# nackdai/aten

Measured on AMD Instinct MI355X. Metric: Mrays/sec (W*H*spp/1e6/s, reference definition), Sponza 1080p 1spp 5-bounce, higher is better.
Workload: dtype f32; 1 GPU; sponza_lod 1920x1080 1spp 5-bounce GGX+IBL, reference-built sponza_lod.sbvh (stand-in for missing sponza.obj); width=1920, height=1080, spp=1, max_depth=5, rr_depth=3, frames_in_flight=4, triangles=12852, bvh_nodes=38000, anyhit_twins=1, planar_area_lights=0

## Files before the change

aten_amd/_lib.py:

```python
import ctypes as C
import os

from . import build

_lib = None

K_NAMES = ["gen_path", "trace_closest", "shade", "trace_shadow", "accumulate_sample", "gather",
           "svgf_prepare", "svgf_temporal", "svgf_variance", "svgf_atrous", "trace_fused"]

SYMBOLS = [
    "atn_create", "atn_destroy", "atn_last_error", "atn_upload_scene", "atn_update_camera", "atn_update_tlas",
    "atn_init_sampler", "atn_set_random", "atn_set_screen_shard", "atn_render", "atn_reset", "atn_set_path_batches",
    "atn_set_frames_in_flight", "atn_bank_streams", "atn_side_stream", "atn_mgpu_set_frames_in_flight", "atn_set_sampling_options", "atn_sample_texture",
    "atn_svgf_render", "atn_svgf_set_motion_depth", "atn_svgf_reset", "atn_svgf_set_atrous_iterations",
    "atn_svgf_download", "atn_svgf_output_device", "atn_svgf_set_dilate_temporal_weight", "atn_svgf_denoise", "atn_svgf_upload",
    "atn_restir_set_options", "atn_restir_render", "atn_restir_set_motion_depth", "atn_restir_reset", "atn_restir_capture",
    "atn_restir_download", "atn_npr_render", "atn_npr_reset", "atn_npr_capture", "atn_npr_download",
    "atn_volume_render", "atn_volume_reset", "atn_volume_capture", "atn_volume_download", "atn_volume_phase_table",
    "atn_ao_set_params", "atn_ao_render", "atn_ao_reset", "atn_ao_capture", "atn_ao_download",
    "atn_film_device", "atn_tile_device", "atn_tile_slots", "atn_anyhit_twins", "atn_planar_area_lights", "atn_stream", "atn_synchronize",
    "atn_assemble_tiles", "atn_assemble_tiles_on", "atn_download_film", "atn_upload_film", "atn_get_stats", "atn_get_kernel_times",
    "atn_reset_kernel_times", "atn_generate_paths", "atn_trace_closest", "atn_cmj_samples", "atn_cmj_batch", "atn_ray_offset", "atn_get_random", "atn_random_count",
    "atn_material_table", "atn_material_eval", "atn_compact", "atn_compact2", "atn_sizeof_scene_desc", "atn_sizeof_destination",
    "atn_abi_version", "atn_build_id",
    "atn_download_path_cost", "atn_update_geometry", "atn_scene_device_arrays", "atn_lbvh_rebuild_list", "atn_lbvh_build",
    "atn_mgpu_update_geometry", "atn_mgpu_lbvh_rebuild_list",
    "atn_skin_create", "atn_skin_update", "atn_skin_compute", "atn_lbvh_rebuild_list_skinned", "atn_skin_download",
    "atn_skin_download_list", "atn_skin_destroy",
    "atn_set_geometry_motion", "atn_geometry_motion_stats", "atn_geometry_motion_matrices",
    "atn_mgpu_create", "atn_mgpu_destroy", "atn_mgpu_last_error", "atn_mgpu_shard_count", "atn_mgpu_shard_device",
    "atn_mgpu_upload_scene", "atn_mgpu_update_tlas", "atn_mgpu_update_camera", "atn_mgpu_init_sampler",
    "atn_mgpu_set_random", "atn_mgpu_render", "atn_mgpu_reset", "atn_mgpu_synchronize", "atn_mgpu_film_device",
    "atn_mgpu_download_film",
    "atn_set_regeneration", "atn_get_regeneration", "atn_render_burst", "atn_regen_stage_counts",
    "atn_mgpu_set_regeneration", "atn_mgpu_render_burst", "atn_set_upload_options", "atn_libm_probe", "atn_set_shade_math",
]


class Destination(C.Structure):
    _fields_ = [("width", C.c_int32), ("height", C.c_int32), ("maxDepth", C.c_int32),
                ("russianRouletteDepth", C.c_int32), ("sample", C.c_int32), ("frame", C.c_uint32),
                ("progressive", C.c_int32), ("break_on_terminate", C.c_int32),
                ("count_stats", C.c_int32), ("profile", C.c_int32)]


def lib():
    global _lib
    if _lib is None:
        path = os.environ.get("ATEN_AMD_LIB", build.HIP_LIB)
        if not os.path.exists(path):
            raise RuntimeError(
                "aten_amd: %s is missing. Build it with `python -m aten_amd.build hip` "
                "(or __graft_entry__.build()); there is no CPU fallback." % path)
        l = C.CDLL(path)
        vp = C.c_void_p
        l.atn_create.argtypes = [C.POINTER(vp), C.c_int]
        l.atn_destroy.argtypes = [vp]; l.atn_destroy.restype = None
        l.atn_last_error.argtypes = [vp]; l.atn_last_error.restype = C.c_char_p
        l.atn_upload_scene.argtypes = [vp, vp]
        l.atn_update_camera.argtypes = [vp, vp]
        l.atn_update_tlas.argtypes = [vp, vp, C.c_uint32, vp, C.c_uint32, vp, C.c_uint32]
        l.atn_download_path_cost.argtypes = [vp, vp]
        l.atn_update_geometry.argtypes = [vp, vp, vp, C.c_uint32, C.c_uint32, vp, C.c_uint32, C.c_uint32]
        l.atn_scene_device_arrays.argtypes = [vp, vp, vp, vp]
        l.atn_lbvh_rebuild_list.argtypes = [vp, C.c_uint32, C.c_uint32, C.c_uint32, vp, vp]
        l.atn_lbvh_build.argtypes = [vp, vp, C.c_uint32, C.c_int32, vp, vp, vp, C.c_uint32, C.c_int32, vp, vp, vp]
        l.atn_skin_create.argtypes = [vp, vp, C.c_uint32, C.c_uint32, C.c_uint32, C.c_uint32, C.c_uint32, C.POINTER(C.c_uint32)]
        l.atn_skin_update.argtypes = [vp, C.c_uint32, vp, C.c_uint32]
        l.atn_skin_compute.argtypes = [vp, C.c_uint32, C.c_int32, vp, vp]
        l.atn_lbvh_rebuild_list_skinned.argtypes = [vp, C.c_uint32, C.c_uint32]
        l.atn_skin_download.argtypes = [vp, C.c_uint32, C.c_int32, vp]
        l.atn_skin_download_list.argtypes = [vp, C.c_uint32, vp, C.c_uint32, C.POINTER(C.c_uint32)]
        l.atn_skin_destroy.argtypes = [vp, C.c_uint32]
        l.atn_set_geometry_motion.argtypes = [vp, C.c_int32]
        l.atn_geometry_motion_stats.argtypes = [vp, vp]
        l.atn_geometry_motion_matrices.argtypes = [vp, vp, vp]
        l.atn_mgpu_update_geometry.argtypes = [vp, vp, vp, C.c_uint32, C.c_uint32, vp, C.c_uint32, C.c_uint32]
        l.atn_mgpu_lbvh_rebuild_list.argtypes = [vp, C.c_uint32, C.c_uint32, C.c_uint32, vp, vp]
        l.atn_init_sampler.argtypes = [vp, C.c_int32, C.c_int32, C.c_int32]
        l.atn_set_random.argtypes = [vp, vp, C.c_uint32]
        l.atn_get_random.argtypes = [vp, vp, C.c_uint32]
        l.atn_random_count.argtypes = [vp]; l.atn_random_count.restype = C.c_uint32
        l.atn_set_screen_shard.argtypes = [vp, C.c_int32, C.c_int32]
        l.atn_render.argtypes = [vp, C.POINTER(Destination), vp]
        l.atn_reset.argtypes = [vp]
        l.atn_set_upload_options.argtypes = [vp, C.c_int32, C.c_int32, C.c_int32, C.c_int32]
        l.atn_set_regeneration.argtypes = [vp, C.c_int32]
        l.atn_set_shade_math.argtypes = [vp, C.c_int32]
        l.atn_get_regeneration.argtypes = [vp]; l.atn_get_regeneration.restype = C.c_int32
        l.atn_render_burst.argtypes = [vp, C.POINTER(Destination), C.c_int32, vp]
        l.atn_regen_stage_counts.argtypes = [vp, vp, vp, C.c_uint32, C.POINTER(C.c_uint32)]
        l.atn_set_path_batches.argtypes = [vp, C.c_int32]
        l.atn_set_frames_in_flight.argtypes = [vp, C.c_int32]
        l.atn_bank_streams.argtypes = [vp, C.POINTER(C.c_int32), C.POINTER(C.c_int32)]
        l.atn_set_sampling_options.argtypes = [vp, C.c_int32, C.c_int32]
        l.atn_sample_texture.argtypes = [vp, C.c_int32, C.c_uint32, vp, vp]
        l.atn_mgpu_set_frames_in_flight.argtypes = [vp, C.c_int32]
        l.atn_svgf_render.argtypes = [vp, vp, C.c_int32, vp, vp]
        l.atn_svgf_set_motion_depth.argtypes = [vp, vp, C.c_uint32]
        l.atn_svgf_reset.argtypes = [vp]
        l.atn_svgf_set_atrous_iterations.argtypes = [vp, C.c_int32]
        l.atn_svgf_download.argtypes = [vp, C.c_int32, vp]
        l.atn_restir_set_options.argtypes = [vp, C.c_int32, C.c_int32]
        l.atn_restir_render.argtypes = [vp, vp, C.c_int32, vp]
        l.atn_restir_set_motion_depth.argtypes = [vp, vp, C.c_uint32]
        l.atn_restir_reset.argtypes = [vp]
        l.atn_restir_capture.argtypes = [vp, C.c_int32]
        l.atn_restir_download.argtypes = [vp, C.c_int32, vp]
        l.atn_npr_render.argtypes = [vp, vp, vp]
        l.atn_npr_reset.argtypes = [vp]
        l.atn_npr_capture.argtypes = [vp, C.c_int32]
        l.atn_npr_download.argtypes = [vp, C.c_int32, vp]
        l.atn_volume_render.argtypes = [vp, vp, vp]
        l.atn_volume_reset.argtypes = [vp]
        l.atn_volume_capture.argtypes = [vp, C.c_int32]
        l.atn_volume_download.argtypes = [vp, C.c_int32, vp]
        l.atn_volume_phase_table.argtypes = [vp, C.c_float, C.c_uint32, vp, vp, vp, vp, vp, vp]
        l.atn_ao_set_params.argtypes = [vp, C.c_int32, C.c_float, C.c_int32]
        l.atn_ao_render.argtypes = [vp, vp, vp]
        l.atn_ao_reset.argtypes = [vp]
        l.atn_ao_capture.argtypes = [vp, C.c_int32]
        l.atn_ao_download.argtypes = [vp, C.c_int32, vp]
        l.atn_svgf_set_dilate_temporal_weight.argtypes = [vp, C.c_int32]
        l.atn_svgf_denoise.argtypes = [vp, vp, C.c_int32, vp, vp]
        l.atn_svgf_upload.argtypes = [vp, C.c_int32, C.c_int32, C.c_int32, vp]
        l.atn_svgf_output_device.argtypes = [vp]
        l.atn_svgf_output_device.restype = vp
        l.atn_film_device.argtypes = [vp]; l.atn_film_device.restype = vp
        l.atn_tile_device.argtypes = [vp]; l.atn_tile_device.restype = vp
        l.atn_tile_slots.argtypes = [vp]; l.atn_tile_slots.restype = C.c_uint32
        l.atn_anyhit_twins.argtypes = [vp]; l.atn_anyhit_twins.restype = C.c_uint32
        l.atn_planar_area_lights.argtypes = [vp]; l.atn_planar_area_lights.restype = C.c_uint32
        l.atn_stream.argtypes = [vp]; l.atn_stream.restype = vp
        l.atn_side_stream.argtypes = [vp]; l.atn_side_stream.restype = vp
        l.atn_synchronize.argtypes = [vp]
        l.atn_assemble_tiles.argtypes = [vp, vp, C.c_int32, vp]
        l.atn_assemble_tiles_on.argtypes = [vp, vp, C.c_int32, vp, vp]
        l.atn_download_film.argtypes = [vp, vp]
        l.atn_upload_film.argtypes = [vp, C.c_int32, C.c_int32, vp]
        l.atn_get_stats.argtypes = [vp, vp]
        l.atn_get_kernel_times.argtypes = [vp, vp, vp]
        l.atn_reset_kernel_times.argtypes = [vp]
        l.atn_generate_paths.argtypes = [vp, C.c_int32, C.c_int32, C.c_int32, C.c_uint32, vp]
        l.atn_trace_closest.argtypes = [vp, vp, C.c_uint32, C.c_float, C.c_float, vp, vp]
        l.atn_cmj_samples.argtypes = [vp, C.c_uint32, C.c_uint32, C.c_uint32, C.c_int32, vp]
        l.atn_cmj_batch.argtypes = [vp, C.c_uint32, vp, vp, vp, C.c_int32, vp]
        l.atn_ray_offset.argtypes = [vp, C.c_uint32, vp, vp, vp]
        l.atn_libm_probe.argtypes = [vp, C.c_int32, C.c_uint32, vp, vp, vp]
        l.atn_material_table.argtypes = [vp, C.c_int32, C.c_uint32, vp, vp, vp, vp, vp, vp, vp, vp]
        l.atn_material_eval.argtypes = [vp, C.c_int32, C.c_uint32, vp, vp, vp, vp, vp]
        l.atn_compact.argtypes = [vp, vp, C.c_uint32, vp, C.POINTER(C.c_uint32)]
        l.atn_compact2.argtypes = [vp, vp, vp, C.c_uint32, C.c_uint32, vp, C.POINTER(C.c_uint32), vp, C.POINTER(C.c_uint32)]
        l.atn_mgpu_create.argtypes = [C.POINTER(vp), vp, C.c_int32]
        l.atn_mgpu_destroy.argtypes = [vp]; l.atn_mgpu_destroy.restype = None
        l.atn_mgpu_last_error.argtypes = [vp]; l.atn_mgpu_last_error.restype = C.c_char_p
        l.atn_mgpu_shard_count.argtypes = [vp]; l.atn_mgpu_shard_count.restype = C.c_int32
        l.atn_mgpu_shard_device.argtypes = [vp, C.c_int32]; l.atn_mgpu_shard_device.restype = C.c_int32
        l.atn_mgpu_upload_scene.argtypes = [vp, vp]
        l.atn_mgpu_update_tlas.argtypes = [vp, vp, C.c_uint32, vp, C.c_uint32, vp, C.c_uint32]
        l.atn_mgpu_update_camera.argtypes = [vp, vp]
        l.atn_mgpu_init_sampler.argtypes = [vp, C.c_int32, C.c_int32, C.c_int32]
        l.atn_mgpu_set_random.argtypes = [vp, vp, C.c_uint32]
        l.atn_mgpu_render.argtypes = [vp, C.POINTER(Destination), vp]
        l.atn_mgpu_reset.argtypes = [vp]
        l.atn_mgpu_set_regeneration.argtypes = [vp, C.c_int32]
        l.atn_mgpu_render_burst.argtypes = [vp, C.POINTER(Destination), C.c_int32, vp]
        l.atn_mgpu_synchronize.argtypes = [vp]
        l.atn_mgpu_film_device.argtypes = [vp]; l.atn_mgpu_film_device.restype = vp
        l.atn_mgpu_download_film.argtypes = [vp, vp]
# ... 6 lines not shown
```

aten_amd/csrc/aten_amd.hip:

```cpp
#include <hip/hip_runtime.h>

#include <algorithm>
#include <cstdio>
#include <cstdlib>
#include <chrono>
#include <cstring>
#include <memory>
#include <random>
#include <string>
#include <vector>

#include "../../include/aten_amd.h"
#include "device/kernels.hpp"
#include "device/launch.hpp"
#include "device/svgf.hpp"
#include "device/restir.hpp"
#include "device/npr.hpp"
#include "device/ao.hpp"
#include "device/volume.hpp"
#include "device/lbvh.hpp"
#include "device/skinning.hpp"
#include "device/motion.hpp"
#include "host/scene_upload.hpp"
#include "host/ibl_precompute.hpp"

namespace atn {

#define ATN_HIP(expr)                                                                      \
    do {                                                                                   \
        hipError_t e_ = (expr);                                                            \
        if (e_ != hipSuccess) { return fail(ATN_ERR_HIP, std::string(#expr) + ": " + hipGetErrorString(e_)); } \
    } while (0)

template <class T>
struct DevBuf {
    T* p = nullptr;
    size_t n = 0;
    ~DevBuf() { release(); }
    void release() { if (p) { (void)hipFree(p); p = nullptr; n = 0; } }
    hipError_t resize(size_t count)
    {
        if (count <= n && p) return hipSuccess;
        release();
        if (count == 0) return hipSuccess;
        hipError_t e = hipMalloc((void**)&p, count * sizeof(T) + 256);
        if (e == hipSuccess) n = count;
        return e;
    }
    void swap(DevBuf& o) { std::swap(p, o.p); std::swap(n, o.n); }
    hipError_t upload(const std::vector<T>& v, hipStream_t s)
    {
        hipError_t e = resize(v.size() ? v.size() : 1);
        if (e != hipSuccess || v.empty()) return e;
        return hipMemcpyAsync(p, v.data(), v.size() * sizeof(T), hipMemcpyHostToDevice, s);
    }
};

__global__ void k_spin(unsigned long long ticks)
{
    const unsigned long long t0 = wall_clock64();
    while (wall_clock64() - t0 < ticks) { }
}
constexpr unsigned long long kSpinTicks = 30000;
inline bool streams_run_side_by_side(hipStream_t a, hipStream_t b, bool& ok)
{
    const double spin_us = (double)kSpinTicks / 100.0;
    for (int rep = 0; rep < 3; rep++) {
        if (hipStreamSynchronize(a) != hipSuccess || hipStreamSynchronize(b) != hipSuccess) { ok = false; return false; }
        const auto t0 = std::chrono::steady_clock::now();
        hipLaunchKernelGGL(k_spin, dim3(1), dim3(1), 0, a, kSpinTicks);
        hipLaunchKernelGGL(k_spin, dim3(1), dim3(1), 0, b, kSpinTicks);
        if (hipStreamSynchronize(a) != hipSuccess || hipStreamSynchronize(b) != hipSuccess) { ok = false; return false; }
        const double us = std::chrono::duration<double, std::micro>(std::chrono::steady_clock::now() - t0).count();
        ok = true;
        if (us < 1.5 * spin_us) return true;
    }
    ok = true;
    return false;
}

class PathTracing {
public:
    std::string last_error;
    int device = 0;
    hipStream_t stream = nullptr;
    static constexpr int kMaxBatches = 8;
    static constexpr int kMaxShards = 64;
    hipStream_t bstream[kMaxBatches] = {};
    hipEvent_t ev_fork = nullptr, ev_join[kMaxBatches] = {};
    int n_batches = 3;
    bool batches_forced = false;
    bool fuse_traces = true;
    bool env_probe_streams = true;
    bool env_lds_nodes = true;
    int env_anyhit_twin = 1;
    int env_anyhit_twin_dirs = 8;
    bool opt_node_layout = true, opt_planar_lights = true;
    bool env_atrous4 = true;
    int env_shade_waves = 0;
    int env_flavour = -1;

    DevBuf<float4> nodes, vtx_pos, vtx_nml, matrices, texels, carpaint, shade_tris;
    DevBuf<atn_triangle_param> tris;
    DevBuf<atn_object_param> objects;
    DevBuf<DevMaterial> materials;
    DevBuf<atn_light_param> lights;
    DevBuf<float4> light_plane;
    DevBuf<DevTexture> textures;
    DevBuf<atn_toon_param> toon;
    DevBuf<atn_light_param> npr_lights;
    DevBuf<float> screen_shadow;
    DevBuf<uint32_t> texels8;
    DevScene scene{};
    bool has_scene = false, has_camera = false;
    std::vector<int32_t> list_root_link;
    uint32_t n_planar_lights = 0;
    struct PlanarCert {
        int32_t inst_obj = -1, mesh_obj = -1, mtx_id = -1;
        atn_object_param inst{}, mesh{};
        atn_mat4 l2w{}, w2l{};
        uint32_t tri_first = 0, tri_count = 0, vtx_lo = 0, vtx_hi = 0;
    };
    std::vector<PlanarCert> planar_certs;
    void collect_planar_certs(const atn_scene_desc* s, const std::vector<atn_light_param>& lights)
    {
        planar_certs.clear();
        for (size_t i = 0; i < lights.size() && i < s->n_lights; i++) {
            if (!lights[i]._pad) continue;
            PlanarCert c;
            c.inst_obj = s->lights[i].arealight_objid;
            c.inst = s->objects[c.inst_obj];
            const atn_object_param* o = &s->objects[c.inst_obj];
            if (o->type == ATN_OBJ_INSTANCE) {
                c.mtx_id = o->mtx_id;
                if (c.mtx_id >= 0) { c.l2w = s->matrices[c.mtx_id]; c.w2l = s->matrices[c.mtx_id + 1]; }
                c.mesh_obj = o->object_id;
                c.mesh = s->objects[c.mesh_obj];
                o = &s->objects[c.mesh_obj];
            }
            c.tri_first = (uint32_t)o->triangle_id; c.tri_count = (uint32_t)o->triangle_num;
            c.vtx_lo = 0xFFFFFFFFu; c.vtx_hi = 0;
            for (uint32_t t = c.tri_first; t < c.tri_first + c.tri_count; t++)
                for (int k = 0; k < 3; k++) {
                    const uint32_t v = (uint32_t)s->triangles[t].idx[k];
                    c.vtx_lo = std::min(c.vtx_lo, v); c.vtx_hi = std::max(c.vtx_hi, v);
                }
            planar_certs.push_back(c);
        }
    }
    bool planar_certs_survive_objects(const atn_object_param* objs, uint32_t n_objs, const atn_mat4* mtxs, uint32_t n_mtxs) const
    {
        for (const PlanarCert& c : planar_certs) {
            if ((uint32_t)c.inst_obj >= n_objs || std::memcmp(&objs[c.inst_obj], &c.inst, sizeof(atn_object_param)) != 0) return false;
            if (c.mesh_obj >= 0 && ((uint32_t)c.mesh_obj >= n_objs || std::memcmp(&objs[c.mesh_obj], &c.mesh, sizeof(atn_object_param)) != 0)) return false;
            if (c.mtx_id >= 0 && n_mtxs
                && ((uint32_t)c.mtx_id + 1 >= n_mtxs || std::memcmp(&mtxs[c.mtx_id], &c.l2w, sizeof(atn_mat4)) != 0
                    || std::memcmp(&mtxs[c.mtx_id + 1], &c.w2l, sizeof(atn_mat4)) != 0)) return false;
        }
        return true;
    }
    bool planar_certs_survive_geometry(uint32_t vtx_offset, uint32_t n_vtx, uint32_t tri_offset, uint32_t n_tr) const
    {
        for (const PlanarCert& c : planar_certs) {
            if (n_vtx && vtx_offset <= c.vtx_hi && (uint64_t)vtx_offset + n_vtx > c.vtx_lo) return false;
            if (n_tr && tri_offset < c.tri_first + c.tri_count && (uint64_t)tri_offset + n_tr > c.tri_first) return false;
        }
        return true;
    }
    std::vector<int32_t> list_twin_delta;
    std::vector<HostSceneImage::TlasRef> tlas_refs;
    uint32_t top_base = 0, n_host_matrices = 0;
    std::vector<atn_mat4> host_matrices;
    std::vector<uint32_t> list_base, list_bytes, list_tri_leaves, list_inner;
    uint32_t n_scene_tris = 0, n_scene_vtx = 0, n_scene_mtrls = 0;

    struct LbvhScratch {
        DevBuf<uint32_t> codes[2], indices[2], counts, totals, arrived, offs;
        DevBuf<uint8_t> flips;
        DevBuf<int32_t> left, right, parent, first, last;
        DevBuf<atn_bvh_node> ref_nodes;
// ... 504 lines not shown
        if (const char* e = std::getenv("ATEN_AMD_PROBE_STREAMS")) env_probe_streams = std::atoi(e) != 0;
        if (const char* e = std::getenv("ATEN_AMD_TRACE")) { env_flavour = e[0] == 'r' ? 1 : 0; }
        if (const char* e = std::getenv("ATEN_AMD_BATCHES")) {
            n_batches = std::atoi(e);
            batches_forced = true;
            if (n_batches < 1) n_batches = 1;
            if (n_batches > kMaxBatches) n_batches = kMaxBatches;
        }
        return ATN_OK;
    }

    ~PathTracing()
    {
        for (auto& e : ev_pool) (void)hipEventDestroy(e);
        for (int k = 0; k < kMaxBatches; k++) {
            if (ev_join[k]) (void)hipEventDestroy(ev_join[k]);
            if (bstream[k]) (void)hipStreamDestroy(bstream[k]);
        }
        if (ev_fork) (void)hipEventDestroy(ev_fork);
        if (rs_ev) (void)hipEventDestroy(rs_ev);
        if (gm_ev) (void)hipEventDestroy(gm_ev);
        if (ao_ev) (void)hipEventDestroy(ao_ev);
        if (ev_gather) (void)hipEventDestroy(ev_gather);
        for (auto& e : sv_ev_prepare) if (e) (void)hipEventDestroy(e);
        if (ev_film) (void)hipEventDestroy(ev_film);
        if (sv_stream) (void)hipStreamDestroy(sv_stream);
        for (int i = 0; i < n_spare_ready; i++) {
            Bank& b = spare[i];
            for (int k = 0; k < kMaxBatches; k++) {
                if (b.ev_join[k]) (void)hipEventDestroy(b.ev_join[k]);
                if (b.bstream[k]) (void)hipStreamDestroy(b.bstream[k]);
            }
            if (b.ev_fork) (void)hipEventDestroy(b.ev_fork);
            if (b.ev_gather) (void)hipEventDestroy(b.ev_gather);
            for (auto& e : b.ev_read) if (e) (void)hipEventDestroy(e);
            if (b.stream) (void)hipStreamDestroy(b.stream);
        }
        if (stream) (void)hipStreamDestroy(stream);
        if (side_stream) (void)hipStreamDestroy(side_stream);
        if (scene_stream) (void)hipStreamDestroy(scene_stream);
        for (auto& e : ev_read) if (e) (void)hipEventDestroy(e);
        if (ev_scene) (void)hipEventDestroy(ev_scene);
        if (ev_stage) (void)hipEventDestroy(ev_stage);
        if (stage_p) (void)hipHostFree(stage_p);
    }

    int UpdateSceneData(const atn_scene_desc* s)
    {
        ATN_HIP(hipSetDevice(device));
        { int q = quiesce(); if (q) return q; }
        drop_alt_set(); cur_set = 0; scene_in_place = false; frame_since_update = true;
        skins.clear();
        HostSceneImage img;
        std::string err;
        const int layout_top = opt_node_layout ? kLayoutTopLevels : 0;
        const bool planar_lights = opt_planar_lights;
        if (!build_host_image(img, s, err, env_anyhit_twin, env_anyhit_twin_dirs, layout_top, planar_lights)) return fail(ATN_ERR_UNSUPPORTED, err);
        n_planar_lights = 0;
        for (const atn_light_param& l : img.lights) n_planar_lights += l._pad != 0 ? 1u : 0u;
        collect_planar_certs(s, img.lights);
        ATN_HIP(nodes.upload(img.nodes, stream));
        ATN_HIP(tris.upload(img.tris, stream));
        ATN_HIP(vtx_pos.upload(img.vtx_pos, stream));
        ATN_HIP(vtx_nml.upload(img.vtx_nml, stream));
        ATN_HIP(objects.upload(img.objects, stream));
        ATN_HIP(matrices.upload(img.matrices, stream));
        ATN_HIP(materials.upload(img.materials, stream));
        ATN_HIP(carpaint.upload(img.carpaint, stream));
        ATN_HIP(toon.upload(img.toon, stream));
        ATN_HIP(npr_lights.upload(img.npr_lights, stream));
        ATN_HIP(screen_shadow.upload(img.screen_shadow, stream));
        ATN_HIP(lights.upload(img.lights, stream));
        ATN_HIP(light_plane.upload(img.light_plane, stream));
        ATN_HIP(texels.upload(img.texels, stream));
        ATN_HIP(texels8.upload(img.texels8, stream));
        ATN_HIP(textures.upload(img.textures, stream));
        ATN_HIP(shade_tris.resize((size_t)kShadeTriQuads * (img.tris.size() ? img.tris.size() : 1)));
        if (!img.tris.empty())
            hipLaunchKernelGGL(k_pack_shade_tris, dim3(((uint32_t)img.tris.size() + 255) / 256), dim3(256), 0, stream, (const atn_triangle_param*)tris.p,
                               (const float4*)vtx_pos.p, (const float4*)vtx_nml.p, 0u, (uint32_t)img.tris.size(), shade_tris.p);
        ATN_HIP(hipGetLastError());
        ATN_HIP(hipStreamSynchronize(stream));
        scene = img.params;
        scene.nodes = nodes.p; scene.tris = tris.p; scene.shade_tris = shade_tris.p; scene.vtx_pos = vtx_pos.p; scene.vtx_nml = vtx_nml.p;
        scene.objects = objects.p; scene.matrices = matrices.p; scene.materials = materials.p; scene.carpaint = carpaint.p;
        scene.toon = toon.p; scene.npr_lights = npr_lights.p; scene.screen_shadow = img.screen_shadow.empty() ? nullptr : screen_shadow.p;
        scene.lights = lights.p; scene.light_plane = light_plane.p; scene.texels = texels.p; scene.texels8 = texels8.p; scene.textures = textures.p;
        scene.mtx_quads = (uint32_t)img.matrices.size();
        has_scene = true;
        if (gm_on) { gm_sv_ids[0] = gm_sv_ids[1] = gm_rs_has_ids = false; const int grc = gm_reset_history(); if (grc) return grc; }
        { const int nrc = npr_decode(s, img); if (nrc) return nrc; }
        { const int vrc = vol_decode(s, img); if (vrc) return vrc; }
        env_host.clear(); env_w = env_h = 0; ibl_tables_ready = false;
        {
            const int32_t ei = s->config.bg.envmap_tex_idx;
            if (ei >= 0 && (uint32_t)ei < s->n_textures && s->config.bg.enable_env_map) {
                const atn_texture_desc& t = s->textures[ei];
                env_host.assign(t.texels, t.texels + (size_t)t.width * t.height);
                env_w = t.width; env_h = t.height; env_multiplyer = s->config.bg.multiplyer;
            }
        }
        {
            int orc = apply_sampling_options();
            if (orc) return orc;
        }
        list_root_link = img.list_root_link; list_twin_delta = img.list_twin_delta; tlas_refs = img.tlas_refs;
        list_base = img.list_root; list_bytes = img.list_bytes; list_tri_leaves = img.list_tri_leaves; list_inner = img.list_inner;
        n_scene_tris = s->n_triangles; n_scene_vtx = s->n_vertices; n_scene_mtrls = s->n_materials;
        top_base = img.list_root[0];
        n_bottom_nodes = img.n_nodes - s->bvh_lists[0].count;
        n_host_matrices = s->n_matrices;
        host_matrices.assign(s->matrices, s->matrices + s->n_matrices);
        tree_is_deep = img.n_nodes >= kRefillMinNodes;
        return ATN_OK;
    }

    int apply_sampling_options()
    {
        scene.tex_bilinear = opt_tex_bilinear;
        scene.ibl_importance = 0;
        scene.ibl_cdf_v = nullptr; scene.ibl_cdf_u = nullptr; scene.ibl_w = 0; scene.ibl_h = 0;
        if (!opt_ibl_importance || env_host.empty()) return ATN_OK;
        if (!ibl_tables_ready) {
            IblTables t;
            const int32_t w = env_w, h = env_h;
            const atn_vec4* tex = env_host.data();
            const float mul = env_multiplyer;
            ibl_precompute(t, w, h, [&](int32_t x, int32_t y, float& r, float& g, float& b) {
                const float u = (float)(x + 0.5) / w, v = (float)(y + 0.5) / h;
                int32_t iu = (int32_t)(u * (float)(w - 1)), iv = (int32_t)(v * (float)(h - 1));
                iu = iu < 0 ? 0 : (iu > w - 1 ? w - 1 : iu); iv = iv < 0 ? 0 : (iv > h - 1 ? h - 1 : iv);
                const atn_vec4& c = tex[(size_t)iv * w + iu];
                r = c.x * mul; g = c.y * mul; b = c.z * mul;
            });
            ATN_HIP(ibl_cdf_v.upload(t.cdf_v, stream));
            ATN_HIP(ibl_cdf_u.upload(t.cdf_u, stream));
            ATN_HIP(hipStreamSynchronize(stream));
            ibl_tables_ready = true;
        }
        scene.ibl_cdf_v = ibl_cdf_v.p; scene.ibl_cdf_u = ibl_cdf_u.p; scene.ibl_w = env_w; scene.ibl_h = env_h;
        scene.ibl_importance = 1;
        return ATN_OK;
    }
    int set_sampling_options(int32_t ibl_importance, int32_t tex_bilinear)
    {
        ATN_HIP(hipSetDevice(device));
        { int q = quiesce(); if (q) return q; }
        opt_ibl_importance = ibl_importance ? 1 : 0;
        opt_tex_bilinear = tex_bilinear ? 1 : 0;
        return has_scene ? apply_sampling_options() : ATN_OK;
    }

    int updateBVH(const atn_object_param* objs, uint32_t n_objs, const atn_mat4* mtxs, uint32_t n_mtxs,
                  const atn_bvh_node* top, uint32_t n_top)
    {
        if (!has_scene) return fail(ATN_ERR_NO_SCENE, "atn_upload_scene has not been called");
        if (!objs || n_objs == 0 || !top || n_top == 0) return fail(ATN_ERR_INVALID_ARG, "empty object or top-layer array");
        ATN_HIP(hipSetDevice(device));
        if ((uint64_t)top_base + (uint64_t)n_top * kInnerBytes >= (1ull << 31)) return fail(ATN_ERR_UNSUPPORTED, "too many BVH nodes for 31-bit byte-offset links");
        if (n_mtxs && !mtxs) return fail(ATN_ERR_INVALID_ARG, "null matrix array");
        {
            std::string rerr;
            if (!validate_ranges(objs, n_objs, n_mtxs ? n_mtxs : n_host_matrices, nullptr, rerr)) return fail(ATN_ERR_UNSUPPORTED, rerr);
            for (uint32_t i = 0; i < n_objs; i++)
                if (objs[i].light_id >= scene.n_lights) return fail(ATN_ERR_UNSUPPORTED, "object light id out of range");
        }
        ListLayout lay;
        std::string err;
        if (!analyse_list(lay, top, n_top, true, err)) return fail(ATN_ERR_UNSUPPORTED, err);
        for (uint32_t j = 0; j < lay.order.size(); j++) {
            if (lay.kind[j] == KIND_TRI) return fail(ATN_ERR_UNSUPPORTED, "triangle leaves in this list need a full scene upload");
            lay.offset[j] = top_base + j * kInnerBytes;
        }
        ListEmitCtx c;
        c.objects = objs; c.n_objects = n_objs; c.n_matrices = n_mtxs ? n_mtxs : n_host_matrices;
        c.matrices = n_mtxs ? mtxs : (host_matrices.size() == n_host_matrices ? host_matrices.data() : nullptr);
        c.list_root_link = list_root_link.data(); c.n_lists = (uint32_t)list_root_link.size();
        c.list_twin_delta = list_twin_delta.size() == list_root_link.size() ? list_twin_delta.data() : nullptr;
        std::vector<HostSceneImage::TlasRef> new_refs;
        c.tlas_refs = &new_refs;
        const size_t top_bytes = lay.order.size() * (size_t)kInnerBytes;
        std::vector<float4> rec(top_bytes / 16 + 1, make_float4(0, 0, 0, 0));
        int32_t root = kLinkEnd;
        uint64_t counts[3] = { 0, 0, 0 };
        if (!emit_list(reinterpret_cast<char*>(rec.data()), lay, top, c, root, counts, err, top_base)) return fail(ATN_ERR_UNSUPPORTED, err);
        std::vector<float4> mv;
        if (n_mtxs) {
            mv.resize((size_t)n_mtxs * 4);
            for (uint32_t i = 0; i < n_mtxs; i++)
                for (int r = 0; r < 4; r++)
                    mv[4 * (size_t)i + r] = make_float4(mtxs[i].m[r][0], mtxs[i].m[r][1], mtxs[i].m[r][2], mtxs[i].m[r][3]);
        }
        const size_t need = ((size_t)top_base + top_bytes + 15) / 16;
        const size_t obj_bytes = (size_t)n_objs * sizeof(atn_object_param), mtx_bytes = mv.size() * sizeof(float4);
        const bool grow = need > nodes.n || n_objs > objects.n || mv.size() > matrices.n;
        if (grow) {
            { int q = quiesce(); if (q) return q; }
            drop_alt_set();
            if (need > nodes.n) {
                float4* bigger = nullptr;
                ATN_HIP(hipMalloc((void**)&bigger, need * sizeof(float4)));
                hipError_t e = hipMemcpyAsync(bigger, nodes.p, (size_t)top_base, hipMemcpyDeviceToDevice, stream);
                if (e == hipSuccess) e = hipStreamSynchronize(stream);
                if (e != hipSuccess) { (void)hipFree(bigger); return fail(ATN_ERR_HIP, hipGetErrorString(e)); }
                nodes.release();
                nodes.p = bigger; nodes.n = need;
            }
            if (n_objs > objects.n) ATN_HIP(objects.resize(n_objs));
            if (mv.size() > matrices.n) ATN_HIP(matrices.resize(mv.size()));
        }
        { int r = begin_scene_update(top_bytes + obj_bytes + mtx_bytes + 512); if (r) return r; }
        { int r = stage_copy(reinterpret_cast<char*>(nodes.p) + top_base, rec.data(), top_bytes); if (r) return r; log_range(SB_NODES, top_base, top_bytes); }
        { int r = stage_copy(objects.p, objs, obj_bytes); if (r) return r; log_range(SB_OBJECTS, 0, obj_bytes); }
        if (n_mtxs) { int r = stage_copy(matrices.p, mv.data(), mtx_bytes); if (r) return r; log_range(SB_MATRICES, 0, mtx_bytes); n_host_matrices = n_mtxs; host_matrices.assign(mtxs, mtxs + n_mtxs); }
        { int r = end_scene_update(); if (r) return r; }
        list_root_link[0] = root;
        if (scene.planar_lights && !planar_certs_survive_objects(objs, n_objs, mtxs, n_mtxs)) scene.planar_lights = 0;
        tlas_refs.swap(new_refs);
        scene.root_link = root;
        fill_root_direct(scene, rec.data(), top_base, n_mtxs ? mtxs : (host_matrices.size() == n_host_matrices ? host_matrices.data() : nullptr), n_mtxs ? n_mtxs : n_host_matrices);
        scene.node_bytes = (uint32_t)(top_base + top_bytes);
        scene.ident_row = c.ident_row;
        if (n_mtxs) scene.mtx_quads = (uint32_t)mv.size();
        point_scene_at_current_set();
        tree_is_deep = n_bottom_nodes + n_top >= kRefillMinNodes;
        return ATN_OK;
    }


    int updateGeometry(const atn_vec4* pos, const atn_vec4* nml, uint32_t n_vtx, uint32_t vtx_offset,
                       const atn_triangle_param* tr, uint32_t n_tr, uint32_t tri_offset)
    {
        if (!has_scene) return fail(ATN_ERR_NO_SCENE, "atn_upload_scene has not been called");
        if ((n_vtx && !pos && !nml) || (n_tr && !tr)) return fail(ATN_ERR_INVALID_ARG, "null geometry array");
        if ((uint64_t)vtx_offset + n_vtx > n_scene_vtx) return fail(ATN_ERR_INVALID_ARG, "vertex range outside the uploaded scene");
        if ((uint64_t)tri_offset + n_tr > n_scene_tris) return fail(ATN_ERR_INVALID_ARG, "triangle range outside the uploaded scene");
        for (uint32_t i = 0; i < n_tr; i++) {
            if (tr[i].mtrlid >= 0 && (uint32_t)tr[i].mtrlid >= n_scene_mtrls) return fail(ATN_ERR_UNSUPPORTED, "triangle material id out of range");
            for (int v = 0; v < 3; v++)
                if (tr[i].idx[v] < 0 || (uint32_t)tr[i].idx[v] >= n_scene_vtx) return fail(ATN_ERR_UNSUPPORTED, "triangle vertex index out of range");
        }
        skins_note_triangles(tr, n_tr, tri_offset);
        ATN_HIP(hipSetDevice(device));
        if (scene.planar_lights && !planar_certs_survive_geometry(vtx_offset, n_vtx, tri_offset, n_tr)) scene.planar_lights = 0;
        const size_t vb = (size_t)n_vtx * sizeof(float4), tb = (size_t)n_tr * sizeof(atn_triangle_param);
        { int r = begin_scene_update((pos ? vb : 0) + (nml ? vb : 0) + tb + 256); if (r) return r; }
        if (n_vtx && pos) { int r = stage_copy(vtx_pos.p + vtx_offset, pos, vb); if (r) return r; log_range(SB_VTX_POS, (size_t)vtx_offset * sizeof(float4), vb); }
        if (n_vtx && nml) { int r = stage_copy(vtx_nml.p + vtx_offset, nml, vb); if (r) return r; log_range(SB_VTX_NML, (size_t)vtx_offset * sizeof(float4), vb); }
        if (n_tr) { int r = stage_copy(tris.p + tri_offset, tr, tb); if (r) return r; log_range(SB_TRIS, (size_t)tri_offset * sizeof(atn_triangle_param), tb); }
        { int r = repack_shade_tris(0, n_scene_tris); if (r) return r; }
        return end_scene_update();
    }

    int repack_shade_tris(uint32_t first, uint32_t count)
    {
        if (!count) return ATN_OK;
        hipLaunchKernelGGL(k_pack_shade_tris, dim3((count + 255) / 256), dim3(256), 0, upd, (const atn_triangle_param*)tris.p,
                           (const float4*)vtx_pos.p, (const float4*)vtx_nml.p, first, count, shade_tris.p);
        ATN_HIP(hipGetLastError());
        log_range(SB_SHADE, (size_t)first * kShadeTriQuads * sizeof(float4), (size_t)count * kShadeTriQuads * sizeof(float4));
        return ATN_OK;
    }

    int lbvh_reserve(uint32_t n)
    {
        const uint32_t rounds = radix_rounds(n), tile = kSortThreads * rounds, nb = (n + tile - 1) / tile, nn = 2 * n - 1;
        for (int k = 0; k < 2; k++) {
            if (lb.codes[k].n < n) ATN_HIP(lb.codes[k].resize(n));
            if (lb.indices[k].n < n) ATN_HIP(lb.indices[k].resize(n));
        }
        if (lb.counts.n < 256u * nb) ATN_HIP(lb.counts.resize(256u * nb));
        if (lb.totals.n < 256u) ATN_HIP(lb.totals.resize(256u));
        if (lb.arrived.n < n) ATN_HIP(lb.arrived.resize(n));
        if (lb.offs.n < nn) ATN_HIP(lb.offs.resize(nn));
        if (lb.left.n < nn) ATN_HIP(lb.left.resize(nn));
        if (lb.right.n < nn) ATN_HIP(lb.right.resize(nn));
        if (lb.parent.n < nn) ATN_HIP(lb.parent.resize(nn));
        if (lb.first.n < n) ATN_HIP(lb.first.resize(n));
        if (lb.last.n < n) ATN_HIP(lb.last.resize(n));
        if (lb.ref_nodes.n < nn) ATN_HIP(lb.ref_nodes.resize(nn));
        if (lb.pre.n < n) ATN_HIP(lb.pre.resize(n));
        if (lb.suf.n < n) ATN_HIP(lb.suf.resize(n));
        { const uint32_t ns = (n + kBoundsBlock * kBoundsSuper - 1) / (kBoundsBlock * kBoundsSuper); if (lb.sup.n < ns) ATN_HIP(lb.sup.resize(ns)); }
        return ATN_OK;
    }

    int lbvh_enqueue(const atn_triangle_param* tr, uint32_t n, int32_t tri_id_offset, const float* bmin, const float* bmax,
                     const float4* vtx, int32_t vtx_offset, uint32_t image_base, hipStream_t st, const float* box_dev = nullptr)
    {
        { int r = lbvh_reserve(n); if (r) return r; }
        const uint32_t rounds = radix_rounds(n), tile = kSortThreads * rounds, nb = (n + tile - 1) / tile, nn = 2 * n - 1;
        const dim3 b256(256);
        if (box_dev) skin_launch_morton(st, tr, vtx, vtx_offset, n, box_dev, lb.codes[0].p, lb.indices[0].p);
        else {
            f3 mn, mx;
            mn.x = bmin[0]; mn.y = bmin[1]; mn.z = bmin[2]; mx.x = bmax[0]; mx.y = bmax[1]; mx.z = bmax[2];
            hipLaunchKernelGGL(k_lbvh_morton, dim3((n + 255) / 256), b256, 0, st, tr, vtx, vtx_offset, n, mn, mx, lb.codes[0].p, lb.indices[0].p);
        }
        for (uint32_t pass = 0; pass < 4; pass++) {
            const int in = pass & 1, out = in ^ 1;
            hipLaunchKernelGGL(k_radix_count, dim3(nb), dim3(kSortThreads), 0, st, (const uint32_t*)lb.codes[in].p, n, pass * 8u, lb.counts.p, nb, rounds);
            hipLaunchKernelGGL(k_radix_scan, dim3(256), dim3(64), 0, st, lb.counts.p, nb, lb.totals.p);
            hipLaunchKernelGGL(k_radix_scatter, dim3(nb), dim3(kSortThreads), 0, st, (const uint32_t*)lb.codes[in].p, (const uint32_t*)lb.indices[in].p,
// ... 306 lines not shown
        const uint32_t n_tiles = (uint32_t)tx * ty;
        const uint32_t tiles_per_rank = (n_tiles + world - 1) / world;
        const uint32_t slots = tiles_per_rank * 64;
        if (slots > kShadowSlotMask) return fail(ATN_ERR_UNSUPPORTED, "more than 2^26 path slots per GPU (shard the screen)");
        if (slots != n_slots) {
            ATN_HIP(ray_o.resize(slots)); ATN_HIP(ray_d.resize(slots)); ATN_HIP(thr.resize(slots));
            ATN_HIP(contrib.resize(slots)); ATN_HIP(isect.resize(slots));
            ATN_HIP(sh_o.resize(slots)); ATN_HIP(sh_d.resize(slots)); ATN_HIP(sh_c.resize(slots));
            ATN_HIP(accum.resize(slots)); ATN_HIP(done.resize(slots));
            ATN_HIP(queue0.resize(slots)); ATN_HIP(queue1.resize(slots)); ATN_HIP(shadow_q.resize(slots));
            ATN_HIP(tile_out.resize(slots));
            n_slots = slots;
        }
        if (w != film_w || h != film_h) {
            if (frames_in_flight > 1) { int qrc = quiesce(); if (qrc) return qrc; }
            ATN_HIP(film.resize((size_t)w * h));
            ATN_HIP(hipMemsetAsync(film.p, 0, (size_t)w * h * sizeof(float4), stream));
            film_w = w; film_h = h;
        }
        if (max_depth + 2 > counters_depth) {
            ATN_HIP(counters.resize((size_t)kMaxBatches * 4 * (max_depth + 2)));
            counters_depth = max_depth + 2;
        }
        if (!stats.p) {
            ATN_HIP(stats.resize(8));
            ATN_HIP(hipMemsetAsync(stats.p, 0, 64, stream));
        }
        return ATN_OK;
    }

    PathBuffers buffers(bool count, int batch = 0, uint32_t slot_begin = 0)
    {
        PathBuffers pb{};
        pb.ray_o = ray_o.p; pb.ray_d = ray_d.p; pb.thr = thr.p; pb.contrib = contrib.p; pb.seeds = seeds.p;
        pb.isect = isect.p; pb.sh_o = sh_o.p; pb.sh_d = sh_d.p; pb.sh_c = sh_c.p;
        pb.accum = accum.p; pb.done = done.p; pb.queue[0] = queue0.p + slot_begin; pb.queue[1] = queue1.p + slot_begin;
        pb.shadow_q = shadow_q.p + slot_begin;
        uint32_t* cb = counters.p + (size_t)batch * 4 * counters_depth;
        pb.q_count = cb; pb.sh_count = cb + counters_depth;
        pb.fetch_closest = cb + 2 * counters_depth; pb.fetch_shadow = cb + 3 * counters_depth;
        pb.stats = count ? stats.p : nullptr;
        pb.cost = count ? cost.p : nullptr;
        return pb;
    }

    FrameParams frame_params(const atn_destination& d)
    {
        FrameParams fp{};
        fp.width = d.width; fp.height = d.height; fp.n_slots = (int32_t)n_slots;
        fp.tiles_x = (d.width + 7) / 8; fp.tiles_y = (d.height + 7) / 8; fp.tiles_x_rcp = udiv_rcp((uint32_t)fp.tiles_x);
        fp.rank = rank; fp.world = world;
        fp.max_depth = d.maxDepth;
        fp.rr_depth = d.russianRouletteDepth;
        if (fp.rr_depth > fp.max_depth) fp.rr_depth = fp.max_depth - 1;
        fp.slot_begin = 0; fp.slot_end = (int32_t)n_slots;
        fp.chunk_items = kChunkItems;
        fp.sample = 0; fp.frame = d.frame; fp.n_seeds = n_seeds;
        fp.break_on_terminate = d.break_on_terminate; fp.progressive = d.progressive;
        return fp;
    }

    static uint32_t grid_for(uint32_t n, uint32_t cap_blocks = 256u * 16u)
    {
        uint32_t b = (n + 255u) / 256u;
        if (b == 0) b = 1;
        return b < cap_blocks ? b : cap_blocks;
    }

    bool tree_is_deep = false;
    static constexpr size_t kRefillMinNodes = 2048;
    static constexpr uint32_t kRefillMinPaths = 400u * 1000u;
    bool refill_walk(bool frame) const
    {
        if (env_flavour >= 0) return env_flavour == 1;
        return tree_is_deep && (!frame || n_slots >= kRefillMinPaths);
    }

    uint32_t lds_scene_bytes() const
    {
        const uint64_t b = (uint64_t)scene.node_bytes + (uint64_t)scene.mtx_quads * 16u;
        return (env_lds_nodes && b <= kLdsNodesMaxBytes) ? (uint32_t)b : 0u;
    }

    uint32_t trace_grid(uint32_t n_jobs, bool refill) const
    {
        if (refill) {
            const uint32_t waves_per_block = (uint32_t)kTraceBlock / 64u;
            uint32_t blocks = ((n_jobs + atn::kFetchChunk - 1u) / atn::kFetchChunk + waves_per_block - 1u) / waves_per_block;
            if (blocks < 1u) blocks = 1u;
            const uint32_t cap = (frames_in_flight > 1 ? 256u * 18u : 256u * 32u) / waves_per_block;
            return blocks < cap ? blocks : cap;
        }
        return grid_for(n_jobs);
    }

    PassPlan plan_pass(PassKind kind, uint32_t n) const
    {
        PassPlan p{};
        p.kind = kind;
        p.refill = refill_walk(true);
        p.lds_bytes = lds_scene_bytes();
        p.block = p.lds_bytes > 8192u ? 256u : 64u;
        p.trace_grid = trace_grid(n, p.refill);
        p.fused_grid = trace_grid(2u * n, p.refill);
        p.shade_items = n >= 400u * 1000u ? kChunkItems : 2;
        p.shade_grid = grid_for((n + (uint32_t)p.shade_items - 1u) / (uint32_t)p.shade_items);
        const bool big = n >= 1500u * 1000u;
        p.shade_waves = env_shade_waves ? env_shade_waves
                      : (kind == PassKind::Serial && frames_in_flight > 1 && (scene.material_set != kMsCore || big) ? 5 : 4);
        return p;
    }

    template <bool SHADOW>
    void launch_trace(const PassPlan& p, const PathBuffers& pb, bool count, int32_t b, hipStream_t st)
    {
        const dim3 g(p.trace_grid), t(p.refill ? (uint32_t)kTraceBlock : 256u);
        with_flags([&](auto c, auto refill) {
            if constexpr (SHADOW) hipLaunchKernelGGL((k_trace_shadow<decltype(c)::value, decltype(refill)::value>), g, t, 0, st, pb, scene, b);
            else hipLaunchKernelGGL((k_trace_closest<decltype(c)::value, decltype(refill)::value>), g, t, 0, st, pb, scene, b);
        }, count, p.refill);
    }

    template <bool SVGF>
    void launch_shade(const PassPlan& p, hipStream_t st, const PathBuffers& pb, const FrameParams& fp, int32_t b, const SvgfShade& sv)
    {
        if (!SVGF && shade_math_relaxed) {
            relaxed_launch_shade(scene.material_set, p.shade_waves, p.shade_grid, st, pb, scene, fp, camera, b);
            return;
        }
        with_shade_flavour(scene.material_set, p.shade_waves, [&](auto k) {
            using K = decltype(k);
            if constexpr (K::waves == 0) hipLaunchKernelGGL((k_shade<SVGF, K::ms>), dim3(p.shade_grid), dim3(256), 0, st, pb, scene, fp, camera, b, sv);
            else hipLaunchKernelGGL((k_shade_wn<SVGF, K::ms, K::waves>), dim3(p.shade_grid), dim3(256), 0, st, pb, scene, fp, camera, b, sv);
        });
    }

    void prof_begin(bool on, int kind, hipStream_t st = nullptr)
    {
        if (!st) st = stream;
        prof_stream = st;
        if (!on) return;
        if (spans.size() >= kMaxSpans) {
            (void)hipStreamSynchronize(stream);
            for (int k = 0; k < kMaxBatches; k++) (void)hipStreamSynchronize(bstream[k]);
            prof_collect();
        }
        if (ev_used + 2 > ev_pool.size()) {
            for (int i = 0; i < 64; i++) { hipEvent_t e; (void)hipEventCreate(&e); ev_pool.push_back(e); }
        }
        spans.push_back(Span{ kind, ev_used, ev_used + 1 });
        (void)hipEventRecord(ev_pool[ev_used], st);
    }
    void prof_end(bool on)
    {
        if (!on) return;
        (void)hipEventRecord(ev_pool[ev_used + 1], prof_stream);
        ev_used += 2;
    }
    void prof_collect()
    {
        for (const Span& s : spans) {
            float ms = 0;
            if (hipEventElapsedTime(&ms, ev_pool[s.e0], ev_pool[s.e1]) == hipSuccess) { k_ms[s.kind] += ms; k_launches[s.kind]++; }
        }
        spans.clear();
        ev_used = 0;
    }

    template <bool SVGF>
    int run_paths(const atn_destination* d, FrameParams fp, bool count, bool prof, const SvgfShade& sv, const SvgfFrame& sf)
    {
        int nb;
        if (batches_forced) {
            nb = n_batches;
            const uint32_t min_batch = 200u * 1000u;
            while (nb > 1 && n_slots / (uint32_t)nb < min_batch) nb--;
        }
        else {
            nb = refill_walk(true) ? 1 : (lds_scene_bytes() && frames_in_flight > 1) ? 1 : (n_slots >= (frames_in_flight > 1 ? 1500u : 800u) * 1000u ? 2 : 1);
            if (nb > n_batches) nb = n_batches;
        }
        if (nb > batch_streams_checked && nb > 1 && env_probe_streams) { int rc = separate_batch_streams(nb); if (rc) return rc; }
        uint32_t per = (n_slots + (uint32_t)nb - 1u) / (uint32_t)nb;
        per = (per + kChunk - 1u) / kChunk * kChunk;
        ATN_HIP(hipMemsetAsync(counters.p, 0, (size_t)nb * 4 * counters_depth * 4, stream));
        ATN_HIP(hipEventRecord(ev_fork, stream));
        for (int k = 0; k < nb; k++) {
            const uint32_t begin = (uint32_t)k * per;
            const uint32_t end = begin + per < n_slots ? begin + per : n_slots;
            if (begin >= end) continue;
            hipStream_t st = nb > 1 ? bstream[k] : stream;
            if (nb > 1) ATN_HIP(hipStreamWaitEvent(st, ev_fork, 0));
            PathBuffers pb = buffers(count, k, begin);
            fp.slot_begin = (int32_t)begin; fp.slot_end = (int32_t)end;
            const uint32_t n = end - begin;
            const PassPlan plan = plan_pass(SVGF ? PassKind::Svgf : PassKind::Serial, n);
            fp.chunk_items = plan.shade_items;
            const uint32_t g_slots = grid_for(n), g_all = (n + 255u) / 256u;
            for (int32_t s = 0; s < d->sample; s++) {
                fp.sample = s;
                if (s > 0) ATN_HIP(hipMemsetAsync(pb.q_count, 0, (size_t)4 * counters_depth * 4, st));
                prof_begin(prof, ATN_K_GEN, st);
                hipLaunchKernelGGL(k_gen_path, dim3(g_slots), dim3(256), 0, st, pb, fp, camera, (const uint32_t*)seeds.p);
// ... 1267 lines not shown
            { int q = quiesce(); if (q) return q; }
            ATN_HIP(hipMemsetAsync(film.p, 0, film.n * sizeof(float4), stream));
            return record_film_writer();
        }
        return ATN_OK;
    }
};

}

#include "host/mgpu.hpp"

struct atn_ctx { atn::PathTracing r; };
struct atn_mgpu { atn::MultiGpu m; };

using atn::PathTracing;

#define CTX_OR_FAIL(ctx) do { if (!(ctx)) return ATN_ERR_INVALID_ARG; } while (0)
#define CTX_QUIET_OR_FAIL(ctx) do { if (!(ctx)) return ATN_ERR_INVALID_ARG; \
    if ((ctx)->r.frames_in_flight > 1) { int q_ = (ctx)->r.quiesce(); if (q_) return q_; } } while (0)

template <class F>
static int guarded(atn_ctx* ctx, F&& f) noexcept
{
    try { return f(); }
    catch (const std::bad_alloc&) {
        try { return ctx->r.fail(ATN_ERR_OUT_OF_MEMORY, "out of host memory"); } catch (...) { return ATN_ERR_OUT_OF_MEMORY; }
    }
    catch (const std::exception& e) {
        try { return ctx->r.fail(ATN_ERR_INVALID_ARG, std::string("unexpected exception: ") + e.what()); } catch (...) { return ATN_ERR_INVALID_ARG; }
    }
    catch (...) { return ATN_ERR_INVALID_ARG; }
}
#define C_HIP(r, expr) do { hipError_t e_ = (expr); if (e_ != hipSuccess) return (r).fail(ATN_ERR_HIP, std::string(#expr) + ": " + hipGetErrorString(e_)); } while (0)

#define MG_OR_FAIL(mg) do { if (!(mg)) return ATN_ERR_INVALID_ARG; } while (0)
template <class F>
static int mg_guarded(atn_mgpu* mg, F&& f) noexcept
{
    try { return f(); }
    catch (const std::bad_alloc&) { try { return mg->m.fail(ATN_ERR_OUT_OF_MEMORY, "out of host memory"); } catch (...) { return ATN_ERR_OUT_OF_MEMORY; } }
    catch (...) { return ATN_ERR_INVALID_ARG; }
}

extern "C" {

int atn_create(atn_ctx** out, int device_ordinal)
{
    if (!out) return ATN_ERR_INVALID_ARG;
    *out = nullptr;
    atn_ctx* c = new (std::nothrow) atn_ctx();
    if (!c) return ATN_ERR_OUT_OF_MEMORY;
    int rc = c->r.init(device_ordinal);
    if (rc != ATN_OK) {
        std::fprintf(stderr, "atn_create: %s\n", c->r.last_error.c_str());
        delete c;
        return rc;
    }
    *out = c;
    return ATN_OK;
}

void atn_destroy(atn_ctx* ctx) { delete ctx; }

const char* atn_last_error(atn_ctx* ctx) { return ctx ? ctx->r.last_error.c_str() : "null context"; }

int atn_upload_scene(atn_ctx* ctx, const atn_scene_desc* scene)
{
    CTX_QUIET_OR_FAIL(ctx);
    if (!scene) return ctx->r.fail(ATN_ERR_INVALID_ARG, "null scene");
    return guarded(ctx, [&] { return ctx->r.UpdateSceneData(scene); });
}

int atn_set_upload_options(atn_ctx* ctx, int32_t anyhit_twin, int32_t anyhit_twin_dirs, int32_t node_layout, int32_t planar_lights)
{
    CTX_QUIET_OR_FAIL(ctx);
    if (anyhit_twin > 2 || (anyhit_twin_dirs >= 0 && anyhit_twin_dirs != 1 && anyhit_twin_dirs != 8)) return ctx->r.fail(ATN_ERR_INVALID_ARG, "upload option out of range");
    if (anyhit_twin >= 0) ctx->r.env_anyhit_twin = anyhit_twin;
    if (anyhit_twin_dirs >= 0) ctx->r.env_anyhit_twin_dirs = anyhit_twin_dirs;
    if (node_layout >= 0) ctx->r.opt_node_layout = node_layout != 0;
    if (planar_lights >= 0) ctx->r.opt_planar_lights = planar_lights != 0;
    return ATN_OK;
}
int atn_update_camera(atn_ctx* ctx, const atn_camera_param* camera) { CTX_OR_FAIL(ctx); return guarded(ctx, [&] { return ctx->r.updateCamera(camera); }); }

int atn_update_tlas(atn_ctx* ctx, const atn_object_param* objects, uint32_t n_objects, const atn_mat4* matrices, uint32_t n_matrices,
                    const atn_bvh_node* top_nodes, uint32_t n_top_nodes)
{
    CTX_OR_FAIL(ctx);
    return guarded(ctx, [&] { return ctx->r.updateBVH(objects, n_objects, matrices, n_matrices, top_nodes, n_top_nodes); });
}
int atn_update_geometry(atn_ctx* ctx, const atn_vec4* vtx_pos, const atn_vec4* vtx_nml, uint32_t n_vertices, uint32_t vtx_offset,
                        const atn_triangle_param* triangles, uint32_t n_triangles, uint32_t tri_offset)
{
    CTX_OR_FAIL(ctx);
    return guarded(ctx, [&] { return ctx->r.updateGeometry(vtx_pos, vtx_nml, n_vertices, vtx_offset, triangles, n_triangles, tri_offset); });
}
int atn_lbvh_rebuild_list(atn_ctx* ctx, uint32_t list_index, uint32_t tri_offset, uint32_t n_triangles, const float* bbox_min, const float* bbox_max)
{
    CTX_OR_FAIL(ctx);
    return guarded(ctx, [&] { return ctx->r.lbvh_rebuild_list(list_index, tri_offset, n_triangles, bbox_min, bbox_max, false); });
}
int atn_lbvh_build(atn_ctx* ctx, const atn_triangle_param* triangles, uint32_t n_triangles, int32_t tri_id_offset,
                   const float* bbox_min, const float* bbox_max, const atn_vec4* vtx_pos, uint32_t n_vertices, int32_t vtx_offset,
                   atn_bvh_node* out_nodes, uint32_t* out_sorted_codes, uint32_t* out_sorted_indices)
{
    CTX_QUIET_OR_FAIL(ctx);
    return guarded(ctx, [&] { return ctx->r.lbvh_build(triangles, n_triangles, tri_id_offset, bbox_min, bbox_max, vtx_pos, n_vertices, vtx_offset,
                                                       out_nodes, out_sorted_codes, out_sorted_indices); });
}
int atn_skin_create(atn_ctx* ctx, const atn_skinning_vertex* vertices, uint32_t n_vertices, uint32_t vtx_offset, uint32_t tri_offset, uint32_t n_triangles,
                    uint32_t n_matrices, atn_skin* out_skin)
{
    CTX_OR_FAIL(ctx);
    return guarded(ctx, [&] { return ctx->r.skin_create(vertices, n_vertices, vtx_offset, tri_offset, n_triangles, n_matrices, out_skin); });
}
int atn_skin_update(atn_ctx* ctx, atn_skin skin, const atn_mat4* matrices, uint32_t n)
{
    CTX_OR_FAIL(ctx);
    return guarded(ctx, [&] { return ctx->r.skin_update(skin, matrices, n); });
}
int atn_skin_compute(atn_ctx* ctx, atn_skin skin, int32_t is_restart, float* bbox_min, float* bbox_max)
{
    CTX_OR_FAIL(ctx);
    return guarded(ctx, [&] { return ctx->r.skin_compute(skin, is_restart != 0, bbox_min, bbox_max); });
}
int atn_lbvh_rebuild_list_skinned(atn_ctx* ctx, uint32_t list_index, atn_skin skin)
{
    CTX_OR_FAIL(ctx);
    return guarded(ctx, [&] { return ctx->r.lbvh_rebuild_list_skinned(list_index, skin); });
}
int atn_skin_download(atn_ctx* ctx, atn_skin skin, int32_t which, void* out_host)
{
    CTX_OR_FAIL(ctx);
    return guarded(ctx, [&] { return ctx->r.skin_download(skin, which, out_host); });
}
int atn_skin_download_list(atn_ctx* ctx, uint32_t list_index, void* out_host, uint32_t capacity_bytes, uint32_t* n_bytes)
{
    CTX_OR_FAIL(ctx);
    return guarded(ctx, [&] { return ctx->r.download_list(list_index, out_host, capacity_bytes, n_bytes); });
}
int atn_skin_destroy(atn_ctx* ctx, atn_skin skin)
{
    CTX_OR_FAIL(ctx);
    return guarded(ctx, [&] { return ctx->r.skin_destroy(skin); });
}
int atn_scene_device_arrays(atn_ctx* ctx, void** vtx_pos, void** vtx_nml, void** triangles)
{
    CTX_QUIET_OR_FAIL(ctx);
    if (!ctx->r.has_scene) return ctx->r.fail(ATN_ERR_NO_SCENE, "atn_upload_scene has not been called");
    { int q = ctx->r.quiesce(); if (q) return q; }
    ctx->r.drop_alt_set(); ctx->r.scene_in_place = true;
    if (ctx->r.gm_on) { const int g = ctx->r.set_geometry_motion(0); if (g) return g; }
    ctx->r.scene.planar_lights = 0;
    if (vtx_pos) *vtx_pos = ctx->r.vtx_pos.p;
    if (vtx_nml) *vtx_nml = ctx->r.vtx_nml.p;
    if (triangles) *triangles = ctx->r.tris.p;
    return ATN_OK;
}
int atn_set_geometry_motion(atn_ctx* ctx, int32_t on)
{
    CTX_QUIET_OR_FAIL(ctx);
    return guarded(ctx, [&] { return ctx->r.set_geometry_motion(on); });
}
int atn_geometry_motion_stats(atn_ctx* ctx, uint64_t* out3)
{
// ... 406 lines not shown
}
int atn_mgpu_render_burst(atn_mgpu* mg, const atn_destination* dst, int32_t n_frames, atn_vec4* out_host)
{
    MG_OR_FAIL(mg);
    return mg_guarded(mg, [&] { return mg->m.render_burst(dst, n_frames, out_host); });
}
int atn_mgpu_set_regeneration(atn_mgpu* mg, int32_t mode)
{
    MG_OR_FAIL(mg);
    if (mode < 0 || mode > 1) return mg->m.fail(ATN_ERR_INVALID_ARG, "regeneration mode out of range");
    return mg_guarded(mg, [&] {
        int rc = mg->m.synchronize();
        if (rc) return rc;
        for (int i = 0; i < mg->m.n; i++) mg->m.shard[i]->regen_mode = mode;
        return (int)ATN_OK;
    });
}
int atn_mgpu_reset(atn_mgpu* mg)
{
    MG_OR_FAIL(mg);
    return mg_guarded(mg, [&] { return mg->m.on_all([&](int i) { return mg->m.shard[i]->reset(); }); });
}
int atn_mgpu_synchronize(atn_mgpu* mg) { MG_OR_FAIL(mg); return mg_guarded(mg, [&] { return mg->m.synchronize(); }); }
int atn_mgpu_set_frames_in_flight(atn_mgpu* mg, int32_t n)
{
    MG_OR_FAIL(mg);
    return mg_guarded(mg, [&] { return mg->m.on_all([&](int i) { return mg->m.shard[i]->set_frames_in_flight(n); }); });
}
void* atn_mgpu_film_device(atn_mgpu* mg) { return mg ? (void*)mg->m.full.p : nullptr; }
int atn_mgpu_download_film(atn_mgpu* mg, atn_vec4* out_host)
{
    MG_OR_FAIL(mg);
    atn::MultiGpu& m = mg->m;
    if (!out_host || !m.full.p || m.width <= 0) return m.fail(ATN_ERR_INVALID_ARG, "atn_mgpu_download_film: nothing rendered yet");
    if (hipSetDevice(m.shard[0]->device) != hipSuccess
        || hipMemcpyAsync(out_host, m.full.p, (size_t)m.width * m.height * sizeof(float4), hipMemcpyDeviceToHost, m.comm) != hipSuccess
        || hipStreamSynchronize(m.comm) != hipSuccess) return m.fail(ATN_ERR_HIP, "film download failed");
    return ATN_OK;
}

int atn_generate_paths(atn_ctx* ctx, int32_t width, int32_t height, int32_t sample, uint32_t frame, atn_ray* out_host)
{
    CTX_QUIET_OR_FAIL(ctx);
    PathTracing& r = ctx->r;
    if (!r.has_camera || r.n_seeds == 0 || !out_host) return r.fail(ATN_ERR_INVALID_ARG, "atn_generate_paths: camera / sampler / output missing");
    C_HIP(r, hipSetDevice(r.device));
    const int32_t sr = r.rank, sw = r.world;
    r.rank = 0; r.world = 1;
    int rc = r.ensure_frame(width, height, 1);
    if (rc) { r.rank = sr; r.world = sw; return rc; }
    atn_destination d{}; d.width = width; d.height = height; d.maxDepth = 1; d.russianRouletteDepth = 1; d.sample = 1; d.frame = frame;
    atn::FrameParams fp = r.frame_params(d);
    fp.sample = sample;
    atn::PathBuffers pb = r.buffers(false);
    atn::DevBuf<atn_ray> out;
    C_HIP(r, out.resize((size_t)width * height));
    C_HIP(r, hipMemsetAsync(r.counters.p, 0, (size_t)4 * r.counters_depth * 4, r.stream));
    if (sample > 0) C_HIP(r, hipMemsetAsync(r.done.p, 0, (size_t)r.n_slots * 4, r.stream));
    hipLaunchKernelGGL(atn::k_gen_path, dim3(PathTracing::grid_for(r.n_slots)), dim3(256), 0, r.stream, pb, fp, r.camera, (const uint32_t*)r.seeds.p);
    hipLaunchKernelGGL(atn::k_export_rays, dim3((r.n_slots + 255) / 256), dim3(256), 0, r.stream, pb, fp, out.p);
    C_HIP(r, hipMemcpyAsync(out_host, out.p, (size_t)width * height * sizeof(atn_ray), hipMemcpyDeviceToHost, r.stream));
    C_HIP(r, hipStreamSynchronize(r.stream));
    r.rank = sr; r.world = sw;
    return ATN_OK;
}

int atn_trace_closest(atn_ctx* ctx, const atn_ray* rays_host, uint32_t n, float t_min, float t_max,
                      atn_intersection* out_host, uint64_t* stats_out)
{
    CTX_QUIET_OR_FAIL(ctx);
    PathTracing& r = ctx->r;
    if (!r.has_scene) return r.fail(ATN_ERR_NO_SCENE, "atn_upload_scene has not been called");
    if (!rays_host || !out_host) return r.fail(ATN_ERR_INVALID_ARG, "null rays / output");
    if (n == 0) { if (stats_out) { stats_out[0] = stats_out[1] = 0; } return ATN_OK; }
    C_HIP(r, hipSetDevice(r.device));
    atn::DevBuf<atn_ray> rays; atn::DevBuf<atn_intersection> out; atn::DevBuf<unsigned long long> st;
    C_HIP(r, rays.resize(n)); C_HIP(r, out.resize(n)); C_HIP(r, st.resize(8));
    C_HIP(r, hipMemcpyAsync(rays.p, rays_host, (size_t)n * sizeof(atn_ray), hipMemcpyHostToDevice, r.stream));
    C_HIP(r, hipMemsetAsync(st.p, 0, 64, r.stream));
    {
        const bool refill = r.refill_walk(false);
        const dim3 g(r.trace_grid(n, refill)), t(refill ? (uint32_t)atn::kTraceBlock : 256u);
        const atn_ray* rp = rays.p;
        atn::with_flags([&](auto c, auto rf) {
            hipLaunchKernelGGL((atn::k_trace_batch<decltype(c)::value, decltype(rf)::value>), g, t, 0, r.stream, r.scene, rp, n, t_min, t_max, out.p, st.p);
        }, stats_out != nullptr, refill);
    }
    C_HIP(r, hipGetLastError());
    C_HIP(r, hipMemcpyAsync(out_host, out.p, (size_t)n * sizeof(atn_intersection), hipMemcpyDeviceToHost, r.stream));
    unsigned long long hs[8] = {};
    C_HIP(r, hipMemcpyAsync(hs, st.p, 64, hipMemcpyDeviceToHost, r.stream));
    C_HIP(r, hipStreamSynchronize(r.stream));
    if (stats_out) { stats_out[0] = hs[3]; stats_out[1] = hs[4]; }
    return ATN_OK;
}

int atn_cmj_samples(atn_ctx* ctx, uint32_t index, uint32_t dimension, uint32_t scramble, int32_t n, float* out_host)
{
    CTX_QUIET_OR_FAIL(ctx);
    PathTracing& r = ctx->r;
    if (n <= 0 || !out_host) return r.fail(ATN_ERR_INVALID_ARG, "bad sample count");
    C_HIP(r, hipSetDevice(r.device));
    atn::DevBuf<float> out;
    C_HIP(r, out.resize(n));
    hipLaunchKernelGGL(atn::k_cmj_samples, dim3(1), dim3(64), 0, r.stream, index, dimension, scramble, n, out.p);
    C_HIP(r, hipMemcpyAsync(out_host, out.p, (size_t)n * 4, hipMemcpyDeviceToHost, r.stream));
    C_HIP(r, hipStreamSynchronize(r.stream));
    return ATN_OK;
}

int atn_cmj_batch(atn_ctx* ctx, uint32_t n, const uint32_t* index, const uint32_t* dimension, const uint32_t* scramble,
                  int32_t draws, float* out_host)
{
    CTX_QUIET_OR_FAIL(ctx);
    PathTracing& r = ctx->r;
    if (n == 0 || draws <= 0 || !index || !dimension || !scramble || !out_host) return r.fail(ATN_ERR_INVALID_ARG, "bad cmj batch");
    C_HIP(r, hipSetDevice(r.device));
    atn::DevBuf<uint32_t> di, dd, ds; atn::DevBuf<float> out;
    C_HIP(r, di.resize(n)); C_HIP(r, dd.resize(n)); C_HIP(r, ds.resize(n)); C_HIP(r, out.resize((size_t)n * draws));
    C_HIP(r, hipMemcpyAsync(di.p, index, 4 * (size_t)n, hipMemcpyHostToDevice, r.stream));
    C_HIP(r, hipMemcpyAsync(dd.p, dimension, 4 * (size_t)n, hipMemcpyHostToDevice, r.stream));
    C_HIP(r, hipMemcpyAsync(ds.p, scramble, 4 * (size_t)n, hipMemcpyHostToDevice, r.stream));
    hipLaunchKernelGGL(atn::k_cmj_batch, dim3((n + 255) / 256), dim3(256), 0, r.stream, n, (const uint32_t*)di.p,
                       (const uint32_t*)dd.p, (const uint32_t*)ds.p, (int)draws, out.p);
    C_HIP(r, hipGetLastError());
    C_HIP(r, hipMemcpyAsync(out_host, out.p, 4 * (size_t)n * draws, hipMemcpyDeviceToHost, r.stream));
    C_HIP(r, hipStreamSynchronize(r.stream));
    return ATN_OK;
}

int atn_ray_offset(atn_ctx* ctx, uint32_t n, const float* origins, const float* normals, float* out_host)
{
    CTX_QUIET_OR_FAIL(ctx);
    PathTracing& r = ctx->r;
    if (n == 0 || !origins || !normals || !out_host) return r.fail(ATN_ERR_INVALID_ARG, "bad ray offset batch");
    C_HIP(r, hipSetDevice(r.device));
    atn::DevBuf<float> o, nm, out;
    C_HIP(r, o.resize(3 * (size_t)n)); C_HIP(r, nm.resize(3 * (size_t)n)); C_HIP(r, out.resize(3 * (size_t)n));
    C_HIP(r, hipMemcpyAsync(o.p, origins, 12 * (size_t)n, hipMemcpyHostToDevice, r.stream));
    C_HIP(r, hipMemcpyAsync(nm.p, normals, 12 * (size_t)n, hipMemcpyHostToDevice, r.stream));
    hipLaunchKernelGGL(atn::k_ray_offset, dim3((n + 255) / 256), dim3(256), 0, r.stream, n, (const float*)o.p, (const float*)nm.p, out.p);
    C_HIP(r, hipGetLastError());
    C_HIP(r, hipMemcpyAsync(out_host, out.p, 12 * (size_t)n, hipMemcpyDeviceToHost, r.stream));
    C_HIP(r, hipStreamSynchronize(r.stream));
    return ATN_OK;
}

int atn_libm_probe(atn_ctx* ctx, int32_t kind, uint32_t n, const float* a, const float* b, float* out_host)
{
    CTX_QUIET_OR_FAIL(ctx);
    PathTracing& r = ctx->r;
    if (n == 0 || !a || !b || !out_host || kind < 0 || kind > 10) return r.fail(ATN_ERR_INVALID_ARG, "bad libm probe");
    C_HIP(r, hipSetDevice(r.device));
    atn::DevBuf<float> da, db, out;
    C_HIP(r, da.resize(n)); C_HIP(r, db.resize(n)); C_HIP(r, out.resize(n));
    C_HIP(r, hipMemcpyAsync(da.p, a, 4 * (size_t)n, hipMemcpyHostToDevice, r.stream));
    C_HIP(r, hipMemcpyAsync(db.p, b, 4 * (size_t)n, hipMemcpyHostToDevice, r.stream));
    hipLaunchKernelGGL(atn::k_libm_probe, dim3((n + 255) / 256), dim3(256), 0, r.stream, kind, n, (const float*)da.p, (const float*)db.p, out.p);
    C_HIP(r, hipGetLastError());
    C_HIP(r, hipMemcpyAsync(out_host, out.p, 4 * (size_t)n, hipMemcpyDeviceToHost, r.stream));
    C_HIP(r, hipStreamSynchronize(r.stream));
    return ATN_OK;
}

int atn_material_table(atn_ctx* ctx, int32_t mtrl_id, uint32_t n, const float* nrm, const float* wi,
                       const uint32_t* index, const uint32_t* dimension, const uint32_t* scramble, const float* uv,
                       float* out_sample, float* out_eval)
{
    CTX_QUIET_OR_FAIL(ctx);
// ... 103 lines not shown
```

aten_amd/csrc/device/kernels.hpp:

```cpp
#pragma once
#include "shading.hpp"
#include "toon.hpp"

#if defined(ATN_REGEN_TU) || defined(ATN_TEMPLATES_ONLY)
#define ATN_MAIN_TU 0
#else
#define ATN_MAIN_TU 1
#endif
#ifdef ATN_REGEN_TU
#define ATN_REGEN_KERNELS 1
#else
#define ATN_REGEN_KERNELS 0
#endif

namespace atn {

constexpr uint32_t F_TERMINATED = 1u, F_SINGULAR = 2u, F_HIT = 4u;
constexpr uint32_t kShadowSlotMask = (1u << 26) - 1u;
constexpr uint32_t kShadowStencilFlag = 0x40000000u;
constexpr uint32_t F_LAST_SPECULAR = 8u;

constexpr uint32_t F_PENDING = 16u;
constexpr uint32_t kRegenFlagMask = 31u;
constexpr uint32_t kRegenBounceShift = 5u, kRegenBounceMask = 255u;
// ... 243 lines not shown
            const RegenState st = regen_primary_state(pb, fp, cam, slot, 0u, 0u);
            pb.ray_o[slot] = st.o; pb.ray_d[slot] = st.d; pb.thr[slot] = st.t;
            pb.contrib[slot] = make_float4(0.0F, 0.0F, 0.0F, 0.0F);
            flags |= 1u << k;
        }
        auto entry_of = [&](int k) { return chunk + (uint32_t)k * 256u + threadIdx.x; };
        const uint32_t c = chunk / chunk_size;
        block_append2<decltype(entry_of), true>(sh, pb.q_regions + chunk, &pb.region_counts[2u * c], flags,
                                                pb.sh_regions + chunk, &pb.region_counts[2u * c + 1u], 0u, entry_of);
        if (threadIdx.x == 0u) { const uint32_t v = pb.region_counts[2u * c]; if (v) atomicAdd(&pb.group_counts[2u * (c / kRegenGroup)], v); }
    }
}

__global__ void __launch_bounds__(256) k_regen_compact(PathBuffers pb, int32_t stage, uint32_t chunk_size, uint32_t* group_counts_next, uint32_t n_groups)
{
    __shared__ uint32_t red[2][4];
    const uint32_t n_prev = pb.q_count[stage - 1];
    const uint32_t n_chunks = (n_prev + chunk_size - 1u) / chunk_size;
    const uint32_t c = blockIdx.x;
    if (c == 0u) { for (uint32_t g = threadIdx.x; g < 2u * n_groups; g += 256u) group_counts_next[g] = 0u; }
    if (c >= n_chunks) return;
    const uint32_t g0 = c / kRegenGroup;
    uint32_t sq = 0, ss = 0;
    for (uint32_t g = threadIdx.x; g < g0; g += 256u) { sq += pb.group_counts[2u * g]; ss += pb.group_counts[2u * g + 1u]; }
    for (uint32_t r = g0 * kRegenGroup + threadIdx.x; r < c; r += 256u) { sq += pb.region_counts[2u * r]; ss += pb.region_counts[2u * r + 1u]; }
    for (int off = 32; off > 0; off >>= 1) { sq += __shfl_down(sq, off); ss += __shfl_down(ss, off); }
    if ((threadIdx.x & 63u) == 0u) { red[0][threadIdx.x >> 6] = sq; red[1][threadIdx.x >> 6] = ss; }
    __syncthreads();
    const uint32_t base_q = red[0][0] + red[0][1] + red[0][2] + red[0][3];
    const uint32_t base_s = red[1][0] + red[1][1] + red[1][2] + red[1][3];
    const uint32_t nq = pb.region_counts[2u * c], ns = pb.region_counts[2u * c + 1u];
    uint32_t* __restrict__ qd = pb.queue[stage & 1];
    for (uint32_t e = threadIdx.x; e < nq; e += 256u) qd[base_q + e] = pb.q_regions[(size_t)c * chunk_size + e];
    for (uint32_t e = threadIdx.x; e < ns; e += 256u) pb.shadow_q[base_s + e] = pb.sh_regions[(size_t)c * chunk_size + e];
    if (c == n_chunks - 1u && threadIdx.x == 0u) { pb.q_count[stage] = base_q + nq; pb.sh_count[stage - 1] = base_s + ns; }
}

__global__ void __launch_bounds__(256) k_regen_flush(PathBuffers pb, FrameParams fp, RegenOut ro)
{
    const uint32_t slot = blockIdx.x * blockDim.x + threadIdx.x;
    if (slot >= (fp.n_valid < fp.n_items ? fp.n_valid : fp.n_items)) return;
    const uint32_t w = __float_as_uint(pb.ray_d[slot].w);
    if (w & F_PENDING) {
        const float4 pd = pb.pend[slot];
        regen_epilogue(pb, fp, ro, slot, mk3(pd), (uint32_t)fp.spp - 1u, __float_as_uint(pd.w), true);
    }
}

__global__ void __launch_bounds__(256) k_regen_end(PathBuffers pb, FrameParams fp, RegenOut ro)
{
    const uint32_t slot = blockIdx.x * blockDim.x + threadIdx.x;
    if (slot >= (uint32_t)fp.n_slots) return;
    int32_t x, y;
    if (!slot_to_pixel(fp, slot, x, y)) {
        if (ro.tile_out) ro.tile_out[slot] = make_float4(0.0F, 0.0F, 0.0F, 0.0F);
        return;
    }
    const uint32_t pixel = (uint32_t)(y * fp.width + x);
    float4 out = make_float4(0.0F, 0.0F, 0.0F, 0.0F);
    if (fp.progressive) out = ro.film[pixel];
    for (int32_t k = 0; k < fp.burst_frames; k++) {
        const float4 v = ro.frames[(size_t)k * (uint32_t)fp.n_slots + slot];
        if (fp.progressive) {
            const float4 cur = out;
            const float n = (float)((int32_t)cur.w);
            const float d = n + 1;
            out = make_float4((n * cur.x + v.x) / d, (n * cur.y + v.y) / d, (n * cur.z + v.z) / d, n + 1);
        }
        else {
            out = v;
        }
    }
    ro.film[pixel] = out;
    if (ro.tile_out) ro.tile_out[slot] = out;
}
#endif

#ifdef ATN_TRACE_WPE
#define ATN_TRACE_ATTR __attribute__((amdgpu_waves_per_eu(ATN_TRACE_WPE, ATN_TRACE_WPE)))
#else
#define ATN_TRACE_ATTR
#endif

template <bool COUNT, bool REFILL, class Job, bool LDSN = false>
ATN_DEV void trace_dispatch(const DevScene& sc, uint32_t count, uint32_t* fetch_counter, const Job& job, TravCounters* tc)
{
    if constexpr (REFILL) {
        __shared__ TraceShared sh;
        if (LDSN) lds_scene_copy(sc);
        trace_refill<COUNT, Job, LDSN>(sc, sh, count, fetch_counter, job, tc);
    }
    else {
        trace_simple<COUNT, Job, LDSN>(sc, count, job, tc);
    }
}

struct ClosestJob {
    PathBuffers pb;
    const uint32_t* __restrict__ q;
    float t_min;
    ATN_DEV void fetch(uint32_t j, float4& a, float4& b, float& stop_t) const { fetch_slot(q[j], a, b, stop_t); }
    ATN_DEV void fetch_slot(uint32_t slot, float4& a, float4& b, float& stop_t) const
    {
        const float4 ro = pb.ray_o[slot], rd = pb.ray_d[slot];
        stop_t = -kInf;
        a = make_float4(ro.x, ro.y, ro.z, kInf);
        b = make_float4(rd.x, rd.y, rd.z, __uint_as_float(slot));
    }
    ATN_DEV bool finish(uint32_t slot, const Hit& h, bool, float4&, float4&, float&) const
    {
        pb.isect[slot] = make_float4(__int_as_float(h.objid), h.a, h.b, __int_as_float(h.tri));
        return false;
    }
    ATN_DEV void cost(uint32_t slot, uint32_t nodes, uint32_t tris) const
    {
        if (pb.cost) { atomicAdd(&pb.cost[2u * slot], nodes); atomicAdd(&pb.cost[2u * slot + 1u], tris); }
    }
};

template <bool COUNT, bool REFILL>
__global__ void __launch_bounds__(kTraceBlock > 256 ? kTraceBlock : 256) k_trace_closest(PathBuffers pb, DevScene sc, int32_t bounce)
{
    const uint32_t count = pb.q_count[bounce];
    const ClosestJob job{ pb, pb.queue[bounce & 1], kEps };
    TravCounters tc{};
    trace_dispatch<COUNT, REFILL>(sc, count, &pb.fetch_closest[bounce], job, &tc);
    if (COUNT) {
        if (blockIdx.x == 0 && threadIdx.x == 0) atomicAdd(&pb.stats[0], (unsigned long long)count);
        wave_add_stat(&pb.stats[3], tc.nodes);
        wave_add_stat(&pb.stats[4], tc.tris);
    }
}

struct SvgfShade {
    float4* nd;
    float4* am;
    float4* primary;
    float w2c3[4];
};

#ifdef ATN_SHADE_WPE
#define ATN_SHADE_ATTR __attribute__((amdgpu_waves_per_eu(ATN_SHADE_WPE, ATN_SHADE_WPE)))
#else
#define ATN_SHADE_ATTR
#endif
#ifndef ATN_SHADE_PARTITION
#define ATN_SHADE_PARTITION 1
#endif
struct ShadePartShared { uint32_t perm[kChunk]; uint32_t wcount[kChunkItems][4][2]; };
template <bool ON> struct ShadeOrderShared { uint16_t inv[ON ? kChunk : 1]; uint8_t oflag[ON ? kChunk : 1]; };

template <bool SVGF, int MS, bool REGEN = false>
ATN_DEV void shade_body(const PathBuffers& pb, const DevScene& sc, const FrameParams& fp, const atn_camera_param& cam, int32_t bounce_arg, const SvgfShade& sv,
                        const RegenOut& ro = RegenOut{})
{
    __shared__ BlockAppendShared sh;
#if ATN_SHADE_PARTITION
    __shared__ ShadePartShared part;
    __shared__ ShadeOrderShared<REGEN> order[1];
#endif
    const uint32_t count = pb.q_count[bounce_arg];
    const uint32_t* __restrict__ q = pb.queue[bounce_arg & 1];
    uint32_t* __restrict__ qn = pb.queue[(bounce_arg + 1) & 1];
#if !ATN_SHADE_PARTITION
    uint32_t nhits = 0;
#endif

    const int items = fp.chunk_items;
    const uint32_t chunk_size = 256u * (uint32_t)items;
    for (uint32_t chunk = blockIdx.x * chunk_size; chunk < count; chunk += gridDim.x * chunk_size) {
      uint32_t push_bits = 0;
#if ATN_SHADE_PARTITION
      const uint32_t n_valid = count - chunk < chunk_size ? count - chunk : chunk_size;
      {
          const uint32_t tid = here_v(threadIdx.x);
          const uint32_t lane = tid & 63u, wave = tid >> 6;
          uint32_t hitmask = 0;
          __syncthreads();
#pragma unroll 1
          for (int k = 0; k < items; k++) {
              const uint32_t j = chunk + (uint32_t)k * 256u + threadIdx.x;
              const bool valid = j < count;
              const bool hit = valid && __float_as_int(pb.isect[q[j]].x) >= 0;
              if (hit) hitmask |= 1u << k;
              const unsigned long long bh = __ballot(hit), bm = __ballot(valid && !hit);
              if (lane == 0) { part.wcount[k][wave][0] = (uint32_t)__popcll(bh); part.wcount[k][wave][1] = (uint32_t)__popcll(bm); }
          }
          if (pb.stats) wave_add_stat(&pb.stats[2], (uint32_t)__popc(hitmask));
          __syncthreads();
          uint32_t total_hits = 0;
          for (int k = 0; k < items; k++) for (uint32_t w = 0; w < 4; w++) total_hits += part.wcount[k][w][0];
          uint32_t before_h = 0, before_m = 0;
#pragma unroll 1
          for (int k = 0; k < items; k++) {
              const uint32_t j = chunk + (uint32_t)k * 256u + threadIdx.x;
              const bool valid = j < count;
              const bool hit = (hitmask >> k) & 1u;
              const unsigned long long bh = __ballot(hit), bm = __ballot(valid && !hit);
              uint32_t bh_w = before_h, bm_w = before_m;
              for (uint32_t w = 0; w < 4; w++) {
                  if (w < wave) { bh_w += part.wcount[k][w][0]; bm_w += part.wcount[k][w][1]; }
                  before_h += part.wcount[k][w][0]; before_m += part.wcount[k][w][1];
              }
              if (valid) {
                  const uint32_t pos = hit ? bh_w + bits_below_lane(bh) : total_hits + bm_w + bits_below_lane(bm);
                  part.perm[pos] = q[j];
                  if constexpr (REGEN) order[0].inv[pos] = (uint16_t)(j - chunk);
              }
          }
// ... 450 lines not shown
                const uint32_t mattr = mid >= 0 ? sc.materials[mid].attrib : 0u;
                bool ignore = need_stencil && (mattr & kAttrStencilStencil);
                f3 hit_p = mk3(0.0F), hit_n = mk3(0.0F, 1.0F, 0.0F);
                if (ignore || (mattr & kAttrMaybeAlpha)) {
                    HitRec rec;
                    evaluate_hit(rec, sc, h.objid, h.tri, h.a, h.b);
                    hit_p = rec.p; hit_n = rec.normal;
                    if (mattr & kAttrMaybeAlpha) {
                        const DevMaterial& hm = sc.materials[mid];
                        const float4 albedo = sample_texture(sc, hm.albedoMap, rec.u, rec.v, make_float4(1.0F, 1.0F, 1.0F, 1.0F));
                        if (albedo.w * hm.baseColor.w < 1.0F) ignore = true;
                    }
                }
                if (ignore) {
                    if (lookups + 1u >= max_lookups) return false;
                    const float distToLight = pb.sh_o[slot].w;
                    const f3 odir = normalize(mk3(pb.sh_d[slot]));
                    const bool is_same_facing = dot(hit_n, odir) > 0.0F;
                    const f3 on = is_same_facing ? hit_n : -hit_n;
                    const f3 o = ray_offset(hit_p, on);
                    const f3 d = normalize(odir);
                    ra = make_float4(o.x, o.y, o.z, distToLight - kEps);
                    rb = make_float4(d.x, d.y, d.z, __uint_as_float(slot | ((lookups + 1u) << 27) | (h.objid == lightobj ? (1u << 26) : 0u)));
                    rstop = -kInf;
                    return true;
                }
            }
        }
        if (visible) {
            float4* dst = pb.contrib;
            if constexpr (REGEN) { if (lbits & kShadowFinalFlag) dst = pb.pend; }
            const float4 c = dst[slot];
            dst[slot] = make_float4(c.x + lc.x, c.y + lc.y, c.z + lc.z, REGEN ? c.w : 0.0F);
        }
        return false;
    }
};

template <bool COUNT, bool REFILL>
__global__ void __launch_bounds__(kTraceBlock > 256 ? kTraceBlock : 256) k_trace_shadow(PathBuffers pb, DevScene sc, int32_t bounce)
{
    const uint32_t count = pb.sh_count[bounce];
    const ShadowJob<true> job{ pb, sc, kEps };
    TravCounters tc{};
    trace_dispatch<COUNT, REFILL>(sc, count, &pb.fetch_shadow[bounce], job, &tc);
    if (COUNT) {
        if (blockIdx.x == 0 && threadIdx.x == 0) atomicAdd(&pb.stats[1], (unsigned long long)count);
        wave_add_stat(&pb.stats[5], tc.nodes);
        wave_add_stat(&pb.stats[6], tc.tris);
    }
}

template <bool ALPHA, bool REGEN = false>
struct FusedJob {
    ShadowJob<ALPHA, REGEN> s;
    ClosestJob c;
    uint32_t n_shadow;
    float t_min;
    ATN_DEV void fetch(uint32_t j, float4& a, float4& b, float& stop_t) const
    {
        if (j < n_shadow) {
            s.fetch(j, a, b, stop_t);
            b.w = __uint_as_float(__float_as_uint(b.w) | 0x80000000u);
        }
        else {
            c.fetch(j - n_shadow, a, b, stop_t);
        }
    }
    ATN_DEV bool finish(uint32_t payload, const Hit& h, bool is_hit, float4& ra, float4& rb, float& rstop) const
    {
        if (payload & 0x80000000u) {
            const bool again = s.finish(payload & 0x7fffffffu, h, is_hit, ra, rb, rstop);
            if (again) rb.w = __uint_as_float(__float_as_uint(rb.w) | 0x80000000u);
            return again;
        }
        return c.finish(payload, h, is_hit, ra, rb, rstop);
    }
    ATN_DEV void cost(uint32_t payload, uint32_t nodes, uint32_t tris) const
    {
        if (payload & 0x80000000u) s.cost(payload & 0x7fffffffu, nodes, tris); else c.cost(payload, nodes, tris);
    }
};

template <bool REFILL, bool ALPHA, bool LDSN = false, bool REGEN = false>
__global__ void ATN_TRACE_ATTR __launch_bounds__(kTraceBlock > 256 ? kTraceBlock : 256) k_trace_fused(PathBuffers pb, DevScene sc, int32_t bs, int32_t bc, int32_t launch)
{
    const uint32_t n_shadow = bs >= 0 ? pb.sh_count[bs] : 0u;
    const uint32_t n_closest = bc >= 0 ? pb.q_count[bc] : 0u;
    const FusedJob<ALPHA, REGEN> job{ ShadowJob<ALPHA, REGEN>{ pb, sc, kEps }, ClosestJob{ pb, pb.queue[(bc >= 0 ? bc : 0) & 1], kEps }, n_shadow, kEps };
    TravCounters tc{};
    trace_dispatch<false, REFILL, FusedJob<ALPHA, REGEN>, LDSN>(sc, n_shadow + n_closest, &pb.fetch_closest[launch], job, &tc);
}

template <int MS>
__global__ void __launch_bounds__(256) k_regen_shade(PathBuffers pb, DevScene sc, FrameParams fp, atn_camera_param cam, int32_t stage, RegenOut ro)
{
    shade_body<false, MS, true>(pb, sc, fp, cam, stage, SvgfShade{}, ro);
}
template <int MS, int WAVES>
__global__ void __attribute__((amdgpu_waves_per_eu(WAVES, WAVES))) __launch_bounds__(256) k_regen_shade_wn(PathBuffers pb, DevScene sc, FrameParams fp, atn_camera_param cam, int32_t stage, RegenOut ro)
{
    shade_body<false, MS, true>(pb, sc, fp, cam, stage, SvgfShade{}, ro);
}

#if ATN_MAIN_TU
__global__ void __launch_bounds__(256) k_accumulate_sample(PathBuffers pb, FrameParams fp)
{
    const uint32_t slot = (uint32_t)fp.slot_begin + blockIdx.x * blockDim.x + threadIdx.x;
    if (slot >= (uint32_t)fp.slot_end) return;
    int32_t x, y;
    if (!slot_to_pixel(fp, slot, x, y)) return;
    if (fp.sample > 0 && pb.done[slot]) return;
    const float4 c = pb.contrib[slot];
    const bool invalid = isnan(c.x) || isinf(c.x) || isnan(c.y) || isinf(c.y) || isnan(c.z) || isinf(c.z)
        || c.x < 0 || c.y < 0 || c.z < 0;
    if (invalid) return;
    float4 a = pb.accum[slot];
    a.x += c.x; a.y += c.y; a.z += c.z; a.w += 1.0F;
    pb.accum[slot] = a;
    const uint32_t flags = __float_as_uint(pb.ray_d[slot].w);
    if (fp.break_on_terminate && (flags & F_TERMINATED)) pb.done[slot] = 1;
}
#endif

template <bool ONE_SAMPLE>
__global__ void __launch_bounds__(256) k_gather(PathBuffers pb, FrameParams fp, float4* film, float4* tile_out)
{
    const uint32_t slot = blockIdx.x * blockDim.x + threadIdx.x;
    if (slot >= (uint32_t)fp.n_slots) return;
    int32_t x, y;
    float4 out = make_float4(0, 0, 0, 0);
    if (slot_to_pixel(fp, slot, x, y)) {
        float4 a;
        if (ONE_SAMPLE) {
            const float4 c = pb.contrib[slot];
            const bool invalid = isnan(c.x) || isinf(c.x) || isnan(c.y) || isinf(c.y) || isnan(c.z) || isinf(c.z)
                || c.x < 0 || c.y < 0 || c.z < 0;
            a = invalid ? make_float4(0.0F, 0.0F, 0.0F, 0.0F) : make_float4(0.0F + c.x, 0.0F + c.y, 0.0F + c.z, 1.0F);
        }
        else {
            a = pb.accum[slot];
        }
        const float cnt = a.w;
        const float4 v = make_float4(a.x / cnt, a.y / cnt, a.z / cnt, 1.0F);
        const uint32_t idx = (uint32_t)(y * fp.width + x);
        if (fp.progressive) {
            const float4 cur = film[idx];
            const float n = (float)((int32_t)cur.w);
            const float d = n + 1;
            out = make_float4((n * cur.x + v.x) / d, (n * cur.y + v.y) / d, (n * cur.z + v.z) / d, n + 1);
        }
        else {
            out = v;
        }
        film[idx] = out;
    }
    if (tile_out) tile_out[slot] = out;
}

#if ATN_MAIN_TU
__global__ void __launch_bounds__(256) k_assemble_tiles(const float4* __restrict__ gathered, float4* film,
                                                        int32_t width, int32_t height, int32_t tiles_x, int32_t tiles_y,
                                                        int32_t world, int32_t slots_per_rank)
{
    const uint32_t g = blockIdx.x * blockDim.x + threadIdx.x;
    if (g >= (uint32_t)(world * slots_per_rank)) return;
    FrameParams fp{};
    fp.width = width; fp.height = height; fp.tiles_x = tiles_x; fp.tiles_y = tiles_y; fp.tiles_x_rcp = udiv_rcp((uint32_t)tiles_x);
    fp.world = world; fp.rank = (int32_t)(g / (uint32_t)slots_per_rank);
    const uint32_t slot = g % (uint32_t)slots_per_rank;
    int32_t x, y;
    if (slot_to_pixel(fp, slot, x, y)) film[y * width + x] = gathered[g];
}

struct BatchJob {
    DevScene sc;
    const atn_ray* __restrict__ rays;
    atn_intersection* out;
    float t_min, t_max;
    ATN_DEV void fetch(uint32_t j, float4& a, float4& b, float& stop_t) const
    {
        const atn_ray r = rays[j];
        stop_t = -kInf;
        a = make_float4(r.org[0], r.org[1], r.org[2], t_max);
        b = make_float4(r.dir[0], r.dir[1], r.dir[2], __uint_as_float(j));
    }
    ATN_DEV bool finish(uint32_t j, const Hit& h, bool, float4&, float4&, float&) const
    {
        atn_intersection o;
        o.t = h.t; o.objid = h.objid; o.tri_id = h.tri; o.a = h.a; o.b = h.b; o.isVoxel = 0;
        o.mtrlid = -1; o.meshid = -1;
        if (h.objid >= 0) {
            const atn_triangle_param tp = sc.tris[h.tri];
            o.mtrlid = tp.mtrlid;
            o.meshid = tp.mesh_id < 0 ? h.meshid : tp.mesh_id;
        }
        out[j] = o;
        return false;
    }
    ATN_DEV void cost(uint32_t, uint32_t, uint32_t) const {}
};

template <bool COUNT, bool REFILL>
__global__ void __launch_bounds__(kTraceBlock > 256 ? kTraceBlock : 256) k_trace_batch(DevScene sc, const atn_ray* __restrict__ rays, uint32_t n,
                                                     float t_min, float t_max, atn_intersection* out,
                                                     unsigned long long* stats)
{
    const BatchJob job{ sc, rays, out, t_min, t_max };
    TravCounters tc{};
    trace_dispatch<COUNT, REFILL>(sc, n, reinterpret_cast<uint32_t*>(&stats[7]), job, &tc);
    if (COUNT) { wave_add_stat(&stats[3], tc.nodes); wave_add_stat(&stats[4], tc.tris); }
}

__global__ void __launch_bounds__(256) k_export_rays(PathBuffers pb, FrameParams fp, atn_ray* out)
{
    const uint32_t slot = blockIdx.x * blockDim.x + threadIdx.x;
    if (slot >= (uint32_t)fp.n_slots) return;
    int32_t x, y;
    if (!slot_to_pixel(fp, slot, x, y)) return;
    const float4 o = pb.ray_o[slot], d = pb.ray_d[slot];
    atn_ray r; r.org[0] = o.x; r.org[1] = o.y; r.org[2] = o.z; r.dir[0] = d.x; r.dir[1] = d.y; r.dir[2] = d.z;
    out[y * fp.width + x] = r;
}

__global__ void __launch_bounds__(64) k_cmj_samples(uint32_t index, uint32_t dim, uint32_t scramble, int n, float* out)
{
    if (blockIdx.x == 0 && threadIdx.x == 0) {
        Cmj s; s.idx = index; s.dim = dim; s.scramble = scramble;
        for (int i = 0; i < n; i++) out[i] = cmj_next(s);
    }
}

__global__ void __launch_bounds__(256) k_libm_probe(int32_t kind, uint32_t n, const float* __restrict__ a, const float* __restrict__ b, float* __restrict__ out)
{
    const uint32_t i = blockIdx.x * blockDim.x + threadIdx.x;
    if (i >= n) return;
    const float x = a[i], y = b[i];
    float r = 0.0F;
    switch (kind) {
    case 0: r = sinf(x); break;
    case 1: r = cosf(x); break;
    case 2: r = atanf(x); break;
    case 3: r = acosf(x); break;
    case 4: r = atan2f(x, y); break;
    case 5: r = logf(x); break;
    case 6: r = expf(x); break;
    case 7: r = powf(x, y); break;
    case 8: r = sqrtf(x); break;
    case 9: r = x / y; break;
    case 10: r = 1.0F / sqrtf(x); break;
    default: break;
    }
    out[i] = r;
}

__global__ void __launch_bounds__(256) k_ray_offset(uint32_t n, const float* __restrict__ o, const float* __restrict__ nrm, float* __restrict__ out)
{
    const uint32_t k = blockIdx.x * blockDim.x + threadIdx.x;
    if (k >= n) return;
    const f3 r = ray_offset(mk3(o[3 * k], o[3 * k + 1], o[3 * k + 2]), mk3(nrm[3 * k], nrm[3 * k + 1], nrm[3 * k + 2]));
    out[3 * k] = r.x; out[3 * k + 1] = r.y; out[3 * k + 2] = r.z;
}

__global__ void __launch_bounds__(256) k_cmj_batch(uint32_t n, const uint32_t* __restrict__ index, const uint32_t* __restrict__ dim,
                                                   const uint32_t* __restrict__ scramble, int draws, float* __restrict__ out)
{
    const uint32_t k = blockIdx.x * blockDim.x + threadIdx.x;
    if (k >= n) return;
    Cmj s; s.idx = index[k]; s.dim = dim[k]; s.scramble = scramble[k];
    for (int d = 0; d < draws; d++) out[(size_t)k * draws + d] = cmj_next(s);
}

__global__ void __launch_bounds__(256) k_sample_texture(DevScene sc, int32_t texid, uint32_t n, const float* __restrict__ uv, float* out)
{
    const uint32_t i = blockIdx.x * blockDim.x + threadIdx.x;
    if (i >= n) return;
    const float4 c = sample_texture(sc, texid, uv[2 * i], uv[2 * i + 1], make_float4(0, 0, 0, 0));
    out[4 * i] = c.x; out[4 * i + 1] = c.y; out[4 * i + 2] = c.z; out[4 * i + 3] = c.w;
}

__global__ void __launch_bounds__(64) k_material_table(DevScene sc, int32_t mtrl_id, uint32_t n, const float* nrm, const float* wi,
                                                       const uint32_t* index, const uint32_t* dimension, const uint32_t* scramble, const float* uv,
                                                       float* out_sample, float* out_eval)
{
    const uint32_t i = blockIdx.x * blockDim.x + threadIdx.x;
    if (i >= n) return;
    const DevMaterial m = sc.materials[mtrl_id];
    Cmj s; s.idx = index[i]; s.dim = dimension ? dimension[i] : 0u; s.scramble = scramble[i];
    f3 N = mk3(nrm[3 * i], nrm[3 * i + 1], nrm[3 * i + 2]);
    const f3 WI = mk3(wi[3 * i], wi[3 * i + 1], wi[3 * i + 2]);
    const float pre_r = m.type == ATN_MTRL_CARPAINT ? apply_normal<kMsCarPaint>(sc, m, mtrl_id, N, uv[2 * i], uv[2 * i + 1], WI, s) : 0.0F;
    MtrlSample ms;
    sample_material(ms, sc, m, N, WI, s, uv[2 * i], uv[2 * i + 1], mtrl_id, pre_r);
// ... 78 lines not shown
```

aten_amd/csrc/device/launch.hpp:

```cpp
#pragma once
#include <type_traits>
#include "kernels.hpp"

namespace atn {

template <class F>
void with_flags(F&& f) { f(); }
template <class F, class... B>
void with_flags(F&& f, bool flag, B... rest)
{
    if (flag) with_flags([&](auto... x) { f(std::true_type{}, x...); }, rest...);
    else with_flags([&](auto... x) { f(std::false_type{}, x...); }, rest...);
}

template <int MS, int WAVES>
struct ShadeFlavour { static constexpr int ms = MS, waves = WAVES; };
template <class F>
void with_shade_flavour(int material_set, int waves, F&& f)
{
    switch (material_set) {
    case kMsCore: if (waves == 5) f(ShadeFlavour<kMsCore, 5>{}); else f(ShadeFlavour<kMsCore, 4>{}); break;
    case kMsDisney: if (waves == 5) f(ShadeFlavour<kMsDisney, 5>{}); else f(ShadeFlavour<kMsDisney, 4>{}); break;
    case kMsAnalytic: if (waves == 5) f(ShadeFlavour<kMsAnalytic, 5>{}); else f(ShadeFlavour<kMsAnalytic, 4>{}); break;
    case kMsCarPaint: f(ShadeFlavour<kMsCarPaint, 0>{}); break;
    default: f(ShadeFlavour<kMsToon, 0>{}); break;
    }
}

enum class PassKind { Serial, Svgf, Regen };

struct PassPlan {
    PassKind kind;
    bool refill;
    uint32_t lds_bytes;
    uint32_t block;
    uint32_t trace_grid;
    uint32_t fused_grid;
    int shade_items;
    uint32_t shade_grid;
    int shade_waves;
};

struct TraceLaunch {
    bool closest;
    bool refill, lds;
    uint32_t grid, block, lds_bytes;
    int prof_kind;
};

inline TraceLaunch trace_launch(const PassPlan& p, int32_t stage)
{
    const bool refill = p.refill && stage != 0;
    const bool closest = p.kind != PassKind::Regen && stage == 0 && p.lds_bytes == 0u;
    return TraceLaunch{ closest, refill, p.lds_bytes != 0u, refill ? p.fused_grid : p.fused_grid * (256u / p.block),
                        refill ? (uint32_t)kTraceBlock : p.block, p.lds_bytes, p.refill && stage == 0 ? ATN_K_TRACE_CLOSEST : ATN_K_TRACE_FUSED };
}

template <bool REGEN>
void launch_trace_fused(const TraceLaunch& l, hipStream_t st, const PathBuffers& pb, const DevScene& sc, int32_t bs, int32_t bc, int32_t launch)
{
    const dim3 g(l.grid), t(l.block);
    if constexpr (!REGEN) if (l.closest) { hipLaunchKernelGGL((k_trace_closest<false, false>), g, t, l.lds_bytes, st, pb, sc, bc); return; }
    with_flags([&](auto refill, auto alpha, auto lds) {
        hipLaunchKernelGGL((k_trace_fused<decltype(refill)::value, decltype(alpha)::value, decltype(lds)::value, REGEN>), g, t, l.lds_bytes, st, pb, sc, bs, bc, launch);
    }, l.refill, sc.any_alpha != 0, l.lds);
}

void regen_launch_begin(uint32_t grid, hipStream_t st, const PathBuffers& pb, const FrameParams& fp, const atn_camera_param& cam);
void regen_launch_trace(const TraceLaunch& l, hipStream_t st, const PathBuffers& pb, const DevScene& sc, int32_t bs, int32_t bc, int32_t launch);
void regen_launch_shade(int material_set, int waves, uint32_t grid, hipStream_t st, const PathBuffers& pb, const DevScene& sc, const FrameParams& fp,
                        const atn_camera_param& cam, int32_t stage, const RegenOut& ro);
void regen_launch_compact(uint32_t grid, hipStream_t st, const PathBuffers& pb, int32_t stage, uint32_t chunk_size, uint32_t* group_counts_next, uint32_t n_groups);
void regen_launch_flush(uint32_t grid, hipStream_t st, const PathBuffers& pb, const FrameParams& fp, const RegenOut& ro);
void regen_launch_end(uint32_t grid, hipStream_t st, const PathBuffers& pb, const FrameParams& fp, const RegenOut& ro);

void relaxed_launch_shade(int material_set, int waves, uint32_t grid, hipStream_t st, const PathBuffers& pb, const DevScene& sc, const FrameParams& fp,
                          const atn_camera_param& cam, int32_t bounce);

struct RestirArgs;
void restir_launch_shade(int material_set, uint32_t grid, hipStream_t st, const PathBuffers& pb, const DevScene& sc, const FrameParams& fp,
                         const atn_camera_param& cam, const RestirArgs& ra);
void restir_launch_vis_prep(uint32_t grid, hipStream_t st, const PathBuffers& pb, const DevScene& sc, const FrameParams& fp, const RestirArgs& ra);
void restir_launch_temporal(int material_set, bool temporal, hipStream_t st, const PathBuffers& pb, const DevScene& sc, const FrameParams& fp,
                            const RestirArgs& ra);
void restir_launch_spatial(int material_set, hipStream_t st, const PathBuffers& pb, const DevScene& sc, const FrameParams& fp, const RestirArgs& ra);
void restir_launch_color(int material_set, hipStream_t st, const PathBuffers& pb, const DevScene& sc, const FrameParams& fp, const RestirArgs& ra);
void restir_launch_motion(hipStream_t st, const FrameParams& fp, const RestirArgs& ra);

struct NprArgs;
struct NprLaunch {
    uint32_t grid;
    bool refill;
    uint32_t trace_grid, trace_block, lds_bytes;
};
void npr_launch_gen(uint32_t grid, hipStream_t st, const PathBuffers& pb, const FrameParams& fp, const NprArgs& na);
void npr_launch_bounce(const NprLaunch& l, hipStream_t st, const PathBuffers& pb, const DevScene& sc, const FrameParams& fp,
                       const atn_camera_param& cam, const NprArgs& na, int32_t bounce);
void npr_launch_capture0(uint32_t grid, hipStream_t st, const PathBuffers& pb, const FrameParams& fp, const NprArgs& na);

struct AoArgs;
struct AoLaunch {
    uint32_t grid;
    uint32_t slot_grid;
    bool refill;
    uint32_t trace_grid, trace_block, lds_bytes;
};
void ao_launch_primary(const TraceLaunch& l, hipStream_t st, const PathBuffers& pb, const DevScene& sc, const AoArgs& aa);
void ao_launch_rays(const AoLaunch& l, hipStream_t st, const PathBuffers& pb, const DevScene& sc, const FrameParams& fp, const AoArgs& aa);
void ao_launch_resolve(const AoLaunch& l, hipStream_t st, const FrameParams& fp, const AoArgs& aa, float4* film, float4* tile_out);

struct VolArgs;
struct VolLaunch {
    uint32_t grid;
    uint32_t slot_grid;
    bool refill;
    uint32_t trace_grid, trace_block, lds_bytes;
};
inline VolLaunch vol_launch(const PassPlan& p, uint32_t n_slots, uint32_t shade_grid, uint32_t plain_trace_grid)
{
    VolLaunch l{};
    l.grid = shade_grid; l.slot_grid = (n_slots + 255u) / 256u;
    l.refill = p.refill; l.lds_bytes = p.lds_bytes;
    l.trace_block = p.refill ? (uint32_t)kTraceBlock : p.block;
    l.trace_grid = p.refill ? p.trace_grid : plain_trace_grid * (256u / p.block);
    return l;
}
void vol_launch_begin(const VolLaunch& l, hipStream_t st, const FrameParams& fp, const VolArgs& va);
void vol_launch_closest(const VolLaunch& l, hipStream_t st, const PathBuffers& pb, const DevScene& sc, const VolArgs& va, int32_t it);
void vol_launch_shade(int material_set, const VolLaunch& l, hipStream_t st, const PathBuffers& pb, const DevScene& sc, const FrameParams& fp,
                      const atn_camera_param& cam, const VolArgs& va, int32_t it);
void vol_launch_transmit(const VolLaunch& l, hipStream_t st, const PathBuffers& pb, const DevScene& sc, const VolArgs& va, int32_t it);
void vol_launch_reduce(const VolLaunch& l, hipStream_t st, const FrameParams& fp, const VolArgs& va);
void vol_launch_phase_table(hipStream_t st, float g, uint32_t n, const float* w, const float* r1, const float* r2, const float* wo, float* out_dir, float* out_eval);

struct SkinVtxArgs;
struct SkinTriArgs;
struct SkinLaunch {
    uint32_t vtx_grid, tri_grid;
    bool palette_lds;
};
inline SkinLaunch skin_launch(uint32_t n_vtx, uint32_t n_tri, uint32_t n_matrices, uint32_t palette_lds_max)
{
    SkinLaunch l{};
    l.vtx_grid = (n_vtx + 255u) / 256u;
    l.tri_grid = n_tri ? (n_tri + 255u) / 256u : 1u;
    l.palette_lds = n_matrices <= palette_lds_max;
    return l;
}
// ... 17 lines not shown
```

aten_amd/csrc/device/traverse.hpp:

```cpp
#pragma once
#include "scene_dev.hpp"

namespace atn {

struct Hit {
    float t;
    int32_t objid;
    int32_t tri;
    float a, b;
    int32_t meshid;
};

struct TravCounters { uint32_t nodes, tris, ray_nodes, ray_tris; };

struct RaySlab { f3 org, dir, invdir, oxinvdir; bool finite; };

ATN_DEV bool is_finite3(const f3& v)
{
    return (fabsf(v.x) <= kInf) && (fabsf(v.y) <= kInf) && (fabsf(v.z) <= kInf);
}

ATN_DEV void slab_setup(RaySlab& s, const f3& org, const f3& dir)
{
    s.org = org; s.dir = dir;
    s.invdir = 1.0F / (dir + 1e-6F);
    s.oxinvdir = (-org) * s.invdir;
    s.finite = is_finite3(s.invdir) && is_finite3(s.oxinvdir);
}

ATN_DEV bool slab_hit_exact(const RaySlab& s, const f3& bmin, const f3& bmax, float t_min, float t_max)
{
    const f3 f = bmax * s.invdir + s.oxinvdir;
    const f3 n = bmin * s.invdir + s.oxinvdir;
    const f3 tmx = mk3(smax(f.x, n.x), smax(f.y, n.y), smax(f.z, n.z));
    const f3 tmn = mk3(smin(f.x, n.x), smin(f.y, n.y), smin(f.z, n.z));
    const float t1 = smin(min3(tmx), t_max);
    const float t0 = smax(max3(tmn), t_min);
    return t0 <= t1;
}

ATN_DEV float hw_max(float a, float b) { float r; asm("v_max_f32 %0, %1, %2" : "=v"(r) : "v"(a), "v"(b)); return r; }
ATN_DEV float hw_min(float a, float b) { float r; asm("v_min_f32 %0, %1, %2" : "=v"(r) : "v"(a), "v"(b)); return r; }
ATN_DEV float hw_max3(float a, float b, float c) { float r; asm("v_max3_f32 %0, %1, %2, %3" : "=v"(r) : "v"(a), "v"(b), "v"(c)); return r; }
ATN_DEV float hw_min3(float a, float b, float c) { float r; asm("v_min3_f32 %0, %1, %2, %3" : "=v"(r) : "v"(a), "v"(b), "v"(c)); return r; }

ATN_DEV bool slab_hit_fast(const RaySlab& s, const f3& bmin, const f3& bmax, float t_min, float t_max)
{
    const f3 f = bmax * s.invdir + s.oxinvdir;
    const f3 n = bmin * s.invdir + s.oxinvdir;
    const float t1 = hw_min3(hw_min(hw_max(f.x, n.x), hw_max(f.y, n.y)), hw_max(f.z, n.z), t_max);
    const float t0 = hw_max3(hw_max(hw_min(f.x, n.x), hw_min(f.y, n.y)), hw_min(f.z, n.z), t_min);
    return t0 <= t1;
}

#ifndef ATN_TRACE_BLOCK
#define ATN_TRACE_BLOCK 256
#endif
constexpr int kTraceBlock = ATN_TRACE_BLOCK;

ATN_DEV float4 ld16(const char* base, uint32_t byte_off)
{
    return *reinterpret_cast<const float4*>(base + byte_off);
}

typedef int atn_v4i __attribute__((ext_vector_type(4)));
ATN_DEV __amdgpu_buffer_rsrc_t node_rsrc(const DevScene& sc)
{
    return __builtin_amdgcn_make_buffer_rsrc((void*)sc.nodes, 0, (int)sc.node_bytes, 0x00020000);
}
ATN_DEV float4 ld16_buf(__amdgpu_buffer_rsrc_t r, uint32_t byte_off)
{
    const atn_v4i v = __builtin_amdgcn_raw_buffer_load_b128(r, (int)byte_off, 0, 0);
    return make_float4(__int_as_float(v.x), __int_as_float(v.y), __int_as_float(v.z), __int_as_float(v.w));
}

extern __shared__ float4 atn_dyn_lds[];
template <bool LDSN>
ATN_DEV float4 ldn(const char* base, uint32_t byte_off)
{
    if constexpr (LDSN) return atn_dyn_lds[byte_off >> 4];
    else return ld16(base, byte_off);
}

ATN_DEV void lds_scene_copy(const DevScene& sc)
{
    const uint32_t n16 = sc.node_bytes >> 4;
    for (uint32_t i = threadIdx.x; i < n16; i += blockDim.x) atn_dyn_lds[i] = sc.nodes[i];
    for (uint32_t i = threadIdx.x; i < sc.mtx_quads; i += blockDim.x) atn_dyn_lds[n16 + i] = sc.matrices[i];
    __syncthreads();
}
template <bool LDSN>
ATN_DEV float4 ldm(const DevScene& sc, int32_t row)
{
    if constexpr (LDSN) return atn_dyn_lds[(sc.node_bytes >> 4) + (uint32_t)row];
    else return sc.matrices[row];
}

ATN_DEV bool leaf_test(const RaySlab& ray, const float4& q0, const float4& q1, const float4& q2, float t_min,
                       Hit& hit, float& t_max, int32_t objid, int32_t meshid, bool& accept, float& t_out)
{
    const f3 e1 = mk3(q1), e2 = mk3(q2);
    const f3 r = ray.org - mk3(q0);
    const f3 u = cross(ray.dir, e2);
    const f3 v = cross(r, e1);
    const float inv = 1.0F / dot(u, e1);
    const float t = dot(v, e2) * inv;
    const float beta = dot(u, r) * inv;
    const float gamma = dot(v, ray.dir) * inv;
    const bool isect = ((beta >= 0.0F && beta <= 1.0F) && (gamma >= 0.0F && gamma <= 1.0F)
        && (beta + gamma <= 1.0F) && t >= 0.0F);
    const bool is_hit = isect && (t < kInf);
    accept = (t_min < (is_hit ? t : kInf)) && is_hit && (t < hit.t);
    if (accept) {
        hit.t = t; hit.a = beta; hit.b = gamma;
        hit.objid = objid; hit.tri = __float_as_int(q0.w); hit.meshid = meshid;
        t_max = t;
    }
    t_out = t;
    return is_hit;
}


struct Walk {
    RaySlab wray, ray;
    RaySlab lray;
    bool pending;
    Hit hit;
    float t_max, stop_t;
    uint32_t payload;
    int32_t node, objid, meshid, top_hit, top_miss;
};

ATN_DEV int32_t anyhit_root(int32_t root, int32_t twin, const f3& d)
{
    const int32_t delta = twin & ~15;
    const uint32_t octant = (d.x > 0.0F ? 1u : 0u) | (d.y > 0.0F ? 2u : 0u) | (d.z > 0.0F ? 4u : 0u);
    return root + delta + (int32_t)((twin & 1) ? octant : 0u) * delta;
}

template <bool IDENT = false, bool COUNT = false>
ATN_DEV void walk_start(Walk& w, const DevScene& sc, const float4& a, const float4& b, float stop_t, TravCounters* cnt = nullptr)
{
    w.t_max = a.w;
    w.stop_t = stop_t;
    w.payload = __float_as_uint(b.w);
    w.hit.t = kInf; w.hit.objid = -1; w.hit.tri = -1; w.hit.a = 0.0F; w.hit.b = 0.0F; w.hit.meshid = -1;
    if (sc.root_direct) {
        if (COUNT) { cnt->nodes++; cnt->ray_nodes++; }
        w.wray.org = mk3(a); w.wray.dir = mk3(b); w.wray.invdir = mk3(0.0F); w.wray.oxinvdir = mk3(0.0F); w.wray.finite = true;
        if (sc.root_w2l >= 0) {
            m4 m;
            m.r0 = make_float4(sc.root_m[0], sc.root_m[1], sc.root_m[2], sc.root_m[3]);
            m.r1 = make_float4(sc.root_m[4], sc.root_m[5], sc.root_m[6], sc.root_m[7]);
            m.r2 = make_float4(sc.root_m[8], sc.root_m[9], sc.root_m[10], sc.root_m[11]);
            m.r3 = make_float4(0.0F, 0.0F, 0.0F, 1.0F);
            const f3 o = m4_apply(m, w.wray.org);
            const f3 d = normalize(m4_applyXYZ(m, w.wray.dir));
            slab_setup(w.ray, o, d);
        }
        else {
            slab_setup(w.ray, w.wray.org, w.wray.dir);
        }
        w.lray = w.ray;
        w.node = sc.root_blas;
        if (sc.root_twin != 0 && stop_t == kInf) w.node = anyhit_root(sc.root_blas, sc.root_twin, w.ray.dir);
        w.objid = sc.root_objid; w.meshid = sc.root_meshid; w.top_hit = kLinkEnd; w.top_miss = kLinkEnd;
        return;
    }
    slab_setup(w.wray, mk3(a), mk3(b));
    w.ray = w.wray;
    w.node = sc.root_link; w.objid = -1; w.meshid = -1; w.top_hit = kLinkEnd; w.top_miss = kLinkEnd;
    if constexpr (IDENT) {
        if (sc.ident_row >= 0) {
            m4 m;
            m.r0 = ldm<true>(sc, sc.ident_row + 0); m.r1 = ldm<true>(sc, sc.ident_row + 1);
            m.r2 = ldm<true>(sc, sc.ident_row + 2); m.r3 = ldm<true>(sc, sc.ident_row + 3);
            const f3 o = m4_apply(m, w.wray.org);
            const f3 d = normalize(m4_applyXYZ(m, w.wray.dir));
            slab_setup(w.lray, o, d);
        }
    }
}

#ifndef ATN_INNER_BURST
#define ATN_INNER_BURST 5
#endif
constexpr int kInnerBurst = ATN_INNER_BURST;
#ifndef ATN_SIMPLE_BURST_LDS
#define ATN_SIMPLE_BURST_LDS 2
#endif
constexpr int kSimpleBurstLds = ATN_SIMPLE_BURST_LDS;

template <bool LDSN>
ATN_DEV void ld32(const char* base, uint32_t byte_off, float4& a, float4& b)
{
    if constexpr (LDSN) { a = atn_dyn_lds[byte_off >> 4]; b = atn_dyn_lds[(byte_off >> 4) + 1u]; }
    else {
        const float4* p = reinterpret_cast<const float4*>(base + byte_off);
        a = p[0]; b = p[1];
    }
}

template <bool COUNT, int BURST, bool FAST, bool LDSN>
ATN_DEV void inner_burst(Walk& w, const char* __restrict__ nb, float t_min, TravCounters* cnt)
{
#pragma unroll
    for (int k = 0; k < BURST; k++) {
        if (w.node >= 0) {
            float4 q0, q1;
            ld32<LDSN>(nb, (uint32_t)w.node, q0, q1);
            if (COUNT) { cnt->nodes++; cnt->ray_nodes++; }
            const bool box = FAST ? slab_hit_fast(w.ray, mk3(q0), mk3(q1), t_min, w.t_max)
                                  : slab_hit_exact(w.ray, mk3(q0), mk3(q1), t_min, w.t_max);
            w.node = __float_as_int(box ? q0.w : q1.w);
        }
    }
}

#ifndef ATN_TLAS_PERIOD
#define ATN_TLAS_PERIOD 3
#endif
template <bool COUNT, int BURST, class Job, bool LDSN = false, bool DEFER = false>
ATN_DEV void walk_iteration(Walk& w, bool& all_finite, const DevScene& sc, const char* __restrict__ nb, float t_min,
                            const Job& job, TravCounters* cnt, uint32_t iter = 0)
{
    const bool live = w.node != kLinkEnd;
    if (all_finite) inner_burst<COUNT, BURST, true, LDSN>(w, nb, t_min, cnt);
    else inner_burst<COUNT, BURST, false, LDSN>(w, nb, t_min, cnt);
    bool ended = live && w.node == kLinkEnd;
    bool is_hit = false;

    const bool tlas_turn = LDSN || ATN_TLAS_PERIOD <= 1 || (iter % (uint32_t)ATN_TLAS_PERIOD) == 0u;
    const bool at_tlas = w.node != kLinkEnd && (w.node & kLinkTypeMask) == kLinkTlasBit && tlas_turn;
    if (w.node != kLinkEnd && w.node < 0 && ((w.node & kLinkLeafBit) || tlas_turn)) {
        const uint32_t off = (uint32_t)w.node & kLinkOffsetMask;
        float4 q0, q1;
        if constexpr (LDSN) { q0 = ldn<true>(nb, off); q1 = ldn<true>(nb, off + 16u); }
        else { const __amdgpu_buffer_rsrc_t rs = node_rsrc(sc); q0 = ld16_buf(rs, off); q1 = ld16_buf(rs, off + 16u); }
        if (COUNT) { cnt->nodes++; cnt->ray_nodes++; }
        if (w.node & kLinkLeafBit) {
            float4 q2;
            if constexpr (LDSN) q2 = ldn<true>(nb, off + 32u);
            else q2 = ld16_buf(node_rsrc(sc), off + 32u);
            if (COUNT) { cnt->tris++; cnt->ray_tris++; }
            bool accept; float t;
            is_hit = leaf_test(w.ray, q0, q1, q2, t_min, w.hit, w.t_max, w.objid, w.meshid, accept, t);
            w.node = __float_as_int(q1.w);
            if (accept && t <= w.stop_t) { w.node = kLinkEnd; w.top_hit = kLinkEnd; w.top_miss = kLinkEnd; }
            ended = w.node == kLinkEnd;
        }
        else {
            w.objid = __float_as_int(q0.x);
            const int32_t w2l = __float_as_int(q0.y);
            w.meshid = __float_as_int(q1.x);
            w.top_hit = __float_as_int(q1.y);
            w.top_miss = __float_as_int(q1.z);
            if (LDSN && (__float_as_int(q0.w) & kTlasIdentity)) {
                w.ray = w.lray;
            }
            else if (w2l >= 0) {
                m4 m;
                m.r0 = ldm<LDSN>(sc, w2l + 0); m.r1 = ldm<LDSN>(sc, w2l + 1);
                m.r2 = ldm<LDSN>(sc, w2l + 2); m.r3 = ldm<LDSN>(sc, w2l + 3);
                const f3 o = m4_apply(m, w.wray.org);
                const f3 d = normalize(m4_applyXYZ(m, w.wray.dir));
                slab_setup(w.ray, o, d);
            }
            else {
                w.ray = w.wray;
            }
            is_hit = true;
            w.node = __float_as_int(q0.z);
            if (w.stop_t == kInf && __float_as_int(q1.w) != 0) w.node = anyhit_root(w.node, __float_as_int(q1.w), w.ray.dir);
            ended = false;
        }
    }

    if (ended) {
        w.node = is_hit ? w.top_hit : w.top_miss;
        w.top_hit = kLinkEnd; w.top_miss = kLinkEnd;
        if (w.node != kLinkEnd) w.ray = w.wray;
        if (w.node == kLinkEnd) {
            if constexpr (DEFER) w.pending = true;
            else {
                float4 ra, rb;
                float rstop;
                if (COUNT) { job.cost(w.payload, cnt->ray_nodes, cnt->ray_tris); cnt->ray_nodes = 0; cnt->ray_tris = 0; }
                if (job.finish(w.payload, w.hit, w.hit.objid >= 0, ra, rb, rstop)) walk_start<LDSN, COUNT>(w, sc, ra, rb, rstop, cnt);
            }
        }
    }
    if (__any(ended || at_tlas) || !all_finite) all_finite = __all(w.node == kLinkEnd || w.ray.finite) != 0;
}

template <bool COUNT>
ATN_DEV void walk_run(Walk& w, const DevScene& sc, const char* __restrict__ nb, float t_min, TravCounters* cnt)
{
    while (w.node != kLinkEnd) {
        const uint32_t off = (uint32_t)w.node & kLinkOffsetMask;
        const float4 q0 = ld16(nb, off);
        const float4 q1 = ld16(nb, off + 16u);
        if (COUNT) { cnt->nodes++; cnt->ray_nodes++; }
        bool is_hit;
        if (w.node >= 0) {
            const bool box = w.ray.finite ? slab_hit_fast(w.ray, mk3(q0), mk3(q1), t_min, w.t_max)
                                          : slab_hit_exact(w.ray, mk3(q0), mk3(q1), t_min, w.t_max);
            w.node = __float_as_int(box ? q0.w : q1.w);
            is_hit = false;
        }
        else if (w.node & kLinkLeafBit) {
            const float4 q2 = ld16(nb, off + 32u);
            if (COUNT) { cnt->tris++; cnt->ray_tris++; }
            bool accept; float t;
            is_hit = leaf_test(w.ray, q0, q1, q2, t_min, w.hit, w.t_max, w.objid, w.meshid, accept, t);
            w.node = __float_as_int(q1.w);
            if (accept && t <= w.stop_t) { w.node = kLinkEnd; w.top_hit = kLinkEnd; w.top_miss = kLinkEnd; }
        }
        else {
            w.objid = __float_as_int(q0.x);
            const int32_t w2l = __float_as_int(q0.y);
            w.meshid = __float_as_int(q1.x);
            w.top_hit = __float_as_int(q1.y);
            w.top_miss = __float_as_int(q1.z);
            if (w2l >= 0) {
                m4 m;
                m.r0 = sc.matrices[w2l + 0]; m.r1 = sc.matrices[w2l + 1];
                m.r2 = sc.matrices[w2l + 2]; m.r3 = sc.matrices[w2l + 3];
                const f3 o = m4_apply(m, w.wray.org);
                const f3 d = normalize(m4_applyXYZ(m, w.wray.dir));
                slab_setup(w.ray, o, d);
            }
            else {
                w.ray = w.wray;
            }
            is_hit = true;
            w.node = __float_as_int(q0.z);
            if (w.stop_t == kInf && __float_as_int(q1.w) != 0) w.node = anyhit_root(w.node, __float_as_int(q1.w), w.ray.dir);
        }
        if (w.node == kLinkEnd) {
            w.node = is_hit ? w.top_hit : w.top_miss;
            w.top_hit = kLinkEnd; w.top_miss = kLinkEnd;
            w.ray = w.wray;
        }
    }
}

#ifndef ATN_DEFER_FINISH
#define ATN_DEFER_FINISH 1
#endif
template <bool COUNT, class Job, bool LDSN>
ATN_DEV bool walk_finish(Walk& w, const DevScene& sc, const Job& job, TravCounters* cnt)
{
    bool restarted = false;
    if (w.pending) {
        w.pending = false;
        float4 ra, rb;
        float rstop;
        if (COUNT) { job.cost(w.payload, cnt->ray_nodes, cnt->ray_tris); cnt->ray_nodes = 0; cnt->ray_tris = 0; }
        if (job.finish(w.payload, w.hit, w.hit.objid >= 0, ra, rb, rstop)) { walk_start<LDSN, COUNT>(w, sc, ra, rb, rstop, cnt); restarted = true; }
    }
    return __any(restarted) != 0;
}

template <bool COUNT, class Job, bool LDSN = false>
ATN_DEV void trace_simple(const DevScene& sc, uint32_t count, const Job& job, TravCounters* cnt)
{
    const char* __restrict__ nb = reinterpret_cast<const char*>(sc.nodes);
    if constexpr (LDSN) lds_scene_copy(sc);
    const float t_min = sc.bvh_hit_min > 0 ? sc.bvh_hit_min : job.t_min;
    const uint32_t stride = gridDim.x * blockDim.x;
    for (uint32_t j = blockIdx.x * blockDim.x + threadIdx.x; j < count; j += stride) {
        Walk w;
        float4 a, b;
        float stop_t;
        job.fetch(j, a, b, stop_t);
        if constexpr (LDSN && kSimpleBurstLds > 0) {
            walk_start<true, COUNT>(w, sc, a, b, stop_t, cnt);
            w.pending = false;
            bool all_finite = __all(w.ray.finite) != 0;
            for (;;) {
                while (__any(w.node != kLinkEnd))
                    walk_iteration<COUNT, kSimpleBurstLds, Job, LDSN, true>(w, all_finite, sc, nb, t_min, job, cnt);
                if (!walk_finish<COUNT, Job, LDSN>(w, sc, job, cnt)) break;
                all_finite = __all(w.node == kLinkEnd || w.ray.finite) != 0;
            }
            continue;
        }
      restart:
        walk_start<LDSN, COUNT>(w, sc, a, b, stop_t, cnt);
        while (w.node != kLinkEnd) {
            const uint32_t off = (uint32_t)w.node & kLinkOffsetMask;
            const float4 q0 = ldn<LDSN>(nb, off);
            const float4 q1 = ldn<LDSN>(nb, off + 16u);
            if (COUNT) { cnt->nodes++; cnt->ray_nodes++; }
            bool is_hit;
            if (w.node >= 0) {
                const bool box = w.ray.finite ? slab_hit_fast(w.ray, mk3(q0), mk3(q1), t_min, w.t_max)
                                              : slab_hit_exact(w.ray, mk3(q0), mk3(q1), t_min, w.t_max);
                w.node = __float_as_int(box ? q0.w : q1.w);
                is_hit = false;
            }
            else if (w.node & kLinkLeafBit) {
                const float4 q2 = ldn<LDSN>(nb, off + 32u);
                if (COUNT) { cnt->tris++; cnt->ray_tris++; }
                bool accept; float t;
                is_hit = leaf_test(w.ray, q0, q1, q2, t_min, w.hit, w.t_max, w.objid, w.meshid, accept, t);
                w.node = __float_as_int(q1.w);
                if (accept && t <= w.stop_t) { w.node = kLinkEnd; w.top_hit = kLinkEnd; w.top_miss = kLinkEnd; }
            }
            else {
                w.objid = __float_as_int(q0.x);
                const int32_t w2l = __float_as_int(q0.y);
                w.meshid = __float_as_int(q1.x);
                w.top_hit = __float_as_int(q1.y);
                w.top_miss = __float_as_int(q1.z);
                if (LDSN && (__float_as_int(q0.w) & kTlasIdentity)) {
                    w.ray = w.lray;
                }
                else if (w2l >= 0) {
                    m4 m;
                    m.r0 = ldm<LDSN>(sc, w2l + 0); m.r1 = ldm<LDSN>(sc, w2l + 1);
                    m.r2 = ldm<LDSN>(sc, w2l + 2); m.r3 = ldm<LDSN>(sc, w2l + 3);
                    const f3 o = m4_apply(m, w.wray.org);
                    const f3 d = normalize(m4_applyXYZ(m, w.wray.dir));
                    slab_setup(w.ray, o, d);
                }
                else {
                    w.ray = w.wray;
                }
                is_hit = true;
                w.node = __float_as_int(q0.z);
            if (w.stop_t == kInf && __float_as_int(q1.w) != 0) w.node = anyhit_root(w.node, __float_as_int(q1.w), w.ray.dir);
            }
            if (w.node == kLinkEnd) {
                w.node = is_hit ? w.top_hit : w.top_miss;
                w.top_hit = kLinkEnd; w.top_miss = kLinkEnd;
                w.ray = w.wray;
            }
        }
        if (COUNT) { job.cost(w.payload, cnt->ray_nodes, cnt->ray_tris); cnt->ray_nodes = 0; cnt->ray_tris = 0; }
        if (job.finish(w.payload, w.hit, w.hit.objid >= 0, a, b, stop_t)) goto restart;
    }
}

#ifndef ATN_REFILL_LANES
#define ATN_REFILL_LANES 16
#endif
constexpr uint32_t kRefillLanes = ATN_REFILL_LANES;
#ifndef ATN_FETCH_CHUNK
#define ATN_FETCH_CHUNK 128
#endif
constexpr uint32_t kFetchChunk = ATN_FETCH_CHUNK;
constexpr int kTraceWavesPerBlock = kTraceBlock / 64;
struct TraceShared {
    float4 stage[kTraceWavesPerBlock][kFetchChunk][2]; float stop[kTraceWavesPerBlock][kFetchChunk];
};

template <bool COUNT, class Job, bool LDSN = false>
ATN_DEV void trace_refill(const DevScene& sc, TraceShared& sh, uint32_t count, uint32_t* fetch_counter,
                          const Job& job, TravCounters* cnt)
{
    const char* __restrict__ nb = reinterpret_cast<const char*>(sc.nodes);
    const float t_min = sc.bvh_hit_min > 0 ? sc.bvh_hit_min : job.t_min;
    const uint32_t lane = __lane_id();
    float4 (*stage)[2] = sh.stage[threadIdx.x >> 6];
    float* stage_stop = sh.stop[threadIdx.x >> 6];

    uint32_t c_count = 0, c_next = 0;
    bool drained = false;
    const uint32_t wave_id = (blockIdx.x * blockDim.x + threadIdx.x) >> 6;
    const uint32_t n_waves = (gridDim.x * blockDim.x) >> 6;
    bool first_chunk = true;
    bool all_finite = true;
    uint32_t iter = 0;
    Walk w;
    slab_setup(w.wray, mk3(0.0F), mk3(0.0F, 0.0F, 1.0F));
    w.ray = w.wray;
    w.node = kLinkEnd;
    w.t_max = 0.0F; w.stop_t = -kInf; w.payload = 0;
    w.hit.t = kInf; w.hit.objid = -1; w.hit.tri = -1; w.hit.a = 0.0F; w.hit.b = 0.0F; w.hit.meshid = -1;
    w.objid = -1; w.meshid = -1; w.top_hit = kLinkEnd; w.top_miss = kLinkEnd;
    w.pending = false;

    for (;;) {
        unsigned long long m_idle = __ballot(w.node == kLinkEnd);
        uint32_t n_idle = (uint32_t)__popcll(m_idle);
        if (n_idle >= kRefillLanes) {
            if (walk_finish<COUNT, Job, LDSN>(w, sc, job, cnt)) {
                m_idle = __ballot(w.node == kLinkEnd);
                n_idle = (uint32_t)__popcll(m_idle);
                all_finite = __all(w.node == kLinkEnd || w.ray.finite) != 0;
            }
            if (c_next >= c_count && !drained) {
                uint32_t base = 0;
                if (first_chunk) {
                    base = wave_id * kFetchChunk;
                    first_chunk = false;
                }
                else {
                    if (lane == 0) base = (atomicAdd(fetch_counter, 1u) + n_waves) * kFetchChunk;
                }
                base = (uint32_t)__builtin_amdgcn_readfirstlane((int)base);
                if (base >= count) { drained = true; c_count = 0; c_next = 0; }
                else {
                    c_count = count - base < kFetchChunk ? count - base : kFetchChunk;
                    c_next = 0;
#pragma unroll
                    for (uint32_t e = 0; e < kFetchChunk; e += 64) {
                        if (e + lane < c_count) {
                            float4 a, b;
                            float st;
                            job.fetch(base + e + lane, a, b, st);
                            stage[e + lane][0] = a;
                            stage[e + lane][1] = b;
                            stage_stop[e + lane] = st;
                        }
                    }
                }
            }
            if (c_next < c_count) {
                const uint32_t avail = c_count - c_next;
                if (w.node == kLinkEnd) {
                    const uint32_t k = bits_below_lane(m_idle);
                    if (k < avail) walk_start<LDSN, COUNT>(w, sc, stage[c_next + k][0], stage[c_next + k][1], stage_stop[c_next + k], cnt);
                }
                c_next += n_idle < avail ? n_idle : avail;
                all_finite = __all(w.node == kLinkEnd || w.ray.finite) != 0;
            }
            else if (n_idle == 64u) {
                break;
            }
        }
        walk_iteration<COUNT, kInnerBurst, Job, LDSN, ATN_DEFER_FINISH != 0>(w, all_finite, sc, nb, t_min, job, cnt, iter++);
    }
}

}
```

aten_amd/renderer.py:

```python
import ctypes as C

import numpy as np

from . import layout as L
from ._lib import Destination, K_NAMES, lib


class AtenAmdError(RuntimeError):
    pass


class PathTracing:
    def __init__(self, device=0):
        self._l = lib()
        self._ctx = C.c_void_p()
        rc = self._l.atn_create(C.byref(self._ctx), device)
        if rc != 0:
            raise AtenAmdError("atn_create failed (%d): no usable HIP device; libaten_amd has no CPU fallback" % rc)
        if self._l.atn_sizeof_scene_desc() != C.sizeof(L.SceneDesc):
            raise AtenAmdError("atn_scene_desc ABI mismatch")
        if self._l.atn_sizeof_destination() != C.sizeof(Destination):
            raise AtenAmdError("atn_destination ABI mismatch")
        self.width = self.height = 0
        self._skin_sizes = {}
# ... 67 lines not shown
            self._check(self._l.atn_skin_compute(self._ctx, skin, int(bool(is_restart)), None, None))
            return None
        mn, mx = np.zeros(3, np.float32), np.zeros(3, np.float32)
        self._check(self._l.atn_skin_compute(self._ctx, skin, int(bool(is_restart)), mn.ctypes.data, mx.ctypes.data))
        return mn, mx

    def lbvh_rebuild_list_skinned(self, list_index, skin):
        self._check(self._l.atn_lbvh_rebuild_list_skinned(self._ctx, list_index, skin))

    def skin_buffer(self, skin, name):
        which = {"pos": 0, "nml": 1, "prev": 2, "bbox": 3, "area": 4}[name]
        nv, nt = self._skin_sizes.get(skin, (0, 0))
        out = np.zeros((max(nv, 1), 4), np.float32) if which < 3 else np.zeros(6 if which == 3 else max(nt, 1), np.float32)
        self._check(self._l.atn_skin_download(self._ctx, skin, which, out.ctypes.data))
        return out[:nv] if which < 3 else (out if which == 3 else out[:nt])

    def skin_scene_arrays(self, skin, n_vertices, n_triangles):
        out = dict(shade=np.zeros((n_triangles, 8, 4), np.float32), vtx_pos=np.zeros((n_vertices, 4), np.float32),
                   vtx_nml=np.zeros((n_vertices, 4), np.float32), triangles=np.zeros(n_triangles, L.TRIANGLE_PARAM))
        for which, k in ((5, "shade"), (6, "vtx_pos"), (7, "vtx_nml"), (8, "triangles")):
            self._check(self._l.atn_skin_download(self._ctx, skin, which, out[k].ctypes.data))
        return out

    def bvh_list_bytes(self, list_index):
        n = C.c_uint32(0)
        self._check(self._l.atn_skin_download_list(self._ctx, list_index, None, 0, C.byref(n)))
        out = np.zeros(n.value, np.uint8)
        self._check(self._l.atn_skin_download_list(self._ctx, list_index, out.ctypes.data, n.value, C.byref(n)))
        return out

    def skin_close(self, skin):
        self._check(self._l.atn_skin_destroy(self._ctx, skin))
        self._skin_sizes.pop(skin, None)

    def set_geometry_motion(self, on=True):
        self._check(self._l.atn_set_geometry_motion(self._ctx, int(bool(on))))

    def geometry_motion_stats(self):
        s = np.zeros(3, np.uint64)
        self._check(self._l.atn_geometry_motion_stats(self._ctx, s.ctypes.data))
        return dict(passes=int(s[0]), copies=int(s[1]), copied_float4=int(s[2]))

    def geometry_motion_matrices(self):
        a, b = np.zeros((4, 4), np.float32), np.zeros((4, 4), np.float32)
        self._check(self._l.atn_geometry_motion_matrices(self._ctx, a.ctypes.data, b.ctypes.data))
        return a, b

    def scene_device_arrays(self):
        p = [C.c_void_p() for _ in range(3)]
        self._check(self._l.atn_scene_device_arrays(self._ctx, C.byref(p[0]), C.byref(p[1]), C.byref(p[2])))
        return tuple(x.value for x in p)

    def updateCamera(self, cam):
        self._check(self._l.atn_update_camera(self._ctx, cam.ctypes.data))

    def initSampler(self, width, height, seed=0):
        self._check(self._l.atn_init_sampler(self._ctx, width, height, seed))

    def setRandom(self, seeds):
        seeds = np.ascontiguousarray(seeds, np.uint32)
        self._check(self._l.atn_set_random(self._ctx, seeds.ctypes.data, len(seeds)))

    def getRandom(self):
        out = np.zeros(self._l.atn_random_count(self._ctx), np.uint32)
        if len(out):
            self._check(self._l.atn_get_random(self._ctx, out.ctypes.data, len(out)))
        return out

    def setScreenShard(self, rank, world):
        self._check(self._l.atn_set_screen_shard(self._ctx, rank, world))

    def render(self, width, height, max_depth=5, rr_depth=3, spp=1, frame=0, progressive=True,
               break_on_terminate=True, download=True, count_stats=False, profile=False):
        d = Destination(width, height, max_depth, rr_depth, spp, frame, int(progressive),
                        int(break_on_terminate), int(count_stats), int(profile))
        out = np.empty((height, width, 4), np.float32) if download else None
        self._check(self._l.atn_render(self._ctx, C.byref(d), out.ctypes.data if download else None))
        self.width, self.height = width, height
        return out

    def set_upload_options(self, anyhit_twin=None, anyhit_twin_dirs=None, node_layout=None, planar_lights=None):
        v = lambda x: -1 if x is None else int(x)
        self._check(self._l.atn_set_upload_options(self._ctx, v(anyhit_twin), v(anyhit_twin_dirs), v(node_layout), v(planar_lights)))

    def set_shade_math(self, relaxed):
        self._check(self._l.atn_set_shade_math(self._ctx, int(relaxed)))

    def set_regeneration(self, on):
        self._check(self._l.atn_set_regeneration(self._ctx, int(on)))

    def render_burst(self, width, height, n_frames, max_depth=5, rr_depth=3, spp=1, frame=0, progressive=True,
                     break_on_terminate=True, download=True, profile=False):
        d = Destination(width, height, max_depth, rr_depth, spp, frame, int(progressive), int(break_on_terminate), 0, int(profile))
        out = np.empty((height, width, 4), np.float32) if download else None
        self._check(self._l.atn_render_burst(self._ctx, C.byref(d), n_frames, out.ctypes.data if download else None))
        self.width, self.height = width, height
        return out

    def regen_stage_counts(self):
        n = C.c_uint32(0)
        self._check(self._l.atn_regen_stage_counts(self._ctx, None, None, 0, C.byref(n)))
        q = np.zeros(n.value, np.uint32); sh = np.zeros(n.value, np.uint32)
        if n.value:
            self._check(self._l.atn_regen_stage_counts(self._ctx, q.ctypes.data, sh.ctypes.data, n.value, C.byref(n)))
        return q, sh

    def set_path_batches(self, n):
        self._check(self._l.atn_set_path_batches(self._ctx, n))

    def set_frames_in_flight(self, n):
        self._check(self._l.atn_set_frames_in_flight(self._ctx, n))

    def side_stream_ptr(self):
        p = self._l.atn_side_stream(self._ctx)
        if not p:
            raise AtenAmdError("atn_side_stream failed")
        return p

    def bank_streams(self):
        sw, cc = C.c_int32(0), C.c_int32(0)
        self._check(self._l.atn_bank_streams(self._ctx, C.byref(sw), C.byref(cc)))
        self.side_stream_concurrent = bool(cc.value & 2)
        return sw.value, bool(cc.value & 1)

    def set_sampling_options(self, ibl_importance=False, tex_bilinear=False):
        self._check(self._l.atn_set_sampling_options(self._ctx, int(ibl_importance), int(tex_bilinear)))

    def sample_texture(self, texid, uv):
        uv = np.ascontiguousarray(uv, np.float32).reshape(-1, 2)
        out = np.zeros((len(uv), 4), np.float32)
        self._check(self._l.atn_sample_texture(self._ctx, texid, len(uv), uv.ctypes.data, out.ctypes.data))
        return out

    def reset(self):
        self._check(self._l.atn_reset(self._ctx))

    def synchronize(self):
        self._check(self._l.atn_synchronize(self._ctx))

    def film_device_ptr(self):
        return self._l.atn_film_device(self._ctx)

    def tile_device_ptr(self):
        return self._l.atn_tile_device(self._ctx)

    def tile_slots(self):
        return int(self._l.atn_tile_slots(self._ctx))

    def stream_ptr(self):
        return self._l.atn_stream(self._ctx)

    def assemble_tiles(self, gathered_dev_ptr, world, out_dev_ptr=None, stream_ptr=None):
        self._check(self._l.atn_assemble_tiles_on(self._ctx, gathered_dev_ptr, world, out_dev_ptr, stream_ptr))

    def download_film(self):
        out = np.empty((self.height, self.width, 4), np.float32)
        self._check(self._l.atn_download_film(self._ctx, out.ctypes.data))
        return out

    def upload_film(self, film):
        film = np.ascontiguousarray(film, np.float32)
        h, w = film.shape[:2]
        self._check(self._l.atn_upload_film(self._ctx, w, h, film.ctypes.data))
        self.width, self.height = w, h

    def path_cost(self):
# ... 451 lines not shown
```

aten_amd/scene/scenedefs.py:

```python
import os

import numpy as np

from .. import layout as L
from .builder import SceneBuilder

ASSETS = os.path.join(os.path.dirname(os.path.dirname(os.path.dirname(os.path.abspath(__file__)))), "assets")


def cornell_box(asset_dir=None):
    asset_dir = asset_dir or os.path.join(ASSETS, "cornellbox")
    b = SceneBuilder()
    emit = b.add_material("light", L.MTRL_EMISSIVE, (1.0, 1.0, 1.0))

    def create_mtrl(name, mtype, clr, albedo, nml):
        if name == "shortBox":
            return b.add_material(name, L.MTRL_SPECULAR, (0.7, 0.6, 0.5), roughness=0.1, ior=0.01)
        if name == "floor":
            return b.add_material(name, L.MTRL_GGX, (0.7, 0.6, 0.5), roughness=0.1, ior=0.01)
        return b.add_material(name, mtype, clr)

    objs = b.load_obj(os.path.join(asset_dir, "orig.obj"), create_mtrl=create_mtrl,
                      separate_objs=True, normal_on_the_fly=True)
    light = b.create_instance(objs[0])
    b.add_area_light(light, b.materials[emit][1]["baseColor"][:3], 200.0)
    for o in objs[1:]:
        b.create_instance(o)
    b.set_background((0.0, 0.0, 0.0))
    cam = dict(pos=(0.0, 1.0, 3.0), at=(0.0, 1.0, 0.0), vfov=45.0)
    return b.build(), cam


def synthetic_envmap(w=2048, h=1024, seed=0):
    v = (np.arange(h, dtype=np.float32) + 0.5) / h
    u = (np.arange(w, dtype=np.float32) + 0.5) / w
    t = np.clip((v - 0.45) / 0.3, 0, 1)
    t = t * t * (3 - 2 * t)
    ground = np.array([0.35, 0.30, 0.25], np.float32)
    sky = np.array([0.45, 0.65, 1.0], np.float32)
    col = (ground[None, :] * (1 - t[:, None]) + sky[None, :] * t[:, None]) * np.float32(1.2)
    img = np.repeat(col[:, None, :], w, axis=1)
    d2 = (u[None, :] - 0.3) ** 2 + (v[:, None] - 0.8) ** 2
    sun = np.exp(-d2 / 0.0008).astype(np.float32)
    img = img + sun[:, :, None] * np.array([60, 55, 45], np.float32)[None, None, :]
    out = np.ones((h, w, 4), np.float32)
    out[:, :, :3] = img
    return out


def envmap_avg_illum(tex):
    h = tex.shape[0]
    lum = 0.212639 * tex[:, :, 0] + 0.71517 * tex[:, :, 1] + 0.0721926 * tex[:, :, 2]
    theta = np.pi * (np.arange(h) + 0.5) / h
    s = np.sin(theta)[:, None]
    return float((lum * s).sum() / (s.sum() * tex.shape[1]))


def sponza_lod(asset_dir=None, mtype=L.MTRL_GGX, ibl=True, use_sbvh=True, textures=True, bvh_options=None, optimize_sbvh=False,
               add_lights=None):
    asset_dir = asset_dir or os.path.join(ASSETS, "sponza")
    b = SceneBuilder()

    def create_mtrl(name, mt, clr, albedo, nml):
        alb = b.load_image(os.path.join(asset_dir, albedo)) if (albedo and textures) else -1
        nm = b.load_image(os.path.join(asset_dir, nml)) if (nml and textures) else -1
        if mtype == L.MTRL_GGX:
            return b.add_material(name, L.MTRL_GGX, clr, albedo_map=alb, normal_map=nm, roughness=0.3, ior=0.01)
        if mtype == L.MTRL_DISNEY:
            return b.add_material(name, L.MTRL_DISNEY, clr, albedo_map=alb, normal_map=nm,
                                  roughness=0.4, metallic=0.1, specular=0.5, clearcoat=0.2)
        return b.add_material(name, mt, clr, albedo_map=alb, normal_map=nm)

    cam = dict(pos=(0.0, 1.0, 3.0), at=(0.0, 1.0, 0.0), vfov=45.0)
    b.bvh_options = dict(order_point=cam["pos"]) if bvh_options is None else bvh_options
    objs = b.load_obj(os.path.join(asset_dir, "sponza_lod.obj"), create_mtrl=create_mtrl)
    if use_sbvh:
        b.import_sbvh(objs[0], os.path.join(asset_dir, "sponza_lod.sbvh"), optimize=optimize_sbvh)
    b.create_instance(objs[0])
    if add_lights is not None:
        p = np.asarray(b.pos, np.float32).reshape(-1, 4)[:, :3]
        add_lights(b, p.min(axis=0), p.max(axis=0), cam)
    if ibl:
        env = synthetic_envmap()
        tid = b.add_texture("synthetic_sky_2048x1024", env)
        b.add_ibl(tid, avg_illum=envmap_avg_illum(env))
    else:
        b.set_background((1.0, 1.0, 1.0))
    return b.build(), cam


def _light_grid(b, bmin, bmax, intensity, scale, step=5):
    sv = (np.asarray(bmax, np.float32) - np.asarray(bmin, np.float32)) / np.float32(step)
    colors = [(1.0, 0.0, 0.0), (0.0, 1.0, 0.0), (0.0, 0.0, 1.0)]
    num = 0
    y = np.float32(bmin[1])
    for _ in range(step):
        z = np.float32(0.0)
        for _ in range(step):
            x = np.float32(0.0)
            for _ in range(step):
                b.add_point_light((float(x), float(y), float(z)), colors[num % 3], intensity, scale=scale)
                x = np.float32(x + sv[0])
                num += 1
            z = np.float32(z + sv[2])
        y = np.float32(y + sv[1])


def many_light_sponza(asset_dir=None, textures=True):
    def add(b, bmin, bmax, cam):
        _light_grid(b, bmin, bmax, 500.0, 0.01)
        b.add_point_light(tuple(float(c) for c in cam["at"]), (1.0, 1.0, 1.0), 500.0, scale=0.01)
    fs, cam = sponza_lod(asset_dir, ibl=False, textures=textures, add_lights=add)
    return fs, cam


def many_light_cornell(n=8, asset_dir=None):
    asset_dir = asset_dir or os.path.join(ASSETS, "cornellbox")
    b = SceneBuilder()

    def create_mtrl(name, mtype, clr, albedo, nml):
        return b.add_material(name, L.MTRL_DIFFUSE, (1.0, 1.0, 1.0))

    objs = b.load_obj(os.path.join(asset_dir, "orig.obj"), create_mtrl=create_mtrl, separate_objs=True, normal_on_the_fly=True)
    for o in objs:
        if b.objects[o]["name"] != "light":
            b.create_instance(o)
    rng = np.random.default_rng(7)
    colors = [(1.0, 0.3, 0.3), (0.3, 1.0, 0.3), (0.3, 0.3, 1.0), (1.0, 1.0, 0.6)]
    for i in range(n):
        x, z = rng.uniform(-0.8, 0.8), rng.uniform(-0.8, 0.8)
        b.add_point_light((float(x), 1.2 + 0.3 * float(rng.uniform()), float(z)), colors[i % 4], 4.0 * 8.0 / max(n, 1))
    b.set_background((0.0, 0.0, 0.0))
    cam = dict(pos=(0.0, 1.0, 3.0), at=(0.0, 1.0, 0.0), vfov=45.0)
    return b.build(), cam


def cornell_box_variant(lights="area", move_boxes=True, asset_dir=None, extra_materials=False):
    asset_dir = asset_dir or os.path.join(ASSETS, "cornellbox")
    b = SceneBuilder()
    emit = b.add_material("light", L.MTRL_EMISSIVE, (1.0, 1.0, 1.0))

    def create_mtrl(name, mtype, clr, albedo, nml):
        if name == "shortBox":
            return b.add_material(name, L.MTRL_DISNEY, (0.7, 0.6, 0.5), roughness=0.35, metallic=0.3,
                                  specular=0.6, clearcoat=0.4, clearcoatGloss=0.7, sheen=0.3)
        if name == "floor":
            return b.add_material(name, L.MTRL_GGX, (0.7, 0.6, 0.5), roughness=0.1, ior=0.01)
        if extra_materials is True and name == "tallBox":
            return b.add_material(name, L.MTRL_REFRACTION, (0.9, 0.9, 0.9), ior=1.5)
        if extra_materials and name == "leftWall":
            return b.add_material(name, L.MTRL_OREN_NAYAR, clr, roughness=0.6)
        if extra_materials == "rough" and name == "tallBox":
            return b.add_material(name, L.MTRL_MICROFACET_REFRACTION, (0.9, 0.9, 0.9), ior=1.5, roughness=0.2)
        if extra_materials == "rough" and name == "rightWall":
            return b.add_material(name, L.MTRL_VELVET, clr, roughness=0.4)
        if extra_materials == "carpaint" and name == "shortBox":
            return b.add_carpaint_material(name, (1.0, 1.0, 1.0))
        if extra_materials == "carpaint" and name == "backWall":
            return b.add_carpaint_material(name, (0.9, 0.9, 0.9), diffuse_color=(0.1, 0.3, 0.8), flakes_color=(0.9, 0.9, 1.0),
                                           flake_size=0.4, clearcoat_ior=1.6, flake_scale=60.0)
        if extra_materials == "retro" and name == "rightWall":
# ... 505 lines not shown
```

include/aten_amd.h:

```cpp
#ifndef ATEN_AMD_H_
#define ATEN_AMD_H_

#include "aten_layout.h"

#ifdef __cplusplus
extern "C" {
#endif

typedef struct atn_ctx atn_ctx;

typedef enum atn_status {
    ATN_OK = 0,
    ATN_ERR_INVALID_ARG = -1,
    ATN_ERR_NO_DEVICE = -2,
    ATN_ERR_HIP = -3,
    ATN_ERR_NO_SCENE = -4,
    ATN_ERR_UNSUPPORTED = -5,
    ATN_ERR_OUT_OF_MEMORY = -6
} atn_status;

typedef struct atn_destination {
    int32_t width;
    int32_t height;
    int32_t maxDepth;
    int32_t russianRouletteDepth;
    int32_t sample;
    uint32_t frame;
    int32_t progressive;
    int32_t break_on_terminate;
    int32_t count_stats;
    int32_t profile;
} atn_destination;

int atn_create(atn_ctx** out, int device_ordinal);
void atn_destroy(atn_ctx* ctx);
const char* atn_last_error(atn_ctx* ctx);

int atn_upload_scene(atn_ctx* ctx, const atn_scene_desc* scene);

int atn_update_tlas(atn_ctx* ctx, const atn_object_param* objects, uint32_t n_objects,
                    const atn_mat4* matrices, uint32_t n_matrices,
                    const atn_bvh_node* top_nodes, uint32_t n_top_nodes);

int atn_set_upload_options(atn_ctx* ctx, int32_t anyhit_twin, int32_t anyhit_twin_dirs, int32_t node_layout, int32_t planar_lights);

int atn_update_camera(atn_ctx* ctx, const atn_camera_param* camera);



int atn_update_geometry(atn_ctx* ctx, const atn_vec4* vtx_pos, const atn_vec4* vtx_nml, uint32_t n_vertices, uint32_t vtx_offset,
                        const atn_triangle_param* triangles, uint32_t n_triangles, uint32_t tri_offset);
int atn_scene_device_arrays(atn_ctx* ctx, void** vtx_pos, void** vtx_nml, void** triangles);
int atn_lbvh_rebuild_list(atn_ctx* ctx, uint32_t list_index, uint32_t tri_offset, uint32_t n_triangles,
                          const float bbox_min[3], const float bbox_max[3]);
int atn_lbvh_build(atn_ctx* ctx, const atn_triangle_param* triangles, uint32_t n_triangles, int32_t tri_id_offset,
                   const float bbox_min[3], const float bbox_max[3], const atn_vec4* vtx_pos, uint32_t n_vertices, int32_t vtx_offset,
                   atn_bvh_node* out_nodes, uint32_t* out_sorted_codes, uint32_t* out_sorted_indices);

typedef uint32_t atn_skin;
int atn_skin_create(atn_ctx* ctx, const atn_skinning_vertex* vertices, uint32_t n_vertices, uint32_t vtx_offset,
                    uint32_t tri_offset, uint32_t n_triangles, uint32_t n_matrices, atn_skin* out_skin);
int atn_skin_update(atn_ctx* ctx, atn_skin skin, const atn_mat4* matrices, uint32_t n);
int atn_skin_compute(atn_ctx* ctx, atn_skin skin, int32_t is_restart, float bbox_min[3], float bbox_max[3]);
int atn_lbvh_rebuild_list_skinned(atn_ctx* ctx, uint32_t list_index, atn_skin skin);
int atn_skin_download(atn_ctx* ctx, atn_skin skin, int32_t which, void* out_host);
int atn_skin_download_list(atn_ctx* ctx, uint32_t list_index, void* out_host, uint32_t capacity_bytes, uint32_t* n_bytes);
int atn_skin_destroy(atn_ctx* ctx, atn_skin skin);

int atn_init_sampler(atn_ctx* ctx, int32_t width, int32_t height, int32_t seed);
int atn_set_random(atn_ctx* ctx, const uint32_t* seeds, uint32_t n);
int atn_get_random(atn_ctx* ctx, uint32_t* out_host, uint32_t n);
uint32_t atn_random_count(atn_ctx* ctx);

int atn_set_screen_shard(atn_ctx* ctx, int32_t rank, int32_t world);

int atn_render(atn_ctx* ctx, const atn_destination* dst, atn_vec4* out_host);

int atn_set_regeneration(atn_ctx* ctx, int32_t mode);
int32_t atn_get_regeneration(atn_ctx* ctx);
int atn_render_burst(atn_ctx* ctx, const atn_destination* dst, int32_t n_frames, atn_vec4* out_host);
int atn_regen_stage_counts(atn_ctx* ctx, uint32_t* closest, uint32_t* shadow, uint32_t capacity, uint32_t* n_stages);

int atn_set_shade_math(atn_ctx* ctx, int32_t mode);

int atn_reset(atn_ctx* ctx);

void* atn_film_device(atn_ctx* ctx);
void* atn_tile_device(atn_ctx* ctx);
uint32_t atn_anyhit_twins(atn_ctx* ctx);
uint32_t atn_planar_area_lights(atn_ctx* ctx);
uint32_t atn_tile_slots(atn_ctx* ctx);
void* atn_stream(atn_ctx* ctx);
int atn_synchronize(atn_ctx* ctx);

int atn_assemble_tiles(atn_ctx* ctx, const void* gathered_dev, int32_t world, void* film_dev_out);
int atn_assemble_tiles_on(atn_ctx* ctx, const void* gathered_dev, int32_t world, void* film_dev_out, void* hip_stream);
int atn_download_film(atn_ctx* ctx, atn_vec4* out_host);
int atn_upload_film(atn_ctx* ctx, int32_t width, int32_t height, const atn_vec4* film_host);

int atn_get_stats(atn_ctx* ctx, uint64_t out[8]);
int atn_download_path_cost(atn_ctx* ctx, uint32_t* out_host);

enum { ATN_K_GEN = 0, ATN_K_TRACE_CLOSEST = 1, ATN_K_SHADE = 2, ATN_K_TRACE_SHADOW = 3,
       ATN_K_ACCUM = 4, ATN_K_GATHER = 5,
       ATN_K_SVGF_PREPARE = 6, ATN_K_SVGF_TEMPORAL = 7, ATN_K_SVGF_VARIANCE = 8, ATN_K_SVGF_ATROUS = 9,
       ATN_K_TRACE_FUSED = 10,
       ATN_K_COUNT = 11 };
int atn_get_kernel_times(atn_ctx* ctx, float ms[ATN_K_COUNT], uint32_t launches[ATN_K_COUNT]);
int atn_reset_kernel_times(atn_ctx* ctx);

int atn_set_path_batches(atn_ctx* ctx, int32_t n);

int atn_set_frames_in_flight(atn_ctx* ctx, int32_t n);
int atn_bank_streams(atn_ctx* ctx, int32_t* swaps, int32_t* concurrent);
void* atn_side_stream(atn_ctx* ctx);

int atn_set_sampling_options(atn_ctx* ctx, int32_t ibl_importance, int32_t tex_bilinear);
int atn_sample_texture(atn_ctx* ctx, int32_t texid, uint32_t n, const float* uv_host, float* out_host);

typedef struct atn_mgpu atn_mgpu;
int atn_mgpu_create(atn_mgpu** out, const int32_t* devices, int32_t n_devices);
void atn_mgpu_destroy(atn_mgpu* mg);
const char* atn_mgpu_last_error(atn_mgpu* mg);
int32_t atn_mgpu_shard_count(atn_mgpu* mg);
int32_t atn_mgpu_shard_device(atn_mgpu* mg, int32_t shard);
int atn_mgpu_upload_scene(atn_mgpu* mg, const atn_scene_desc* scene);
int atn_mgpu_update_tlas(atn_mgpu* mg, const atn_object_param* objects, uint32_t n_objects,
// ... 86 lines not shown
```

Measured before the change: 667.8 Mrays/s.

## Specialize BVH traversal for single-instance scenes with a direct BLAS walk

Adds a compile-time DIRECT traversal path used when the scene has a single root instance (root_direct). The ray is transformed into the BLAS local space once, at staging time, and the walk skips all TLAS node handling, objid/meshid tracking and top-level return bookkeeping. objid/meshid are reconstructed at finish from scene constants. The aim is fewer registers, branches and per-iteration checks in the hot traversal loop. The trace grid cap is also made a macro, still defaulting to 18. The change adds more kernel template instantiations and a toggle to disable the path.

```diff
diff --git a/aten_amd/_lib.py b/aten_amd/_lib.py
--- a/aten_amd/_lib.py
+++ b/aten_amd/_lib.py
@@ -34,6 +34,7 @@
     "atn_mgpu_download_film",
     "atn_set_regeneration", "atn_get_regeneration", "atn_render_burst", "atn_regen_stage_counts",
     "atn_mgpu_set_regeneration", "atn_mgpu_render_burst", "atn_set_upload_options", "atn_libm_probe", "atn_set_shade_math",
+    "atn_set_direct_walk", "atn_direct_walk",
 ]
 
 
@@ -85,6 +86,8 @@
         l.atn_render.argtypes = [vp, C.POINTER(Destination), vp]
         l.atn_reset.argtypes = [vp]
         l.atn_set_upload_options.argtypes = [vp, C.c_int32, C.c_int32, C.c_int32, C.c_int32]
+        l.atn_set_direct_walk.argtypes = [vp, C.c_int32]
+        l.atn_direct_walk.argtypes = [vp]; l.atn_direct_walk.restype = C.c_uint32
         l.atn_set_regeneration.argtypes = [vp, C.c_int32]
         l.atn_set_shade_math.argtypes = [vp, C.c_int32]
         l.atn_get_regeneration.argtypes = [vp]; l.atn_get_regeneration.restype = C.c_int32
diff --git a/aten_amd/csrc/aten_amd.hip b/aten_amd/csrc/aten_amd.hip
--- a/aten_amd/csrc/aten_amd.hip
+++ b/aten_amd/csrc/aten_amd.hip
@@ -96,6 +96,7 @@
     int env_anyhit_twin = 1;
     int env_anyhit_twin_dirs = 8;
     bool opt_node_layout = true, opt_planar_lights = true;
+    bool opt_direct_walk = true;
     bool env_atrous4 = true;
     int env_shade_waves = 0;
     int env_flavour = -1;
@@ -766,6 +767,7 @@
         ATN_HIP(hipGetLastError());
         ATN_HIP(hipStreamSynchronize(stream));
         scene = img.params;
+        if (!opt_direct_walk) scene.root_direct = 0;
         scene.nodes = nodes.p; scene.tris = tris.p; scene.shade_tris = shade_tris.p; scene.vtx_pos = vtx_pos.p; scene.vtx_nml = vtx_nml.p;
         scene.objects = objects.p; scene.matrices = matrices.p; scene.materials = materials.p; scene.carpaint = carpaint.p;
         scene.toon = toon.p; scene.npr_lights = npr_lights.p; scene.screen_shadow = img.screen_shadow.empty() ? nullptr : screen_shadow.p;
@@ -903,6 +905,7 @@
         tlas_refs.swap(new_refs);
         scene.root_link = root;
         fill_root_direct(scene, rec.data(), top_base, n_mtxs ? mtxs : (host_matrices.size() == n_host_matrices ? host_matrices.data() : nullptr), n_mtxs ? n_mtxs : n_host_matrices);
+        if (!opt_direct_walk) scene.root_direct = 0;
         scene.node_bytes = (uint32_t)(top_base + top_bytes);
         scene.ident_row = c.ident_row;
         if (n_mtxs) scene.mtx_quads = (uint32_t)mv.size();
@@ -1375,13 +1378,16 @@
         return (env_lds_nodes && b <= kLdsNodesMaxBytes) ? (uint32_t)b : 0u;
     }
 
+#ifndef ATN_TRACE_GRID_IN_FLIGHT
+#define ATN_TRACE_GRID_IN_FLIGHT 18
+#endif
     uint32_t trace_grid(uint32_t n_jobs, bool refill) const
     {
         if (refill) {
             const uint32_t waves_per_block = (uint32_t)kTraceBlock / 64u;
             uint32_t blocks = ((n_jobs + atn::kFetchChunk - 1u) / atn::kFetchChunk + waves_per_block - 1u) / waves_per_block;
             if (blocks < 1u) blocks = 1u;
-            const uint32_t cap = (frames_in_flight > 1 ? 256u * 18u : 256u * 32u) / waves_per_block;
+            const uint32_t cap = (frames_in_flight > 1 ? 256u * (uint32_t)ATN_TRACE_GRID_IN_FLIGHT : 256u * 32u) / waves_per_block;
             return blocks < cap ? blocks : cap;
         }
         return grid_for(n_jobs);
@@ -1408,10 +1414,10 @@
     void launch_trace(const PassPlan& p, const PathBuffers& pb, bool count, int32_t b, hipStream_t st)
     {
         const dim3 g(p.trace_grid), t(p.refill ? (uint32_t)kTraceBlock : 256u);
-        with_flags([&](auto c, auto refill) {
+        with_flags([&](auto c, auto refill, auto direct) {
             if constexpr (SHADOW) hipLaunchKernelGGL((k_trace_shadow<decltype(c)::value, decltype(refill)::value>), g, t, 0, st, pb, scene, b);
-            else hipLaunchKernelGGL((k_trace_closest<decltype(c)::value, decltype(refill)::value>), g, t, 0, st, pb, scene, b);
-        }, count, p.refill);
+            else hipLaunchKernelGGL((k_trace_closest<decltype(c)::value, decltype(refill)::value, decltype(direct)::value>), g, t, 0, st, pb, scene, b);
+        }, count, p.refill, !SHADOW && direct_walk(scene, false));
     }
 
     template <bool SVGF>
@@ -2845,6 +2851,13 @@
     if (planar_lights >= 0) ctx->r.opt_planar_lights = planar_lights != 0;
     return ATN_OK;
 }
+int atn_set_direct_walk(atn_ctx* ctx, int32_t on)
+{
+    CTX_QUIET_OR_FAIL(ctx);
+    ctx->r.opt_direct_walk = on != 0;
+    return ATN_OK;
+}
+uint32_t atn_direct_walk(atn_ctx* ctx) { return (ctx && ctx->r.has_scene && ctx->r.scene.root_direct != 0) ? 1u : 0u; }
 int atn_update_camera(atn_ctx* ctx, const atn_camera_param* camera) { CTX_OR_FAIL(ctx); return guarded(ctx, [&] { return ctx->r.updateCamera(camera); }); }
 
 int atn_update_tlas(atn_ctx* ctx, const atn_object_param* objects, uint32_t n_objects, const atn_mat4* matrices, uint32_t n_matrices,
@@ -3417,9 +3430,9 @@
         const bool refill = r.refill_walk(false);
         const dim3 g(r.trace_grid(n, refill)), t(refill ? (uint32_t)atn::kTraceBlock : 256u);
         const atn_ray* rp = rays.p;
-        atn::with_flags([&](auto c, auto rf) {
-            hipLaunchKernelGGL((atn::k_trace_batch<decltype(c)::value, decltype(rf)::value>), g, t, 0, r.stream, r.scene, rp, n, t_min, t_max, out.p, st.p);
-        }, stats_out != nullptr, refill);
+        atn::with_flags([&](auto c, auto rf, auto direct) {
+            hipLaunchKernelGGL((atn::k_trace_batch<decltype(c)::value, decltype(rf)::value, decltype(direct)::value>), g, t, 0, r.stream, r.scene, rp, n, t_min, t_max, out.p, st.p);
+        }, stats_out != nullptr, refill, atn::direct_walk(r.scene, false));
     }
     C_HIP(r, hipGetLastError());
     C_HIP(r, hipMemcpyAsync(out_host, out.p, (size_t)n * sizeof(atn_intersection), hipMemcpyDeviceToHost, r.stream));
diff --git a/aten_amd/csrc/device/kernels.hpp b/aten_amd/csrc/device/kernels.hpp
--- a/aten_amd/csrc/device/kernels.hpp
+++ b/aten_amd/csrc/device/kernels.hpp
@@ -349,16 +349,16 @@
 #define ATN_TRACE_ATTR
 #endif
 
-template <bool COUNT, bool REFILL, class Job, bool LDSN = false>
+template <bool COUNT, bool REFILL, class Job, bool LDSN = false, bool DIRECT = false>
 ATN_DEV void trace_dispatch(const DevScene& sc, uint32_t count, uint32_t* fetch_counter, const Job& job, TravCounters* tc)
 {
     if constexpr (REFILL) {
         __shared__ TraceShared sh;
         if (LDSN) lds_scene_copy(sc);
-        trace_refill<COUNT, Job, LDSN>(sc, sh, count, fetch_counter, job, tc);
+        trace_refill<COUNT, Job, LDSN, DIRECT>(sc, sh, count, fetch_counter, job, tc);
     }
     else {
-        trace_simple<COUNT, Job, LDSN>(sc, count, job, tc);
+        trace_simple<COUNT, Job, LDSN, DIRECT>(sc, count, job, tc);
     }
 }
 
@@ -385,13 +385,13 @@
     }
 };
 
-template <bool COUNT, bool REFILL>
+template <bool COUNT, bool REFILL, bool DIRECT = false>
 __global__ void __launch_bounds__(kTraceBlock > 256 ? kTraceBlock : 256) k_trace_closest(PathBuffers pb, DevScene sc, int32_t bounce)
 {
     const uint32_t count = pb.q_count[bounce];
     const ClosestJob job{ pb, pb.queue[bounce & 1], kEps };
     TravCounters tc{};
-    trace_dispatch<COUNT, REFILL>(sc, count, &pb.fetch_closest[bounce], job, &tc);
+    trace_dispatch<COUNT, REFILL, ClosestJob, false, DIRECT>(sc, count, &pb.fetch_closest[bounce], job, &tc);
     if (COUNT) {
         if (blockIdx.x == 0 && threadIdx.x == 0) atomicAdd(&pb.stats[0], (unsigned long long)count);
         wave_add_stat(&pb.stats[3], tc.nodes);
@@ -1008,14 +1008,14 @@
     }
 };
 
-template <bool REFILL, bool ALPHA, bool LDSN = false, bool REGEN = false>
+template <bool REFILL, bool ALPHA, bool LDSN = false, bool REGEN = false, bool DIRECT = false>
 __global__ void ATN_TRACE_ATTR __launch_bounds__(kTraceBlock > 256 ? kTraceBlock : 256) k_trace_fused(PathBuffers pb, DevScene sc, int32_t bs, int32_t bc, int32_t launch)
 {
     const uint32_t n_shadow = bs >= 0 ? pb.sh_count[bs] : 0u;
     const uint32_t n_closest = bc >= 0 ? pb.q_count[bc] : 0u;
     const FusedJob<ALPHA, REGEN> job{ ShadowJob<ALPHA, REGEN>{ pb, sc, kEps }, ClosestJob{ pb, pb.queue[(bc >= 0 ? bc : 0) & 1], kEps }, n_shadow, kEps };
     TravCounters tc{};
-    trace_dispatch<false, REFILL, FusedJob<ALPHA, REGEN>, LDSN>(sc, n_shadow + n_closest, &pb.fetch_closest[launch], job, &tc);
+    trace_dispatch<false, REFILL, FusedJob<ALPHA, REGEN>, LDSN, DIRECT>(sc, n_shadow + n_closest, &pb.fetch_closest[launch], job, &tc);
 }
 
 template <int MS>
@@ -1127,14 +1127,14 @@
     ATN_DEV void cost(uint32_t, uint32_t, uint32_t) const {}
 };
 
-template <bool COUNT, bool REFILL>
+template <bool COUNT, bool REFILL, bool DIRECT = false>
 __global__ void __launch_bounds__(kTraceBlock > 256 ? kTraceBlock : 256) k_trace_batch(DevScene sc, const atn_ray* __restrict__ rays, uint32_t n,
                                                      float t_min, float t_max, atn_intersection* out,
                                                      unsigned long long* stats)
 {
     const BatchJob job{ sc, rays, out, t_min, t_max };
     TravCounters tc{};
-    trace_dispatch<COUNT, REFILL>(sc, n, reinterpret_cast<uint32_t*>(&stats[7]), job, &tc);
+    trace_dispatch<COUNT, REFILL, BatchJob, false, DIRECT>(sc, n, reinterpret_cast<uint32_t*>(&stats[7]), job, &tc);
     if (COUNT) { wave_add_stat(&stats[3], tc.nodes); wave_add_stat(&stats[4], tc.tris); }
 }
 
diff --git a/aten_amd/csrc/device/launch.hpp b/aten_amd/csrc/device/launch.hpp
--- a/aten_amd/csrc/device/launch.hpp
+++ b/aten_amd/csrc/device/launch.hpp
@@ -56,14 +56,21 @@
                         refill ? (uint32_t)kTraceBlock : p.block, p.lds_bytes, p.refill && stage == 0 ? ATN_K_TRACE_CLOSEST : ATN_K_TRACE_FUSED };
 }
 
+inline bool direct_walk(const DevScene& sc, bool lds) { return sc.root_direct != 0 && !lds; }
+
 template <bool REGEN>
 void launch_trace_fused(const TraceLaunch& l, hipStream_t st, const PathBuffers& pb, const DevScene& sc, int32_t bs, int32_t bc, int32_t launch)
 {
     const dim3 g(l.grid), t(l.block);
-    if constexpr (!REGEN) if (l.closest) { hipLaunchKernelGGL((k_trace_closest<false, false>), g, t, l.lds_bytes, st, pb, sc, bc); return; }
-    with_flags([&](auto refill, auto alpha, auto lds) {
-        hipLaunchKernelGGL((k_trace_fused<decltype(refill)::value, decltype(alpha)::value, decltype(lds)::value, REGEN>), g, t, l.lds_bytes, st, pb, sc, bs, bc, launch);
-    }, l.refill, sc.any_alpha != 0, l.lds);
+    if constexpr (!REGEN) if (l.closest) {
+        if (direct_walk(sc, l.lds)) hipLaunchKernelGGL((k_trace_closest<false, false, true>), g, t, l.lds_bytes, st, pb, sc, bc);
+        else hipLaunchKernelGGL((k_trace_closest<false, false>), g, t, l.lds_bytes, st, pb, sc, bc);
+        return;
+    }
+    with_flags([&](auto refill, auto alpha, auto lds, auto direct) {
+        constexpr bool kDirect = decltype(direct)::value && !decltype(lds)::value && !REGEN;
+        hipLaunchKernelGGL((k_trace_fused<decltype(refill)::value, decltype(alpha)::value, decltype(lds)::value, REGEN, kDirect>), g, t, l.lds_bytes, st, pb, sc, bs, bc, launch);
+    }, l.refill, sc.any_alpha != 0, l.lds, !REGEN && direct_walk(sc, l.lds));
 }
 
 void regen_launch_begin(uint32_t grid, hipStream_t st, const PathBuffers& pb, const FrameParams& fp, const atn_camera_param& cam);
diff --git a/aten_amd/csrc/device/traverse.hpp b/aten_amd/csrc/device/traverse.hpp
--- a/aten_amd/csrc/device/traverse.hpp
+++ b/aten_amd/csrc/device/traverse.hpp
@@ -96,6 +96,7 @@
     else return sc.matrices[row];
 }
 
+template <bool DIRECT = false>
 ATN_DEV bool leaf_test(const RaySlab& ray, const float4& q0, const float4& q1, const float4& q2, float t_min,
                        Hit& hit, float& t_max, int32_t objid, int32_t meshid, bool& accept, float& t_out)
 {
@@ -113,7 +114,8 @@
     accept = (t_min < (is_hit ? t : kInf)) && is_hit && (t < hit.t);
     if (accept) {
         hit.t = t; hit.a = beta; hit.b = gamma;
-        hit.objid = objid; hit.tri = __float_as_int(q0.w); hit.meshid = meshid;
+        hit.tri = __float_as_int(q0.w);
+        if constexpr (!DIRECT) { hit.objid = objid; hit.meshid = meshid; }
         t_max = t;
     }
     t_out = t;
@@ -138,12 +140,42 @@
     return root + delta + (int32_t)((twin & 1) ? octant : 0u) * delta;
 }
 
-template <bool IDENT = false, bool COUNT = false>
+ATN_DEV void direct_local_ray(const DevScene& sc, const f3& org, const f3& dir, f3& o, f3& d)
+{
+    if (sc.root_w2l >= 0) {
+        m4 m;
+        m.r0 = make_float4(sc.root_m[0], sc.root_m[1], sc.root_m[2], sc.root_m[3]);
+        m.r1 = make_float4(sc.root_m[4], sc.root_m[5], sc.root_m[6], sc.root_m[7]);
+        m.r2 = make_float4(sc.root_m[8], sc.root_m[9], sc.root_m[10], sc.root_m[11]);
+        m.r3 = make_float4(0.0F, 0.0F, 0.0F, 1.0F);
+        o = m4_apply(m, org);
+        d = normalize(m4_applyXYZ(m, dir));
+    }
+    else {
+        o = org; d = dir;
+    }
+}
+
+template <bool IDENT = false, bool COUNT = false, bool DIRECT = false, bool LOCAL = false>
 ATN_DEV void walk_start(Walk& w, const DevScene& sc, const float4& a, const float4& b, float stop_t, TravCounters* cnt = nullptr)
 {
+    static_assert(!(DIRECT && IDENT) && (DIRECT || !LOCAL), "DIRECT walks read global memory; only they are handed local rays");
     w.t_max = a.w;
     w.stop_t = stop_t;
     w.payload = __float_as_uint(b.w);
+    if constexpr (DIRECT) {
+        w.hit.t = kInf; w.hit.tri = -1; w.hit.a = 0.0F; w.hit.b = 0.0F;
+        if (COUNT) { cnt->nodes++; cnt->ray_nodes++; }
+        if constexpr (LOCAL) slab_setup(w.ray, mk3(a), mk3(b));
+        else {
+            f3 o, d;
+            direct_local_ray(sc, mk3(a), mk3(b), o, d);
+            slab_setup(w.ray, o, d);
+        }
+        w.node = sc.root_blas;
+        if (sc.root_twin != 0 && stop_t == kInf) w.node = anyhit_root(sc.root_blas, sc.root_twin, w.ray.dir);
+        return;
+    }
     w.hit.t = kInf; w.hit.objid = -1; w.hit.tri = -1; w.hit.a = 0.0F; w.hit.b = 0.0F; w.hit.meshid = -1;
     if (sc.root_direct) {
         if (COUNT) { cnt->nodes++; cnt->ray_nodes++; }
@@ -220,7 +252,26 @@
 #ifndef ATN_TLAS_PERIOD
 #define ATN_TLAS_PERIOD 3
 #endif
-template <bool COUNT, int BURST, class Job, bool LDSN = false, bool DEFER = false>
+
+ATN_DEV Hit direct_hit(const Walk& w, const DevScene& sc)
+{
+    const bool any = w.hit.tri >= 0;
+    Hit h;
+    h.t = w.hit.t; h.tri = w.hit.tri; h.a = w.hit.a; h.b = w.hit.b;
+    h.objid = any ? sc.root_objid : -1; h.meshid = any ? sc.root_meshid : -1;
+    return h;
+}
+template <bool DIRECT, class Job>
+ATN_DEV bool walk_job_finish(const Job& job, const Walk& w, const DevScene& sc, float4& ra, float4& rb, float& rstop)
+{
+    if constexpr (DIRECT) {
+        const Hit h = direct_hit(w, sc);
+        return job.finish(w.payload, h, h.objid >= 0, ra, rb, rstop);
+    }
+    else return job.finish(w.payload, w.hit, w.hit.objid >= 0, ra, rb, rstop);
+}
+
+template <bool COUNT, int BURST, class Job, bool LDSN = false, bool DEFER = false, bool DIRECT = false>
 ATN_DEV void walk_iteration(Walk& w, bool& all_finite, const DevScene& sc, const char* __restrict__ nb, float t_min,
                             const Job& job, TravCounters* cnt, uint32_t iter = 0)
 {
@@ -230,26 +281,29 @@
     bool ended = live && w.node == kLinkEnd;
     bool is_hit = false;
 
-    const bool tlas_turn = LDSN || ATN_TLAS_PERIOD <= 1 || (iter % (uint32_t)ATN_TLAS_PERIOD) == 0u;
-    const bool at_tlas = w.node != kLinkEnd && (w.node & kLinkTypeMask) == kLinkTlasBit && tlas_turn;
-    if (w.node != kLinkEnd && w.node < 0 && ((w.node & kLinkLeafBit) || tlas_turn)) {
+    const bool tlas_turn = DIRECT || LDSN || ATN_TLAS_PERIOD <= 1 || (iter % (uint32_t)ATN_TLAS_PERIOD) == 0u;
+    const bool at_tlas = !DIRECT && w.node != kLinkEnd && (w.node & kLinkTypeMask) == kLinkTlasBit && tlas_turn;
+    if (w.node != kLinkEnd && w.node < 0 && (DIRECT || (w.node & kLinkLeafBit) || tlas_turn)) {
         const uint32_t off = (uint32_t)w.node & kLinkOffsetMask;
         float4 q0, q1;
         if constexpr (LDSN) { q0 = ldn<true>(nb, off); q1 = ldn<true>(nb, off + 16u); }
         else { const __amdgpu_buffer_rsrc_t rs = node_rsrc(sc); q0 = ld16_buf(rs, off); q1 = ld16_buf(rs, off + 16u); }
         if (COUNT) { cnt->nodes++; cnt->ray_nodes++; }
-        if (w.node & kLinkLeafBit) {
+        if (DIRECT || (w.node & kLinkLeafBit)) {
             float4 q2;
             if constexpr (LDSN) q2 = ldn<true>(nb, off + 32u);
             else q2 = ld16_buf(node_rsrc(sc), off + 32u);
             if (COUNT) { cnt->tris++; cnt->ray_tris++; }
             bool accept; float t;
-            is_hit = leaf_test(w.ray, q0, q1, q2, t_min, w.hit, w.t_max, w.objid, w.meshid, accept, t);
+            is_hit = leaf_test<DIRECT>(w.ray, q0, q1, q2, t_min, w.hit, w.t_max, w.objid, w.meshid, accept, t);
             w.node = __float_as_int(q1.w);
-            if (accept && t <= w.stop_t) { w.node = kLinkEnd; w.top_hit = kLinkEnd; w.top_miss = kLinkEnd; }
+            if (accept && t <= w.stop_t) {
+                w.node = kLinkEnd;
+                if constexpr (!DIRECT) { w.top_hit = kLinkEnd; w.top_miss = kLinkEnd; }
+            }
             ended = w.node == kLinkEnd;
         }
-        else {
+        else if constexpr (!DIRECT) {
             w.objid = __float_as_int(q0.x);
             const int32_t w2l = __float_as_int(q0.y);
             w.meshid = __float_as_int(q1.x);
@@ -277,20 +331,23 @@
     }
 
     if (ended) {
-        w.node = is_hit ? w.top_hit : w.top_miss;
-        w.top_hit = kLinkEnd; w.top_miss = kLinkEnd;
-        if (w.node != kLinkEnd) w.ray = w.wray;
+        if constexpr (!DIRECT) {
+            w.node = is_hit ? w.top_hit : w.top_miss;
+            w.top_hit = kLinkEnd; w.top_miss = kLinkEnd;
+            if (w.node != kLinkEnd) w.ray = w.wray;
+        }
         if (w.node == kLinkEnd) {
             if constexpr (DEFER) w.pending = true;
             else {
                 float4 ra, rb;
                 float rstop;
                 if (COUNT) { job.cost(w.payload, cnt->ray_nodes, cnt->ray_tris); cnt->ray_nodes = 0; cnt->ray_tris = 0; }
-                if (job.finish(w.payload, w.hit, w.hit.objid >= 0, ra, rb, rstop)) walk_start<LDSN, COUNT>(w, sc, ra, rb, rstop, cnt);
-            }
-        }
-    }
-    if (__any(ended || at_tlas) || !all_finite) all_finite = __all(w.node == kLinkEnd || w.ray.finite) != 0;
+                if (walk_job_finish<DIRECT>(job, w, sc, ra, rb, rstop)) walk_start<LDSN, COUNT, DIRECT>(w, sc, ra, rb, rstop, cnt);
+            }
+        }
+    }
+    if constexpr (DIRECT && DEFER) { if (!all_finite) all_finite = __all(w.node == kLinkEnd || w.ray.finite) != 0; }
+    else if (__any(ended || at_tlas) || !all_finite) all_finite = __all(w.node == kLinkEnd || w.ray.finite) != 0;
 }
 
 template <bool COUNT>
@@ -348,7 +405,7 @@
 #ifndef ATN_DEFER_FINISH
 #define ATN_DEFER_FINISH 1
 #endif
-template <bool COUNT, class Job, bool LDSN>
+template <bool COUNT, class Job, bool LDSN, bool DIRECT = false>
 ATN_DEV bool walk_finish(Walk& w, const DevScene& sc, const Job& job, TravCounters* cnt)
 {
     bool restarted = false;
@@ -357,14 +414,15 @@
         float4 ra, rb;
         float rstop;
         if (COUNT) { job.cost(w.payload, cnt->ray_nodes, cnt->ray_tris); cnt->ray_nodes = 0; cnt->ray_tris = 0; }
-        if (job.finish(w.payload, w.hit, w.hit.objid >= 0, ra, rb, rstop)) { walk_start<LDSN, COUNT>(w, sc, ra, rb, rstop, cnt); restarted = true; }
+        if (walk_job_finish<DIRECT>(job, w, sc, ra, rb, rstop)) { walk_start<LDSN, COUNT, DIRECT>(w, sc, ra, rb, rstop, cnt); restarted = true; }
     }
     return __any(restarted) != 0;
 }
 
-template <bool COUNT, class Job, bool LDSN = false>
+template <bool COUNT, class Job, bool LDSN = false, bool DIRECT = false>
 ATN_DEV void trace_simple(const DevScene& sc, uint32_t count, const Job& job, TravCounters* cnt)
 {
+    static_assert(!(DIRECT && LDSN), "the DIRECT walk reads global memory");
     const char* __restrict__ nb = reinterpret_cast<const char*>(sc.nodes);
     if constexpr (LDSN) lds_scene_copy(sc);
     const float t_min = sc.bvh_hit_min > 0 ? sc.bvh_hit_min : job.t_min;
@@ -387,7 +445,7 @@
             continue;
         }
       restart:
-        walk_start<LDSN, COUNT>(w, sc, a, b, stop_t, cnt);
+        walk_start<LDSN, COUNT, DIRECT>(w, sc, a, b, stop_t, cnt);
         while (w.node != kLinkEnd) {
             const uint32_t off = (uint32_t)w.node & kLinkOffsetMask;
             const float4 q0 = ldn<LDSN>(nb, off);
@@ -400,15 +458,18 @@
                 w.node = __float_as_int(box ? q0.w : q1.w);
                 is_hit = false;
             }
-            else if (w.node & kLinkLeafBit) {
+            else if (DIRECT || (w.node & kLinkLeafBit)) {
                 const float4 q2 = ldn<LDSN>(nb, off + 32u);
                 if (COUNT) { cnt->tris++; cnt->ray_tris++; }
                 bool accept; float t;
-                is_hit = leaf_test(w.ray, q0, q1, q2, t_min, w.hit, w.t_max, w.objid, w.meshid, accept, t);
+                is_hit = leaf_test<DIRECT>(w.ray, q0, q1, q2, t_min, w.hit, w.t_max, w.objid, w.meshid, accept, t);
                 w.node = __float_as_int(q1.w);
-                if (accept && t <= w.stop_t) { w.node = kLinkEnd; w.top_hit = kLinkEnd; w.top_miss = kLinkEnd; }
-            }
-            else {
+                if (accept && t <= w.stop_t) {
+                    w.node = kLinkEnd;
+                    if constexpr (!DIRECT) { w.top_hit = kLinkEnd; w.top_miss = kLinkEnd; }
+                }
+            }
+            else if constexpr (!DIRECT) {
                 w.objid = __float_as_int(q0.x);
                 const int32_t w2l = __float_as_int(q0.y);
                 w.meshid = __float_as_int(q1.x);
@@ -432,14 +493,14 @@
                 w.node = __float_as_int(q0.z);
             if (w.stop_t == kInf && __float_as_int(q1.w) != 0) w.node = anyhit_root(w.node, __float_as_int(q1.w), w.ray.dir);
             }
-            if (w.node == kLinkEnd) {
+            if constexpr (!DIRECT) if (w.node == kLinkEnd) {
                 w.node = is_hit ? w.top_hit : w.top_miss;
                 w.top_hit = kLinkEnd; w.top_miss = kLinkEnd;
                 w.ray = w.wray;
             }
         }
         if (COUNT) { job.cost(w.payload, cnt->ray_nodes, cnt->ray_tris); cnt->ray_nodes = 0; cnt->ray_tris = 0; }
-        if (job.finish(w.payload, w.hit, w.hit.objid >= 0, a, b, stop_t)) goto restart;
+        if (walk_job_finish<DIRECT>(job, w, sc, a, b, stop_t)) goto restart;
     }
 }
 
@@ -456,10 +517,11 @@
     float4 stage[kTraceWavesPerBlock][kFetchChunk][2]; float stop[kTraceWavesPerBlock][kFetchChunk];
 };
 
-template <bool COUNT, class Job, bool LDSN = false>
+template <bool COUNT, class Job, bool LDSN = false, bool DIRECT = false>
 ATN_DEV void trace_refill(const DevScene& sc, TraceShared& sh, uint32_t count, uint32_t* fetch_counter,
                           const Job& job, TravCounters* cnt)
 {
+    static_assert(!(DIRECT && LDSN), "the DIRECT walk reads global memory");
     const char* __restrict__ nb = reinterpret_cast<const char*>(sc.nodes);
     const float t_min = sc.bvh_hit_min > 0 ? sc.bvh_hit_min : job.t_min;
     const uint32_t lane = __lane_id();
@@ -474,19 +536,25 @@
     bool all_finite = true;
     uint32_t iter = 0;
     Walk w;
-    slab_setup(w.wray, mk3(0.0F), mk3(0.0F, 0.0F, 1.0F));
-    w.ray = w.wray;
+    if constexpr (DIRECT) {
+        slab_setup(w.ray, mk3(0.0F), mk3(0.0F, 0.0F, 1.0F));
+        w.hit.t = kInf; w.hit.tri = -1; w.hit.a = 0.0F; w.hit.b = 0.0F;
+    }
+    else {
+        slab_setup(w.wray, mk3(0.0F), mk3(0.0F, 0.0F, 1.0F));
+        w.ray = w.wray;
+        w.hit.t = kInf; w.hit.objid = -1; w.hit.tri = -1; w.hit.a = 0.0F; w.hit.b = 0.0F; w.hit.meshid = -1;
+        w.objid = -1; w.meshid = -1; w.top_hit = kLinkEnd; w.top_miss = kLinkEnd;
+    }
     w.node = kLinkEnd;
     w.t_max = 0.0F; w.stop_t = -kInf; w.payload = 0;
-    w.hit.t = kInf; w.hit.objid = -1; w.hit.tri = -1; w.hit.a = 0.0F; w.hit.b = 0.0F; w.hit.meshid = -1;
-    w.objid = -1; w.meshid = -1; w.top_hit = kLinkEnd; w.top_miss = kLinkEnd;
     w.pending = false;
 
     for (;;) {
         unsigned long long m_idle = __ballot(w.node == kLinkEnd);
         uint32_t n_idle = (uint32_t)__popcll(m_idle);
         if (n_idle >= kRefillLanes) {
-            if (walk_finish<COUNT, Job, LDSN>(w, sc, job, cnt)) {
+            if (walk_finish<COUNT, Job, LDSN, DIRECT>(w, sc, job, cnt)) {
                 m_idle = __ballot(w.node == kLinkEnd);
                 n_idle = (uint32_t)__popcll(m_idle);
                 all_finite = __all(w.node == kLinkEnd || w.ray.finite) != 0;
@@ -511,6 +579,12 @@
                             float4 a, b;
                             float st;
                             job.fetch(base + e + lane, a, b, st);
+                            if constexpr (DIRECT) {
+                                f3 o, d;
+                                direct_local_ray(sc, mk3(a), mk3(b), o, d);
+                                a = make_float4(o.x, o.y, o.z, a.w);
+                                b = make_float4(d.x, d.y, d.z, b.w);
+                            }
                             stage[e + lane][0] = a;
                             stage[e + lane][1] = b;
                             stage_stop[e + lane] = st;
@@ -522,7 +596,7 @@
                 const uint32_t avail = c_count - c_next;
                 if (w.node == kLinkEnd) {
                     const uint32_t k = bits_below_lane(m_idle);
-                    if (k < avail) walk_start<LDSN, COUNT>(w, sc, stage[c_next + k][0], stage[c_next + k][1], stage_stop[c_next + k], cnt);
+                    if (k < avail) walk_start<LDSN, COUNT, DIRECT, DIRECT>(w, sc, stage[c_next + k][0], stage[c_next + k][1], stage_stop[c_next + k], cnt);
                 }
                 c_next += n_idle < avail ? n_idle : avail;
                 all_finite = __all(w.node == kLinkEnd || w.ray.finite) != 0;
@@ -531,8 +605,8 @@
                 break;
             }
         }
-        walk_iteration<COUNT, kInnerBurst, Job, LDSN, ATN_DEFER_FINISH != 0>(w, all_finite, sc, nb, t_min, job, cnt, iter++);
-    }
-}
-
-}
+        walk_iteration<COUNT, kInnerBurst, Job, LDSN, ATN_DEFER_FINISH != 0, DIRECT>(w, all_finite, sc, nb, t_min, job, cnt, iter++);
+    }
+}
+
+}
diff --git a/aten_amd/renderer.py b/aten_amd/renderer.py
--- a/aten_amd/renderer.py
+++ b/aten_amd/renderer.py
@@ -173,6 +173,12 @@
     def set_upload_options(self, anyhit_twin=None, anyhit_twin_dirs=None, node_layout=None, planar_lights=None):
         v = lambda x: -1 if x is None else int(x)
         self._check(self._l.atn_set_upload_options(self._ctx, v(anyhit_twin), v(anyhit_twin_dirs), v(node_layout), v(planar_lights)))
+
+    def set_direct_walk(self, on):
+        self._check(self._l.atn_set_direct_walk(self._ctx, int(on)))
+
+    def direct_walk(self):
+        return bool(self._l.atn_direct_walk(self._ctx))
 
     def set_shade_math(self, relaxed):
         self._check(self._l.atn_set_shade_math(self._ctx, int(relaxed)))
diff --git a/aten_amd/scene/scenedefs.py b/aten_amd/scene/scenedefs.py
--- a/aten_amd/scene/scenedefs.py
+++ b/aten_amd/scene/scenedefs.py
@@ -57,7 +57,7 @@
 
 
 def sponza_lod(asset_dir=None, mtype=L.MTRL_GGX, ibl=True, use_sbvh=True, textures=True, bvh_options=None, optimize_sbvh=False,
-               add_lights=None):
+               add_lights=None, instance_matrix=None):
     asset_dir = asset_dir or os.path.join(ASSETS, "sponza")
     b = SceneBuilder()
 
@@ -76,7 +76,7 @@
     objs = b.load_obj(os.path.join(asset_dir, "sponza_lod.obj"), create_mtrl=create_mtrl)
     if use_sbvh:
         b.import_sbvh(objs[0], os.path.join(asset_dir, "sponza_lod.sbvh"), optimize=optimize_sbvh)
-    b.create_instance(objs[0])
+    b.create_instance(objs[0], instance_matrix)
     if add_lights is not None:
         p = np.asarray(b.pos, np.float32).reshape(-1, 4)[:, :3]
         add_lights(b, p.min(axis=0), p.max(axis=0), cam)
diff --git a/include/aten_amd.h b/include/aten_amd.h
--- a/include/aten_amd.h
+++ b/include/aten_amd.h
@@ -43,6 +43,8 @@
                     const atn_bvh_node* top_nodes, uint32_t n_top_nodes);
 
 int atn_set_upload_options(atn_ctx* ctx, int32_t anyhit_twin, int32_t anyhit_twin_dirs, int32_t node_layout, int32_t planar_lights);
+int atn_set_direct_walk(atn_ctx* ctx, int32_t on);
+uint32_t atn_direct_walk(atn_ctx* ctx);
 
 int atn_update_camera(atn_ctx* ctx, const atn_camera_param* camera);
 
```

After: 672.9 Mrays/s, median of 6. Within noise of the previous version (+0.8%).
